# golmschenk/sr-gan

Measured on AMD Instinct MI355X. Metric: SRGAN train images/sec (G+D step), higher is better.
Workload: dtype f32; 1 GPU; crowd SRGAN (KnnDenseNetCat D/DNN + DCGenerator) 512x512, batch 16/GPU, dnn_training_step + gan_training_step per step; global_batch=16, image_size=512, schedule=shared-forwards, parallelism=dp1, random_init_weights=True, gradient_penalty=active, launch=eager (Python tape enqueues every kernel), schedule_check=not run: the --full option runs it

## Files before the change

### include/srgan_hip.h

```cpp
#ifndef SRGAN_HIP_H
#define SRGAN_HIP_H

#include <stdint.h>

#ifdef __cplusplus
extern "C" {
#endif

int srgan_version(void);
const char* srgan_build_id(void);
const char* srgan_last_error(void);

#define SRGAN_DTYPE_F32 0x1u
#define SRGAN_DTYPE_BF16 0x2u
#define SRGAN_DTYPE_F16 0x4u
#define SRGAN_FEATURE_FUSED_BNRELU 0x1u
#define SRGAN_FEATURE_SPLITK_WORKSPACE 0x2u
#define SRGAN_FEATURE_LIVE_PROFILE 0x4u
#define SRGAN_FEATURE_BLOCKED16 0x8u
#define SRGAN_FEATURE_BATCHED_SHADOWS 0x10u
#define SRGAN_FEATURE_CROWD_FULL_IMAGE 0x20u
#define SRGAN_FEATURE_IMAGE_BATCHES 0x40u
#define SRGAN_FEATURE_BATCH_NORM_TRAIN 0x80u
#define SRGAN_FEATURE_BLOCKED_BATCH_NORM 0x100u
#define SRGAN_FEATURE_BLOCKED_FROZEN_NORM 0x200u
#define SRGAN_FEATURE_DEVICE_DRAWS 0x400u
#define SRGAN_FEATURE_IMAGE_SUMMARIES 0x800u
#define SRGAN_FEATURE_DISTRIBUTION_SUMMARIES 0x1000u
typedef struct srgan_capabilities_t {
  int32_t abi_version;
  int32_t struct_bytes;
  char arch[16];
  uint32_t dtypes;
  uint32_t features;
  int64_t workspace_bytes;
  int64_t max_tensor_elements;
} srgan_capabilities_t;
int srgan_capabilities(srgan_capabilities_t* out, int32_t out_bytes);
int64_t srgan_workspace_bytes(void);
int srgan_set_workspace(void* workspace, int64_t bytes, void* stream);
int srgan_split_is_ordered(void* stream);

typedef struct srgan_conv_desc {
  int32_t N, C, H, W;
  int32_t K, R, S;
  int32_t stride_h, stride_w, pad_h, pad_w;
  int32_t OH, OW;
  int64_t x_batch_stride, y_batch_stride;
  int32_t compute_dtype;
} srgan_conv_desc;

#define SRGAN_COMPUTE_F32 0
#define SRGAN_COMPUTE_BF16 1
#define SRGAN_COMPUTE_F16 2

int srgan_conv2d_fwd(const srgan_conv_desc* desc, const float* x, const float* w, const float* bias, float* y,
                     int force_kernel, void* stream);

int srgan_conv2d_bwd_data(const srgan_conv_desc* desc, const float* gy, const float* w, const float* bias, float* gx,
                          int accumulate, int force_kernel, void* stream);

int srgan_conv2d_bwd_weight(const srgan_conv_desc* desc, const float* x, const float* gy, float* gw, int accumulate,
                            int force_kernel, void* stream);

typedef struct srgan_bn_relu { const float* mean; const float* inv_std; const float* gamma; const float* beta; } srgan_bn_relu;
int srgan_conv2d_bnrelu_supported(const srgan_conv_desc* desc, int pass);
int srgan_conv2d_fwd_bnrelu(const srgan_conv_desc* desc, const float* x, const srgan_bn_relu* bn, const float* w,
                            const float* bias, float* y, void* stream);
int srgan_conv2d_fwd_bnrelu_splits(const srgan_conv_desc* desc);
int srgan_conv2d_fwd_bnrelu_into_zeros(const srgan_conv_desc* desc, const float* x, const srgan_bn_relu* bn, const float* w,
                                       const float* bias, float* y, void* stream);
int srgan_conv2d_bwd_data_bnrelu(const srgan_conv_desc* desc, const float* gy, const float* w, const srgan_bn_relu* bn,
                                 const float* x, float* gx, float* g_gamma, float* g_beta, int accumulate, void* stream);
int srgan_conv2d_bwd_weight_bnrelu(const srgan_conv_desc* desc, const float* x, const srgan_bn_relu* bn, const float* gy,
                                   float* gw, int accumulate, void* stream);
typedef struct srgan_bn_reduce_job {
  int64_t partial_offset;
  int32_t tiles, channels;
  const float* inv_std;
  float* g_gamma;
  float* g_beta;
} srgan_bn_reduce_job;
int64_t srgan_conv2d_bwd_data_bnrelu_tiles(const srgan_conv_desc* desc);
int srgan_conv2d_bwd_data_bnrelu_partials(const srgan_conv_desc* desc, const float* gy, const float* w, const srgan_bn_relu* bn,
                                          const float* x, float* gx, float* partials, int accumulate, void* stream);
int srgan_bn_partial_reduce_batched(const srgan_bn_reduce_job* jobs_device, int32_t count, int32_t max_channels, int32_t max_tiles,
                                    const float* scratch, void* stream);

int srgan_wgrad_group_plan(const srgan_conv_desc* desc, const srgan_bn_relu* bn, int64_t x_offset, int64_t gy_offset, float* gw,
                           int64_t gw_offset, int32_t group_size, int64_t group_weights, int64_t partial_offset, void* job,
                           int32_t* grid_x, int32_t* grid_y, int32_t* ragged, int64_t* partial_floats);
int srgan_wgrad_group_run(const void* jobs, int32_t count, int32_t kernel_size, int32_t grid_x, int32_t grid_y, int32_t ragged,
                          int32_t fused_bn, const float* x_base, const float* gy_base, float* gw_base, int64_t sum_co_ci_taps,
                          int64_t pixels, int64_t operand_elements, int64_t partial_floats, void* stream);

int srgan_gemm_f32(int32_t M, int32_t N, int32_t K, const float* A, int64_t sai, int64_t sak, const float* B,
                   int64_t sbk, int64_t sbj, float* C, int64_t sci, int64_t scj, const float* bias,
                   int32_t bias_on_columns, int accumulate, int force_kernel, void* stream);
int srgan_gemm(int32_t M, int32_t N, int32_t K, const float* A, int64_t sai, int64_t sak, const float* B,
               int64_t sbk, int64_t sbj, float* C, int64_t sci, int64_t scj, const float* bias,
               int32_t bias_on_columns, int accumulate, int force_kernel, int compute_dtype, void* stream);

int srgan_ew_unary(int op, const float* x, float* y, int64_t n, float p0, float p1, void* stream);
int srgan_ew_binary(int op, const float* a, const float* b, float* y, int64_t n, float p0, void* stream);
int srgan_fill(float* y, int64_t n, float value, void* stream);

int srgan_chan_affine(const float* x, const float* mean, const float* scale_a, const float* scale_b, const float* shift,
                      float* y, int32_t N, int32_t C, int64_t HW, void* stream);

int srgan_chan_affine_act(const float* x, const float* mean, const float* scale_a, const float* scale_b,
                          const float* shift, const float* mask, int relu, float* y, int32_t N, int32_t C, int64_t HW,
                          void* stream);
int srgan_chan_affine_act_strided(const float* x, const float* mean, const float* scale_a, const float* scale_b,
                                  const float* shift, const float* mask, int relu, float* y, int32_t N, int32_t C,
                                  int64_t HW, int64_t x_batch_stride, int64_t mask_batch_stride, int64_t y_batch_stride,
                                  int accumulate, void* stream);
int srgan_bn_conv_tangent_weights(const float* w, const float* q, const float* inv_std, const float* gamma,
                                  float* w_scaled, float* w_grad, float* gamma_grad, int32_t CO, int32_t CI, int32_t taps,
                                  void* stream);

int srgan_bn_conv_tangent_weights_job(const float* w, const float* inv_std, const float* gamma, float* w_grad,
                                      float* gamma_grad, int64_t offset, int32_t CO, int32_t CI, int32_t taps, void* job);
int srgan_bn_conv_tangent_weights_grouped(const void* jobs, int32_t count, int32_t max_inner, int32_t max_co, float* scaled_base,
                                          const float* q_base, void* stream);

int srgan_bn_act_bwd(const float* g, const float* x, const float* mean, const float* inv_std, const float* gamma,
                     const float* beta, int relu, float* gx, float* g_gamma, float* g_beta, int32_t N, int32_t C,
                     int64_t HW, int64_t g_batch_stride, int64_t x_batch_stride, int64_t gx_batch_stride,
                     int accumulate_gx, int unscaled, void* stream);

int srgan_batch_norm_train_stats(const float* x, float* mean, float* inv_std, float* running_mean, float* running_var,
                                 int64_t* num_batches_tracked, float momentum, float eps, int32_t N, int32_t C, int64_t HW,
                                 void* stream);
int srgan_batch_norm_train_fwd(const float* x, const float* mean, const float* inv_std, const float* gamma, const float* beta,
                               float slope, float* y, int32_t N, int32_t C, int64_t HW, void* stream);
int srgan_batch_norm_train_bwd_reduce(const float* g, const float* x, const float* mean, const float* inv_std, const float* gamma,
                                      const float* beta, float slope, float* sums, float* g_gamma, float* g_beta, int32_t N,
                                      int32_t C, int64_t HW, void* stream);
int srgan_batch_norm_train_bwd_apply(const float* g, const float* x, const float* mean, const float* inv_std, const float* gamma,
                                     const float* beta, float slope, const float* sums, float* gx, int32_t N, int32_t C, int64_t HW,
                                     void* stream);

int srgan_chan_reduce(const float* a, const float* b, const float* mean, const float* scale, float* out, int32_t N,
                      int32_t C, int64_t HW, int accumulate, void* stream);
int srgan_row_max(const float* x, float* out, int32_t B, int32_t F, void* stream);
int srgan_nearest_bin_onehot(const float* y, const float* bins, float* onehot, int32_t B, int32_t K, void* stream);

int srgan_copy_channels(const float* src, int32_t src_channels, int32_t src_first, float* dst, int32_t dst_channels,
                        int32_t dst_first, int32_t count, int32_t N, int64_t HW, int accumulate, void* stream);

int srgan_bn_relu_maxpool_fwd(const float* x, const float* mean, const float* inv_std, const float* gamma, const float* beta,
                              float* y, int32_t* argmax, int32_t N, int32_t C, int32_t H, int32_t W, int32_t k, int32_t s, int32_t p,
                              int32_t OH, int32_t OW, void* stream);
int srgan_bn_relu_maxpool_bwd_supported(int32_t N, int32_t C, int32_t H, int32_t W, int32_t k, int32_t s, int32_t p);
int srgan_bn_relu_maxpool_bwd(const float* gy, const int32_t* argmax, const float* x, const float* mean, const float* inv_std,
                              const float* gamma, const float* beta, float* gx, float* g_gamma, float* g_beta, int32_t N,
                              int32_t C, int32_t H, int32_t W, int32_t k, int32_t s, int32_t p, int32_t OH, int32_t OW,
                              void* stream);
int srgan_bn_relu_avgpool2_supported(int32_t N, int32_t C, int32_t H, int32_t W);
int srgan_bn_relu_avgpool2_fwd(const float* x, const float* mean, const float* inv_std, const float* gamma, const float* beta,
                               float* y, int32_t N, int32_t C, int32_t H, int32_t W, void* stream);
int srgan_bn_relu_avgpool2_bwd(const float* gy, const float* x, const float* mean, const float* inv_std, const float* gamma,
                               const float* beta, float* gx, float* g_gamma, float* g_beta, int32_t N, int32_t C, int32_t H,
                               int32_t W, void* stream);
int srgan_maxpool2d_fwd(const float* x, float* y, int32_t* argmax, int32_t planes, int32_t H, int32_t W, int32_t k,
                        int32_t s, int32_t p, int32_t OH, int32_t OW, void* stream);
int srgan_maxpool2d_bwd(const float* g, const int32_t* argmax, float* gx, int32_t planes, int32_t H, int32_t W, int32_t k,
                        int32_t s, int32_t p, int32_t OH, int32_t OW, void* stream);
int srgan_pool_scatter(const float* g, const int32_t* argmax, float* out, int32_t planes, int64_t in_plane,
                       int64_t out_plane, void* stream);
// ... 20 lines not shown

int srgan_image_batch_gather(const void* store, int store_dtype, int32_t count, int32_t C, int32_t h, int32_t w,
                             const float* labels, const int32_t* order, int64_t first, int32_t B, int32_t H, int32_t W,
                             float* out_images, float* out_labels, void* stream);

int srgan_crowd_extract_windows(const void* image_u8, int32_t H, int32_t W, const int32_t* ys, int32_t ny,
                                const int32_t* xs, int32_t nx, int32_t first, int32_t count, int32_t P,
                                float* out_images, void* stream);
int srgan_crowd_resize_bilinear(const float* in, int32_t B, int32_t h, int32_t w, int32_t P, float* out, void* stream);
int srgan_crowd_blend_windows(const float* densities, const float* counts, const int32_t* ys, int32_t ny, const int32_t* xs,
                              int32_t nx, int32_t H, int32_t W, int32_t P, float* out_density, float* out_count,
                              void* stream);

int srgan_image_grid(const float* images, int32_t N, int32_t C, int32_t H, int32_t W, int32_t nrow, int32_t padding,
                     float pad_value, int32_t normalize, float low, float high, float* out, void* stream);
int srgan_density_heatmaps(const float* labels, const float* predicted, int32_t B, int32_t M, int32_t h, int32_t w, int32_t P,
                           const float* lut, int32_t lut_entries, float* tiles, int64_t tile_stride, float* ranges, void* stream);

#define SRGAN_WASSERSTEIN_MAX_VALUES 16384
int srgan_wasserstein_1d(const float* u, int32_t n, const float* v, int32_t m, float* out, void* stream);
int srgan_kde_curves(const float* samples, const int32_t* offsets, int32_t C, int32_t G, float factor, float cut, float* support,
                     float* density, float* stats, void* stream);
int srgan_curve_frame(const float* vertices, const int32_t* offsets, int32_t C, const float* colours, const float* widths,
                      int32_t H, int32_t W, float x_lo, float x_hi, float y_lo, float y_hi, const float* background,
                      const float* grid_colour, const float* x_ticks, int32_t n_x, const float* y_ticks, int32_t n_y, float* out,
                      void* stream);

int srgan_crowd_iknn_map(const float* heads_yx, int32_t M, int32_t H, int32_t W, int32_t k, float epsilon, float upper_bound,
                         float* out, void* stream);
int srgan_crowd_density_label(const float* heads, int32_t M, int32_t H, int32_t W, float beta, const float* perspective,
                              int32_t flags, void* workspace, float* out, void* stream);

int srgan_adam_step(float* p, const float* g, float* m, float* v, int64_t n, float lr, float beta1, float beta2,
                    float eps, float weight_decay, int32_t step, void* stream);
int srgan_adam_step_counted(float* p, const float* g, float* m, float* v, int64_t n, float lr, float beta1, float beta2,
                            float eps, float weight_decay, int32_t* state, void* stream);

int srgan_pack_bf16(const float* src, uint16_t* dst, int64_t n, void* stream);
int srgan_unpack_bf16(const uint16_t* src, float* dst, int64_t n, void* stream);

int srgan_comm_available(void);
int srgan_comm_unique_id(void* id128);
int srgan_comm_init(void** comm, int32_t world_size, int32_t rank, const void* id128);
int srgan_comm_world_size(void* comm, int32_t* world_size);
int srgan_comm_destroy(void* comm);
int srgan_all_reduce_sum(void* comm, const void* send, void* recv, int64_t count, int32_t dtype, void* stream);
int srgan_reduce_scatter_sum(void* comm, const void* send, void* recv, int64_t recv_count, int32_t dtype, void* stream);
int srgan_all_gather(void* comm, const void* send, void* recv, int64_t send_count, int32_t dtype, void* stream);
int srgan_broadcast(void* comm, void* buffer, int64_t count, int32_t dtype, int32_t root, void* stream);

int srgan_h_pack(const float* x_nchw, void* out, const void* mask_ref, float slope, int32_t N, int32_t C, int64_t HW, int dtype,
                 void* stream);
int srgan_h_unpack(const void* x, float* out_nchw, int32_t N, int32_t C, int64_t HW, int dtype, void* stream);
int srgan_h_add(const void* a, const void* b, void* out, int64_t slots, int dtype, void* stream);
int srgan_h_channel_sums(const void* x, float* out, int32_t N, int32_t C, int64_t HW, int dtype, void* stream);
int srgan_h_maxpool2(const void* x, const void* g, void* out, int64_t planes, int32_t H, int32_t W, int mode, int dtype, void* stream);
int srgan_h_maxpool2_bwd(const void* x, const void* gp, void* gx, int64_t planes, int32_t H, int32_t W, int masked, float slope,
                         int dtype, void* stream);
int64_t srgan_h_conv_weight_slots(int32_t rows, int32_t reduced, int32_t R, int32_t S);
int srgan_h_pack_conv_weights(const float* w, void* packed, int32_t K, int32_t C, int32_t R, int32_t S, int transposed, int dtype,
                              void* stream);
int srgan_h_conv3x3(const void* x, const void* packed, const float* bias, const void* ref, float slope, int epi, void* out,
                    int32_t N, int32_t C_in, int32_t C_out, int32_t rows, int32_t H, int32_t W, int dtype, void* stream);
int srgan_h_conv3x3_wgrad(const void* x, const void* gy, float* gw, int32_t N, int32_t C_in, int32_t C_out, int32_t H, int32_t W,
                          int dtype, void* stream);
int srgan_h_pack_matrix(const float* src, void* out, int64_t rows, int64_t cols, int64_t rows_real, int64_t cols_real,
                        int64_t row_stride, int64_t col_stride, int32_t row_plane, int32_t col_plane, int dtype, void* stream);
int srgan_h_gemm(const void* a, const void* b, const float* bias, const void* ref, float slope, int epi, void* out, int32_t M,
                 int32_t N, int32_t K, int32_t out_cols, int32_t bias_entries, int dtype, void* stream);
int srgan_h_linear_wgrad(const void* s, const void* x, float* gw, int32_t N, int32_t M, int32_t K, int64_t M_real, int64_t K_real,
                         int64_t ldw_m, int64_t ldw_k, int32_t row_plane, int32_t col_plane, int dtype, void* stream);

int64_t srgan_h_k4s2_weight_slots(int32_t A, int32_t B, int direction, int dtype);
int srgan_h_pack_k4s2_weights(const float* w, void* packed, int32_t A, int32_t B, int direction, int dtype, void* stream);
int32_t srgan_h_pack_job_bytes(void);
int64_t srgan_h_pack_job_conv_weights(void* jobs, int64_t first_block, const float* w, void* packed, int32_t K, int32_t C, int32_t R,
                                      int32_t S, int transposed, int dtype);
int64_t srgan_h_pack_job_k4s2_weights(void* jobs, int64_t first_block, const float* w, void* packed, int32_t A, int32_t B,
                                      int direction, int dtype, int32_t* jobs_written);
int64_t srgan_h_pack_job_matrix(void* jobs, int64_t first_block, const float* src, void* out, int64_t rows, int64_t cols,
                                int64_t rows_real, int64_t cols_real, int64_t row_stride, int64_t col_stride, int32_t row_plane,
                                int32_t col_plane, int dtype);
int64_t srgan_h_pack_job_bias_rows(void* jobs, int64_t first_block, const float* bias, float* rows, int32_t channels, int32_t plane);
int srgan_h_pack_batched(const void* jobs_device, int32_t count, int64_t blocks, void* stream);
int srgan_h_conv4x4s2(const void* x, const void* packed, const float* bias, const void* ref, float slope, int epi, void* out,
                      int32_t N, int32_t C_in, int32_t rows, int32_t H, int32_t W, int dtype, void* stream);
int srgan_h_conv_transpose4x4s2(const void* x, const void* packed, const float* bias, const void* ref, float slope, int epi,
                                void* out, int32_t N, int32_t C_in, int32_t rows, int32_t h, int32_t w, int dtype, void* stream);
int srgan_h_k4s2_wgrad(const void* big, const void* small, float* gw, int32_t N, int32_t C_big, int32_t C_small, int32_t H, int32_t W,
                       int small_is_rows, int dtype, void* stream);

int srgan_h_batch_norm_stats(const void* x, float* mean, float* inv_std, float* running_mean, float* running_var,
                             int64_t* num_batches_tracked, float momentum, float eps, int32_t N, int32_t C, int64_t HW,
                             int32_t dtype, void* stream);
int srgan_h_batch_norm_fwd(const void* x, const float* mean, const float* inv_std, const float* gamma, const float* beta,
                           float slope, void* y, int32_t N, int32_t C, int64_t HW, int32_t dtype, void* stream);
int srgan_h_batch_norm_bwd_reduce(const void* s, const void* x, const float* mean, const float* inv_std, float* sums,
                                  float* g_gamma, float* g_beta, int32_t N, int32_t C, int64_t HW, int32_t dtype, void* stream);
int srgan_h_batch_norm_bwd_apply(const void* s, const void* x, const float* mean, const float* inv_std, const float* gamma,
                                 const float* sums, const void* ref, float slope, void* gx, int32_t N, int32_t C, int64_t HW,
                                 int32_t dtype, void* stream);
int srgan_h_frozen_norm_bwd(const void* s, const void* x, const float* mean, const float* inv_std, const float* gamma,
                            const void* ref, float slope, void* gx, float* g_gamma, float* g_beta, int32_t N, int32_t C, int64_t HW,
                            int32_t dtype, void* stream);

int srgan_profile_begin(void);
int srgan_profile_end(double* kernel_ms, double* flops, double* mfma_flops, int64_t* launches);
int srgan_profile_bytes(double* algorithmic_bytes_total);
int srgan_profile_mixed(double* flops, double* kernel_ms);
int64_t srgan_profile_report(char* buffer, int64_t capacity);

#ifdef __cplusplus
}
#endif
#endif
```

### sr-gan_amd/_lib.py

```python
import ctypes
import os

from ._build import LIBRARY, source_id

c_float_p = ctypes.c_void_p
i32, i64, f32, vp = ctypes.c_int32, ctypes.c_int64, ctypes.c_float, ctypes.c_void_p


class ConvDesc(ctypes.Structure):
    _fields_ = [(name, i32) for name in ('N', 'C', 'H', 'W', 'K', 'R', 'S', 'stride_h', 'stride_w', 'pad_h', 'pad_w',
                                         'OH', 'OW')] + [('x_batch_stride', i64), ('y_batch_stride', i64), ('compute_dtype', i32)]


class BnRelu(ctypes.Structure):
    _fields_ = [(name, vp) for name in ('mean', 'inv_std', 'gamma', 'beta')]


class BnReduceJob(ctypes.Structure):
    _fields_ = [('partial_offset', i64), ('tiles', i32), ('channels', i32), ('inv_std', vp), ('g_gamma', vp), ('g_beta', vp)]


class Capabilities(ctypes.Structure):
    _fields_ = [('abi_version', i32), ('struct_bytes', i32), ('arch', ctypes.c_char * 16), ('dtypes', ctypes.c_uint32),
                ('features', ctypes.c_uint32), ('workspace_bytes', i64), ('max_tensor_elements', i64)]


SIGNATURES = {
    'srgan_version': ([], ctypes.c_int),
    'srgan_build_id': ([], ctypes.c_char_p),
    'srgan_last_error': ([], ctypes.c_char_p),
    'srgan_conv2d_fwd': ([ctypes.POINTER(ConvDesc), vp, vp, vp, vp, ctypes.c_int, vp], ctypes.c_int),
    'srgan_conv2d_bwd_data': ([ctypes.POINTER(ConvDesc), vp, vp, vp, vp, ctypes.c_int, ctypes.c_int, vp],
                              ctypes.c_int),
    'srgan_conv2d_bwd_weight': ([ctypes.POINTER(ConvDesc), vp, vp, vp, ctypes.c_int, ctypes.c_int, vp], ctypes.c_int),
    'srgan_conv2d_bnrelu_supported': ([ctypes.POINTER(ConvDesc), ctypes.c_int], ctypes.c_int),
    'srgan_conv2d_fwd_bnrelu': ([ctypes.POINTER(ConvDesc), vp, ctypes.POINTER(BnRelu), vp, vp, vp, vp], ctypes.c_int),
    'srgan_conv2d_fwd_bnrelu_into_zeros': ([ctypes.POINTER(ConvDesc), vp, ctypes.POINTER(BnRelu), vp, vp, vp, vp],
                                           ctypes.c_int),
    'srgan_conv2d_fwd_bnrelu_splits': ([ctypes.POINTER(ConvDesc)], ctypes.c_int),
    'srgan_bn_conv_tangent_weights': ([vp, vp, vp, vp, vp, vp, vp, i32, i32, i32, vp], ctypes.c_int),
    'srgan_conv2d_bwd_data_bnrelu': ([ctypes.POINTER(ConvDesc), vp, vp, ctypes.POINTER(BnRelu), vp, vp, vp, vp,
                                      ctypes.c_int, vp], ctypes.c_int),
    'srgan_conv2d_bwd_data_bnrelu_tiles': ([ctypes.POINTER(ConvDesc)], ctypes.c_int64),
    'srgan_conv2d_bwd_data_bnrelu_partials': ([ctypes.POINTER(ConvDesc), vp, vp, ctypes.POINTER(BnRelu), vp, vp, vp,
                                               ctypes.c_int, vp], ctypes.c_int),
    'srgan_bn_partial_reduce_batched': ([vp, i32, i32, i32, vp, vp], ctypes.c_int),
    'srgan_conv2d_bwd_weight_bnrelu': ([ctypes.POINTER(ConvDesc), vp, ctypes.POINTER(BnRelu), vp, vp, ctypes.c_int, vp],
                                       ctypes.c_int),
    'srgan_gemm_f32': ([i32, i32, i32, vp, i64, i64, vp, i64, i64, vp, i64, i64, vp, i32, ctypes.c_int, ctypes.c_int,
                        vp], ctypes.c_int),
    'srgan_gemm': ([i32, i32, i32, vp, i64, i64, vp, i64, i64, vp, i64, i64, vp, i32, ctypes.c_int, ctypes.c_int,
                    ctypes.c_int, vp], ctypes.c_int),
    'srgan_ew_unary': ([ctypes.c_int, vp, vp, i64, f32, f32, vp], ctypes.c_int),
    'srgan_ew_binary': ([ctypes.c_int, vp, vp, vp, i64, f32, vp], ctypes.c_int),
    'srgan_fill': ([vp, i64, f32, vp], ctypes.c_int),
    'srgan_chan_affine': ([vp, vp, vp, vp, vp, vp, i32, i32, i64, vp], ctypes.c_int),
    'srgan_chan_affine_act': ([vp, vp, vp, vp, vp, vp, ctypes.c_int, vp, i32, i32, i64, vp], ctypes.c_int),
    'srgan_chan_affine_act_strided': ([vp, vp, vp, vp, vp, vp, ctypes.c_int, vp, i32, i32, i64, i64, i64, i64,
                                       ctypes.c_int, vp], ctypes.c_int),
    'srgan_bn_act_bwd': ([vp, vp, vp, vp, vp, vp, ctypes.c_int, vp, vp, vp, i32, i32, i64, i64, i64, i64, ctypes.c_int,
                          ctypes.c_int, vp],
                         ctypes.c_int),
    'srgan_batch_norm_train_stats': ([vp, vp, vp, vp, vp, vp, f32, f32, i32, i32, i64, vp], ctypes.c_int),
    'srgan_batch_norm_train_fwd': ([vp, vp, vp, vp, vp, f32, vp, i32, i32, i64, vp], ctypes.c_int),
    'srgan_batch_norm_train_bwd_reduce': ([vp, vp, vp, vp, vp, vp, f32, vp, vp, vp, i32, i32, i64, vp], ctypes.c_int),
    'srgan_batch_norm_train_bwd_apply': ([vp, vp, vp, vp, vp, vp, f32, vp, vp, i32, i32, i64, vp], ctypes.c_int),
    'srgan_chan_reduce': ([vp, vp, vp, vp, vp, i32, i32, i64, ctypes.c_int, vp], ctypes.c_int),
    'srgan_row_max': ([vp, vp, i32, i32, vp], ctypes.c_int),
    'srgan_nearest_bin_onehot': ([vp, vp, vp, i32, i32, vp], ctypes.c_int),
    'srgan_copy_channels': ([vp, i32, i32, vp, i32, i32, i32, i32, i64, ctypes.c_int, vp], ctypes.c_int),
    'srgan_bn_relu_maxpool_fwd': ([vp, vp, vp, vp, vp, vp, vp, i32, i32, i32, i32, i32, i32, i32, i32, i32, vp], ctypes.c_int),
    'srgan_bn_relu_maxpool_bwd_supported': ([i32, i32, i32, i32, i32, i32, i32], ctypes.c_int),
    'srgan_bn_relu_maxpool_bwd': ([vp, vp, vp, vp, vp, vp, vp, vp, vp, vp, i32, i32, i32, i32, i32, i32, i32, i32, i32, vp],
                                  ctypes.c_int),
    'srgan_bn_relu_avgpool2_supported': ([i32, i32, i32, i32], ctypes.c_int),
    'srgan_bn_relu_avgpool2_fwd': ([vp, vp, vp, vp, vp, vp, i32, i32, i32, i32, vp], ctypes.c_int),
    'srgan_bn_relu_avgpool2_bwd': ([vp, vp, vp, vp, vp, vp, vp, vp, vp, i32, i32, i32, i32, vp], ctypes.c_int),
    'srgan_maxpool2d_fwd': ([vp, vp, vp, i32, i32, i32, i32, i32, i32, i32, i32, vp], ctypes.c_int),
    'srgan_maxpool2d_bwd': ([vp, vp, vp, i32, i32, i32, i32, i32, i32, i32, i32, vp], ctypes.c_int),
    'srgan_pool_scatter': ([vp, vp, vp, i32, i64, i64, vp], ctypes.c_int),
    'srgan_pool_gather': ([vp, vp, vp, i32, i64, i64, vp], ctypes.c_int),
    'srgan_avgpool2d_fwd': ([vp, vp, i32, i32, i32, i32, i32, i32, i32, vp], ctypes.c_int),
    'srgan_avgpool2d_bwd': ([vp, vp, i32, i32, i32, i32, i32, i32, i32, vp], ctypes.c_int),
    'srgan_gp_interpolate': ([vp, vp, vp, vp, i32, i64, vp], ctypes.c_int),
    'srgan_random_fill': ([vp, i64, i64, i32, f32, i32, vp, vp], ctypes.c_int),
    'srgan_random_advance': ([vp, vp], ctypes.c_int),
    'srgan_crowd_map_l1_fwd': ([vp, vp, vp, i32, i32, i64, vp], ctypes.c_int),
    'srgan_crowd_map_l1_bwd': ([vp, vp, vp, vp, i32, i32, i64, vp], ctypes.c_int),
    'srgan_profile_begin': ([], ctypes.c_int),
    'srgan_profile_end': ([ctypes.POINTER(ctypes.c_double), ctypes.POINTER(ctypes.c_double),
                           ctypes.POINTER(ctypes.c_double), ctypes.POINTER(ctypes.c_int64)], ctypes.c_int),
    'srgan_profile_report': ([ctypes.c_char_p, ctypes.c_int64], ctypes.c_int64),
    'srgan_profile_bytes': ([ctypes.POINTER(ctypes.c_double)], ctypes.c_int),
    'srgan_profile_mixed': ([ctypes.POINTER(ctypes.c_double), ctypes.POINTER(ctypes.c_double)], ctypes.c_int),
    'srgan_capabilities': ([ctypes.POINTER(Capabilities), i32], ctypes.c_int),
    'srgan_workspace_bytes': ([], ctypes.c_int64),
    'srgan_set_workspace': ([vp, i64, vp], ctypes.c_int),
    'srgan_split_is_ordered': ([vp], ctypes.c_int),
    'srgan_crowd_density_label': ([vp, i32, i32, i32, f32, vp, i32, vp, vp, vp], ctypes.c_int),
    'srgan_crowd_iknn_map': ([vp, i32, i32, i32, i32, f32, f32, vp, vp], ctypes.c_int),
    'srgan_crowd_extract_patches': ([vp, vp, vp, vp, vp, vp, vp, vp, i32, i32, vp, vp, vp, vp], ctypes.c_int),
    'srgan_image_batch_gather': ([vp, ctypes.c_int, i32, i32, i32, i32, vp, vp, i64, i32, i32, i32, vp, vp, vp], ctypes.c_int),
    'srgan_crowd_extract_windows': ([vp, i32, i32, vp, i32, vp, i32, i32, i32, i32, vp, vp], ctypes.c_int),
    'srgan_crowd_resize_bilinear': ([vp, i32, i32, i32, i32, vp, vp], ctypes.c_int),
    'srgan_crowd_blend_windows': ([vp, vp, vp, i32, vp, i32, i32, i32, i32, vp, vp, vp], ctypes.c_int),
    'srgan_image_grid': ([vp, i32, i32, i32, i32, i32, i32, f32, i32, f32, f32, vp, vp], ctypes.c_int),
    'srgan_density_heatmaps': ([vp, vp, i32, i32, i32, i32, i32, vp, i32, vp, i64, vp, vp], ctypes.c_int),
    'srgan_wasserstein_1d': ([vp, i32, vp, i32, vp, vp], ctypes.c_int),
    'srgan_kde_curves': ([vp, vp, i32, i32, f32, f32, vp, vp, vp, vp], ctypes.c_int),
    'srgan_curve_frame': ([vp, vp, i32, vp, vp, i32, i32, f32, f32, f32, f32, vp, vp, vp, i32, vp, i32, vp, vp], ctypes.c_int),
    'srgan_bn_conv_tangent_weights_job': ([vp, vp, vp, vp, vp, i64, i32, i32, i32, vp], ctypes.c_int),
    'srgan_bn_conv_tangent_weights_grouped': ([vp, i32, i32, i32, vp, vp, vp], ctypes.c_int),
    'srgan_wgrad_group_plan': ([ctypes.POINTER(ConvDesc), ctypes.POINTER(BnRelu), i64, i64, vp, i64, i32, i64, i64, vp, ctypes.POINTER(i32),
                                ctypes.POINTER(i32), ctypes.POINTER(i32), ctypes.POINTER(i64)], ctypes.c_int),
    'srgan_wgrad_group_run': ([vp, i32, i32, i32, i32, i32, i32, vp, vp, vp, i64, i64, i64, i64, vp], ctypes.c_int),
    'srgan_adam_step': ([vp, vp, vp, vp, i64, f32, f32, f32, f32, f32, i32, vp], ctypes.c_int),
    'srgan_adam_step_counted': ([vp, vp, vp, vp, i64, f32, f32, f32, f32, f32, vp, vp], ctypes.c_int),
    'srgan_pack_bf16': ([vp, vp, i64, vp], ctypes.c_int),
    'srgan_unpack_bf16': ([vp, vp, i64, vp], ctypes.c_int),
    'srgan_h_pack': ([vp, vp, vp, f32, i32, i32, i64, ctypes.c_int, vp], ctypes.c_int),
    'srgan_h_unpack': ([vp, vp, i32, i32, i64, ctypes.c_int, vp], ctypes.c_int),
    'srgan_h_add': ([vp, vp, vp, i64, ctypes.c_int, vp], ctypes.c_int),
    'srgan_h_channel_sums': ([vp, vp, i32, i32, i64, ctypes.c_int, vp], ctypes.c_int),
    'srgan_h_maxpool2': ([vp, vp, vp, i64, i32, i32, ctypes.c_int, ctypes.c_int, vp], ctypes.c_int),
    'srgan_h_maxpool2_bwd': ([vp, vp, vp, i64, i32, i32, ctypes.c_int, f32, ctypes.c_int, vp], ctypes.c_int),
    'srgan_h_conv_weight_slots': ([i32, i32, i32, i32], ctypes.c_int64),
    'srgan_h_pack_conv_weights': ([vp, vp, i32, i32, i32, i32, ctypes.c_int, ctypes.c_int, vp], ctypes.c_int),
    'srgan_h_conv3x3': ([vp, vp, vp, vp, f32, ctypes.c_int, vp, i32, i32, i32, i32, i32, i32, ctypes.c_int, vp], ctypes.c_int),
    'srgan_h_conv3x3_wgrad': ([vp, vp, vp, i32, i32, i32, i32, i32, ctypes.c_int, vp], ctypes.c_int),
    'srgan_h_pack_matrix': ([vp, vp, i64, i64, i64, i64, i64, i64, i32, i32, ctypes.c_int, vp], ctypes.c_int),
    'srgan_h_gemm': ([vp, vp, vp, vp, f32, ctypes.c_int, vp, i32, i32, i32, i32, i32, ctypes.c_int, vp], ctypes.c_int),
    'srgan_h_linear_wgrad': ([vp, vp, vp, i32, i32, i32, i64, i64, i64, i64, i32, i32, ctypes.c_int, vp], ctypes.c_int),
    'srgan_h_k4s2_weight_slots': ([i32, i32, ctypes.c_int, ctypes.c_int], ctypes.c_int64),
    'srgan_h_pack_k4s2_weights': ([vp, vp, i32, i32, ctypes.c_int, ctypes.c_int, vp], ctypes.c_int),
    'srgan_h_pack_job_bytes': ([], ctypes.c_int32),
    'srgan_h_pack_job_conv_weights': ([vp, i64, vp, vp, i32, i32, i32, i32, ctypes.c_int, ctypes.c_int], ctypes.c_int64),
    'srgan_h_pack_job_k4s2_weights': ([vp, i64, vp, vp, i32, i32, ctypes.c_int, ctypes.c_int, vp], ctypes.c_int64),
    'srgan_h_pack_job_matrix': ([vp, i64, vp, vp, i64, i64, i64, i64, i64, i64, i32, i32, ctypes.c_int], ctypes.c_int64),
    'srgan_h_pack_job_bias_rows': ([vp, i64, vp, vp, i32, i32], ctypes.c_int64),
    'srgan_h_pack_batched': ([vp, i32, i64, vp], ctypes.c_int),
    'srgan_h_conv4x4s2': ([vp, vp, vp, vp, f32, ctypes.c_int, vp, i32, i32, i32, i32, i32, ctypes.c_int, vp], ctypes.c_int),
    'srgan_h_conv_transpose4x4s2': ([vp, vp, vp, vp, f32, ctypes.c_int, vp, i32, i32, i32, i32, i32, ctypes.c_int, vp], ctypes.c_int),
    'srgan_h_k4s2_wgrad': ([vp, vp, vp, i32, i32, i32, i32, i32, ctypes.c_int, ctypes.c_int, vp], ctypes.c_int),
    'srgan_h_batch_norm_stats': ([vp, vp, vp, vp, vp, vp, f32, f32, i32, i32, i64, i32, vp], ctypes.c_int),
    'srgan_h_batch_norm_fwd': ([vp, vp, vp, vp, vp, f32, vp, i32, i32, i64, i32, vp], ctypes.c_int),
    'srgan_h_batch_norm_bwd_reduce': ([vp, vp, vp, vp, vp, vp, vp, i32, i32, i64, i32, vp], ctypes.c_int),
    'srgan_h_batch_norm_bwd_apply': ([vp, vp, vp, vp, vp, vp, vp, f32, vp, i32, i32, i64, i32, vp], ctypes.c_int),
    'srgan_h_frozen_norm_bwd': ([vp, vp, vp, vp, vp, vp, f32, vp, vp, vp, i32, i32, i64, i32, vp], ctypes.c_int),
    'srgan_comm_available': ([], ctypes.c_int),
    'srgan_comm_unique_id': ([vp], ctypes.c_int),
    'srgan_comm_init': ([ctypes.POINTER(vp), i32, i32, vp], ctypes.c_int),
    'srgan_comm_world_size': ([vp, ctypes.POINTER(i32)], ctypes.c_int),
    'srgan_comm_destroy': ([vp], ctypes.c_int),
    'srgan_all_reduce_sum': ([vp, vp, vp, i64, i32, vp], ctypes.c_int),
    'srgan_reduce_scatter_sum': ([vp, vp, vp, i64, i32, vp], ctypes.c_int),
    'srgan_all_gather': ([vp, vp, vp, i64, i32, vp], ctypes.c_int),
    'srgan_broadcast': ([vp, vp, i64, i32, i32, vp], ctypes.c_int),
}


EINVAL, EUNSUPPORTED, ERANGE = -1, -2, -3


class HipLibraryError(RuntimeError):

    def __init__(self, message, status=None):
        super().__init__(message)
        self.status = status


_library = None


def library():
    global _library
    if _library is None:
        if not os.path.exists(LIBRARY):
            raise HipLibraryError(f'{LIBRARY} is missing: run `python -c "import __graft_entry__ as g; g.build()"` '
                                  '(there is no CPU fallback)')
        import torch
        lib = ctypes.CDLL(LIBRARY)
        for name, (argtypes, restype) in SIGNATURES.items():
            function = getattr(lib, name)
            function.argtypes = argtypes
            function.restype = restype
        built_from = lib.srgan_build_id().decode()
        if built_from != source_id() and os.environ.get('SRGAN_ALLOW_STALE_LIBRARY') != '1':
            raise HipLibraryError(f'{LIBRARY} was built from other kernel sources (library {built_from}, tree '
                                  f'{source_id()}): rebuild with `python -c "import __graft_entry__ as g; g.build()"`')
        _library = lib
    return _library


def capabilities():
    out = Capabilities()
    check(library().srgan_capabilities(ctypes.byref(out), ctypes.sizeof(out)), 'srgan_capabilities')
    return out


_workspaces = {}


def stream_handle(stream=None):
    import torch
    if stream is None:
        device = torch._C._cuda_getDevice()
        handle = torch._C._cuda_getCurrentRawStream(device)
    else:
        device, handle = stream.device.index, stream.cuda_stream
    if (device, handle) not in _workspaces:
        lib = library()
        with torch.cuda.device(device):
            block = torch.empty(lib.srgan_workspace_bytes() // 4, dtype=torch.float32, device=torch.device('cuda', device))
            check(lib.srgan_set_workspace(block.data_ptr(), block.numel() * 4, handle), 'srgan_set_workspace')
        _workspaces[(device, handle)] = block
    return handle


def check(status, what):
    if status != 0:
        message = library().srgan_last_error()
        raise HipLibraryError(f'{what} failed with status {status}: {message.decode() if message else ""}', status)
# ... 1 lines not shown
```

### sr-gan_amd/blocked16.py

```python
import collections
import ctypes
import os

import torch

from . import _lib
from . import functional as F
from .tape import Var, accumulates_into

TORCH_DTYPE = {0: torch.float32, 1: torch.bfloat16, 2: torch.float16}
CODES = {'f32': 0, 'bf16': 1, 'f16': 2, 'fp16': 2}


def group_size(code):
    return 4 if code == 0 else 8


def active_code():
    if not F.STORAGE_DTYPE:
        return None
    return 0 if F.STORAGE_DTYPE == F.STORAGE_BLOCKED_F32 else F.STORAGE_DTYPE


class Blocked:
# ... 145 lines not shown
    data = _new(out_meta.n, out_meta.c, out_meta.h, out_meta.w, out_meta.code, a.device)
    _call(name, a.data_ptr(), b.data_ptr(), bias, _ptr(ref), float(slope), epi, data.data_ptr(), *extents, out_meta.code, F._stream())
    return data, out_meta


class Form(collections.namedtuple('Form', 'name slots source packer tail dtype', defaults=(torch.int32,))):
    __slots__ = ()


class Shadow:
    kind = None

    def __init__(self, module, code, in_blocked=0, plane=1):
        _refuse_under_capture(f'a new {self.kind} weight shadow')
        self.module, self.code, self.in_blocked, self.plane = module, code, in_blocked, plane
        self.forward = self.transposed = self.down = self.up = self.bias_rows = None
        self.key = None
        self._measure()
        arena = getattr(module.weight, '_srgan_arena', None)
        if arena is not None:
            arena.shadows.append(self)

    def fresh(self):
        if self.key != self._version():
            _refuse_under_capture(f'a {self.kind} weight shadow behind its masters')
            self.repack()
            torch.cuda.current_stream().synchronize()
        return self

    def repack(self):
        stream = F._stream()
        for form in self.forms():
            self._pack(form, self._buffer(form.name, form.slots, form.dtype), stream)
        self.key = self._version()

    def _pack(self, form, target, stream):
        _call('srgan_h_pack_' + form.packer, form.source.data_ptr(), target, *form.tail, stream)

    def _fill(self, job, first_block, form, target):
        name = 'srgan_h_pack_job_' + form.packer
        taken = getattr(_lib.library(), name)(job, first_block, form.source.data_ptr(), target, *form.tail)
        _lib.check(min(taken, 0), name)
        return 1, taken

    def _buffer(self, name, slots, dtype=torch.int32):
        if getattr(self, name, None) is None:
            _refuse_under_capture(f'the first {name} buffer of a {self.kind} weight shadow')
            setattr(self, name, torch.empty(slots * 4, dtype=dtype, device=self.module.weight.device))
        return getattr(self, name).data_ptr()

    def _version(self):
        weight = self.module.weight
        arena = getattr(weight, '_srgan_arena', None)
        bias = getattr(self.module, 'bias', None)
        return (weight.data_ptr(), weight._version, None if bias is None else bias._version,
                None if arena is None else (arena.version, arena.data._version))


class Conv3x3Shadow(Shadow):
    kind = 'conv3x3'

    def _measure(self):
        self.k, self.c, self.r, self.s = self.module.weight.shape

    def forms(self):
        k, c, r, s = self.k, self.c, self.r, self.s
        slots = _lib.library().srgan_h_conv_weight_slots
        for name, transposed, rows, reduced in (('forward', 0, k, c), ('transposed', 1, c, k)):
            yield Form(name, slots(rows, reduced, r, s), self.module.weight, 'conv_weights', (k, c, r, s, transposed, self.code))

    def launch(self, x, transposed, epi, slope, ref, bias):
        meta = x.meta
        c_in, c_out = (self.k, self.c) if transposed else (self.c, self.k)
        if meta.c != c_in:
            raise ValueError(f'blocked16 conv: input has {meta.c} channels, the layer expects {c_in}')
        operand = self.transposed if transposed else self.forward
        return _contract('srgan_h_conv3x3', x.data, operand, F._ptr(bias), ref, slope, epi,
                         Blocked(meta.n, c_out, meta.h, meta.w, meta.code), meta.n, c_in, c_out, c_out, meta.h, meta.w)

    def weight_gradient(self, x_side, y_side, into):
        xm = x_side.meta
        _call('srgan_h_conv3x3_wgrad', x_side.data.data_ptr(), y_side.data.data_ptr(), into.data_ptr(), xm.n, xm.c, y_side.meta.c,
              xm.h, xm.w, xm.code, F._stream())


class K4s2Shadow(Shadow):
    kind = 'k4s2'

    def _measure(self):
        self.a, self.b = self.module.weight.shape[:2]
        self.transpose = isinstance(self.module, torch.nn.ConvTranspose2d)

    def forms(self):
        slots = _lib.library().srgan_h_k4s2_weight_slots
        for name, direction in (('down', 0), ('up', 1)):
            yield Form(name, slots(self.a, self.b, direction, self.code), self.module.weight, 'k4s2_weights',
                       (self.a, self.b, direction, self.code))

    def _fill(self, job, first_block, form, target):
        written = ctypes.c_int32()
        _, taken = super()._fill(job, first_block, form._replace(tail=form.tail + (ctypes.byref(written),)), target)
        return written.value, taken

    def launch(self, x, transposed, epi, slope, ref, bias):
        meta, a, b = x.meta, self.a, self.b
        if self.transpose != transposed:
            if meta.c != a:
                raise ValueError(f'blocked16 transposed 4x4 / s2: input has {meta.c} channels, expected {a}')
            return _contract('srgan_h_conv_transpose4x4s2', x.data, self.up, F._ptr(bias), ref, slope, epi,
                             Blocked(meta.n, b, 2 * meta.h, 2 * meta.w, meta.code), meta.n, a, b, meta.h, meta.w)
        if meta.c != b or meta.h % 2 or meta.w % 2:
            raise ValueError(f'blocked16 4x4 / s2: input [{meta.c}, {meta.h}, {meta.w}], expected {b} channels on an even plane')
        return _contract('srgan_h_conv4x4s2', x.data, self.down, F._ptr(bias), ref, slope, epi,
                         Blocked(meta.n, a, meta.h // 2, meta.w // 2, meta.code), meta.n, b, a, meta.h, meta.w)

    def weight_gradient(self, x_side, y_side, into):
        big, small = (y_side, x_side) if self.transpose else (x_side, y_side)
        _call('srgan_h_k4s2_wgrad', big.data.data_ptr(), small.data.data_ptr(), into.data_ptr(), big.meta.n, big.meta.c, small.meta.c,
              big.meta.h, big.meta.w, 1, x_side.meta.code, F._stream())


class LinearShadow(Shadow):
    kind = 'linear'

    def _measure(self):
        weight = self.module.weight
        self.outputs, self.inputs = weight.shape[0], weight.numel() // weight.shape[0]
        self.blocked = self.in_blocked or (self.inputs + 7) // 8 * 8
        self.outputs_padded = (self.outputs + 7) // 8 * 8

    def forms(self):
        outputs, inputs, blocked, padded = self.outputs, self.inputs, self.blocked, self.outputs_padded
        weight, plane, code = self.module.weight, self.plane, self.code
        yield Form('forward', outputs * blocked // 8, weight, 'matrix', (outputs, blocked, outputs, inputs, inputs, 1, 1, plane, code))
        yield Form('transposed', blocked * padded // 8, weight, 'matrix', (blocked, padded, inputs, outputs, 1, inputs, plane, 1, code))

    def launch(self, x, transposed, epi, slope, ref, bias):
        meta, outputs, blocked = x.meta, self.outputs, self.blocked
        if transposed:
            if meta.c != outputs:
                raise ValueError(f'blocked16 linear (data gradient): input has {meta.c} features, expected {outputs}')
            return _contract('srgan_h_gemm', self.transposed, x.data, None, ref, slope, epi,
                             Blocked(meta.n, blocked, 1, 1, meta.code, plane=self.plane, real=self.inputs),
                             blocked, meta.n, outputs, blocked, 0)
        if meta.c != blocked:
            raise ValueError(f'blocked16 linear: input has {meta.c} (blocked) features, the shadow was built for {blocked}')
        return _contract('srgan_h_gemm', self.forward, x.data, F._ptr(bias), ref, slope, epi, Blocked(meta.n, outputs, 1, 1, meta.code),
                         outputs, meta.n, blocked, outputs, outputs)

    def weight_gradient(self, x_side, y_side, into):
        xm = x_side.meta
        _call('srgan_h_linear_wgrad', y_side.data.data_ptr(), x_side.data.data_ptr(), into.data_ptr(), xm.n, self.outputs, xm.c,
              self.outputs, self.inputs, self.inputs, 1, 1, self.plane, xm.code, F._stream())


class SeedShadow(Shadow):
    kind = 'linear_t'

    def _measure(self):
        self.c_in, self.c_out, self.r, self.s = self.module.weight.shape
        self.plane = self.r * self.s
        self.features = self.c_out * self.plane
        self.blocked = (self.c_out + 7) // 8 * 8 * self.plane
        self.c_in_padded = (self.c_in + 7) // 8 * 8

    def forms(self):
        c_in, features, blocked, padded, plane = self.c_in, self.features, self.blocked, self.c_in_padded, self.plane
        weight, code = self.module.weight, self.code
        yield Form('forward', blocked * padded // 8, weight, 'matrix', (blocked, padded, features, c_in, 1, features, plane, 1, code))
        yield Form('transposed', c_in * blocked // 8, weight, 'matrix', (c_in, blocked, c_in, features, features, 1, 1, plane, code))
        if self.module.bias is not None:
            yield Form('bias_rows', blocked // 4, self.module.bias, 'bias_rows', (self.c_out, plane), torch.float32)

    def _pack(self, form, target, stream):
        if form.name != 'bias_rows':
            return super()._pack(form, target, stream)
        channels, plane = form.tail
        full = channels // 8
        rows, bias = self.bias_rows.view(-1, plane, 8), form.source.data
        if full:
            rows[:full].copy_(bias[:full * 8].view(full, 1, 8).expand(full, plane, 8))
        if channels % 8:
            rows[full].zero_()
            rows[full, :, :channels % 8].copy_(bias[full * 8:].view(1, -1).expand(plane, channels % 8))

    def launch(self, x, transposed, epi, slope, ref, bias):
        meta, c_in, c_out, blocked = x.meta, self.c_in, self.c_out, self.blocked
        if transposed:
            if (meta.c, meta.h, meta.w) != (c_out, self.r, self.s):
                raise ValueError('blocked16 seed transposed convolution (data gradient): unexpected input shape')
            return _contract('srgan_h_gemm', self.transposed, x.data, None, ref, slope, epi, Blocked(meta.n, c_in, 1, 1, meta.code),
                             c_in, meta.n, blocked, c_in, 0)
        if meta.c != c_in:
            raise ValueError(f'blocked16 seed transposed convolution: input has {meta.c} features, expected {c_in}')
        rows = None if bias is None else _ptr(self.bias_rows)
        return _contract('srgan_h_gemm', self.forward, x.data, rows, ref, slope, epi, Blocked(meta.n, c_out, self.r, self.s, meta.code),
                         blocked, meta.n, self.c_in_padded, blocked, blocked)

    def weight_gradient(self, x_side, y_side, into):
        xm = x_side.meta
        _call('srgan_h_linear_wgrad', y_side.data.data_ptr(), x_side.data.data_ptr(), into.data_ptr(), xm.n, self.blocked, xm.c,
              self.features, self.c_in, 1, self.features, self.plane, 1, xm.code, F._stream())


SHADOW_KINDS = {cls.kind: cls for cls in (Conv3x3Shadow, K4s2Shadow, LinearShadow, SeedShadow)}
BATCHED_KINDS = tuple(SHADOW_KINDS)


def shadow_of(module, kind, code, in_blocked=0, plane=1):
    table = module.__dict__.setdefault('_srgan_shadows', {})
    key = (kind, code, in_blocked, plane)
    found = table.get(key)
    if found is None:
        found = table[key] = SHADOW_KINDS[kind](module, code, in_blocked, plane)
    return found.fresh()


class _PackPlan:

    def __init__(self, shadows):
        _refuse_under_capture('building the batched shadow refresh')
        size = _lib.library().srgan_h_pack_job_bytes()
        self.shadows = list(shadows)
        self.signature = _signature(self.shadows)
        host = ctypes.create_string_buffer(size * 5 * max(1, len(self.shadows)))
        count = blocks = 0
        device = None
        for shadow in self.shadows:
            device = shadow.module.weight.device
            for form in shadow.forms():
                target = shadow._buffer(form.name, form.slots, form.dtype)
                written, taken = shadow._fill(ctypes.byref(host, count * size), blocks, form, target)
                count, blocks = count + written, blocks + taken
        self.count, self.blocks = count, blocks
        self.table = None
        if count:
            self.table = torch.frombuffer(bytearray(host.raw[:count * size]), dtype=torch.uint8).to(device)

    def run(self):
        if self.table is not None:
            _call('srgan_h_pack_batched', self.table.data_ptr(), self.count, self.blocks, F._stream())
        for shadow in self.shadows:
            shadow.key = shadow._version()


def _signature(shadows):
    return tuple((id(s), s.module.weight.data_ptr(), None if s.module.bias is None else s.module.bias.data_ptr()) for s in shadows)


def _plan(arena):
    plan = getattr(arena, '_pack_plan', None)
    if plan is None or plan.signature != _signature(arena.shadows):
        plan = arena._pack_plan = _PackPlan(arena.shadows)
    return plan


def refresh(arena):
    shadows = getattr(arena, 'shadows', ())
    if not shadows:
        return
    if os.environ.get('SRGAN_H_NO_BATCHED_PACK') == '1':
        for shadow in shadows:
            shadow.repack()
        return
    _plan(arena).run()


def stale(arena):
    return any(shadow.key != shadow._version() for shadow in getattr(arena, 'shadows', ()))


def refresh_if_stale(arena):
    if not stale(arena):
        return False
    refresh(arena)
    return True


def prepare(arena):
    _refuse_under_capture('blocked16.prepare')
    if not getattr(arena, 'shadows', ()):
        return
    if os.environ.get('SRGAN_H_NO_BATCHED_PACK') == '1':
        refresh(arena)
        return
    plan = _plan(arena)
    if stale(arena):
        plan.run()
# ... 220 lines not shown
```

### sr-gan_amd/csrc/blocked16.h

```cpp
#pragma once
#include <type_traits>
#include "common.h"

namespace srgan {

typedef float f32x16 __attribute__((ext_vector_type(16)));
typedef __bf16 h_bf16x8 __attribute__((ext_vector_type(8)));
typedef _Float16 h_f16x8 __attribute__((ext_vector_type(8)));
typedef __bf16 h_bf16x2 __attribute__((ext_vector_type(2)));
typedef _Float16 h_f16x2 __attribute__((ext_vector_type(2)));
typedef short h_s4 __attribute__((ext_vector_type(4)));

struct alignas(16) Slot { uint32_t v[4]; };

template <int PREC>
__device__ __forceinline__ uint32_t h_pack2(float a, float b) {
  if constexpr (PREC == 1) {
    h_bf16x2 h; h[0] = (__bf16)a; h[1] = (__bf16)b;
    return __builtin_bit_cast(uint32_t, h);
  } else {
    h_f16x2 h; h[0] = (_Float16)a; h[1] = (_Float16)b;
    return __builtin_bit_cast(uint32_t, h);
  }
}
// ... 21 lines not shown
  for (int i = 0; i < 4; ++i) s.v[i] = h_pack2<PREC>(f[2 * i], f[2 * i + 1]);
  return s;
}
template <int PREC> struct HGroup { static constexpr int N = PREC == 0 ? 4 : 8; };
template <int PREC>
__device__ __forceinline__ void h_unpack(const Slot& s, float (&f)[HGroup<PREC>::N]) {
  if constexpr (PREC == 0) {
#pragma unroll
    for (int i = 0; i < 4; ++i) f[i] = __uint_as_float(s.v[i]);
  } else {
#pragma unroll
    for (int i = 0; i < 4; ++i) { f[2 * i] = h_lo<PREC>(s.v[i]); f[2 * i + 1] = h_hi<PREC>(s.v[i]); }
  }
}
template <int PREC>
__device__ __forceinline__ Slot h_pack(const float (&f)[HGroup<PREC>::N]) {
  Slot s;
  if constexpr (PREC == 0) {
#pragma unroll
    for (int i = 0; i < 4; ++i) s.v[i] = __float_as_uint(f[i]);
  } else {
#pragma unroll
    for (int i = 0; i < 4; ++i) s.v[i] = h_pack2<PREC>(f[2 * i], f[2 * i + 1]);
  }
  return s;
}
template <int PREC>
__device__ __forceinline__ bool h_slot_positive(const Slot& s, int j) {
  if constexpr (PREC == 0) return __uint_as_float(s.v[j]) > 0.f;
  else return h_positive((s.v[j >> 1] >> (16 * (j & 1))) & 0xFFFFu);
}

__device__ __forceinline__ float h_mask(uint32_t bits16, float slope) { return h_positive(bits16) ? 1.f : slope; }

__device__ __forceinline__ uint2 h_tr_read(uint32_t lds_byte_address) {
  const h_s4 v = __builtin_amdgcn_ds_read_tr16_b64_v4i16((__attribute__((address_space(3))) h_s4*)(uintptr_t)lds_byte_address);
  return __builtin_bit_cast(uint2, v);
}
__device__ __forceinline__ uint32_t h_lds_address(const void* p) {
  return (uint32_t)(uintptr_t)(__attribute__((address_space(3))) const void*)p;
}

template <int PREC>
__device__ __forceinline__ f32x16 h_mfma(const Slot& a, const Slot& b, f32x16 c) {
  if constexpr (PREC == 0) {
#pragma unroll
    for (int i = 0; i < 4; ++i) c = __builtin_amdgcn_mfma_f32_32x32x2f32(__uint_as_float(a.v[i]), __uint_as_float(b.v[i]), c, 0, 0, 0);
    return c;
  } else if constexpr (PREC == 1)
    return __builtin_amdgcn_mfma_f32_32x32x16_bf16(__builtin_bit_cast(h_bf16x8, a), __builtin_bit_cast(h_bf16x8, b), c, 0, 0, 0);
  else
    return __builtin_amdgcn_mfma_f32_32x32x16_f16(__builtin_bit_cast(h_f16x8, a), __builtin_bit_cast(h_f16x8, b), c, 0, 0, 0);
}

__device__ __forceinline__ void h_glds16(const void* lane_pointer, uint32_t lds_dst) {
  unsigned keep;
  asm volatile("s_mov_b32 %0, m0\n\ts_mov_b32 m0, %2\n\ts_nop 0\n\tglobal_load_lds_dwordx4 %1, off\n\ts_mov_b32 m0, %0"
               : "=&s"(keep) : "v"(lane_pointer), "s"(lds_dst) : "memory");
}
template <int N> __device__ __forceinline__ void h_dma_wait_and_barrier() {
  asm volatile("s_waitcnt vmcnt(%0) lgkmcnt(0)\n\ts_barrier" :: "n"(N) : "memory");
}
constexpr int K4_CK = 4;
constexpr int K4_TAPS = 4;

template <int PREC>
__device__ __forceinline__ void h_pack_conv_weights_slot(const float* __restrict__ w, Slot* __restrict__ packed, int64_t slot,
                                                         int32_t CO, int32_t CI, int32_t R, int32_t S, int32_t base, int32_t so,
                                                         int32_t si, int32_t skh, int32_t skw) {
  const int T = R * S;
  const int o = (int)(slot % CO);
  const int64_t rest = slot / CO;
  const int g = (int)(rest & 1);
  const int64_t ct = rest >> 1;
  const int tap = (int)(ct % T), chunk = (int)(ct / T);
  const int kh = tap / S, kw = tap - kh * S;
  float v[8];
#pragma unroll
  for (int j = 0; j < 8; ++j) {
    const int c = chunk * 16 + g * 8 + j;
    v[j] = c < CI ? w[base + o * so + c * si + kh * skh + kw * skw] : 0.f;
  }
  packed[slot] = h_pack8<PREC>(v);
}

template <int PREC>
__device__ __forceinline__ void h_pack_k4s2_weights_slot(const float* __restrict__ w, Slot* __restrict__ packed, int64_t slot,
                                                         int32_t rows, int32_t reduced, int64_t row_stride, int64_t reduced_stride,
                                                         int32_t mode) {
  const int o = (int)(slot % rows);
  int64_t rest = slot / rows;
  const int j = (int)(rest % K4_CK); rest /= K4_CK;
  const int tap = (int)(rest % K4_TAPS);
  const int chunk = (int)(rest / K4_TAPS);
  const int a = tap >> 1, b = tap & 1;
  constexpr int G = HGroup<PREC>::N;
  int kh, kw, first;
  if (mode == 0) { kh = 2 * a + (j >> 1); kw = 2 * b + (j & 1); first = G * chunk; }
  else {
    const int ry = (mode - 1) >> 1, rx = (mode - 1) & 1;
    kh = ry == 0 ? 3 - 2 * a : 2 - 2 * a;
    kw = rx == 0 ? 3 - 2 * b : 2 - 2 * b;
    first = G * (K4_CK * chunk + j);
  }
  float v[G];
#pragma unroll
  for (int i = 0; i < G; ++i)
    v[i] = first + i < reduced ? w[o * row_stride + (int64_t)(first + i) * reduced_stride + kh * 4 + kw] : 0.f;
  packed[slot] = h_pack<PREC>(v);
}

__host__ __device__ __forceinline__ int64_t h_plane_index(int64_t i, int32_t plane) {
  if (plane <= 1) return i;
  const int64_t slot = i >> 3;
  return ((slot / plane) * 8 + (i & 7)) * plane + slot % plane;
}

template <int PREC>
__device__ __forceinline__ void h_pack_matrix_slot(const float* __restrict__ src, Slot* __restrict__ out, int64_t slot,
                                                   int32_t row_slots, int64_t rows_real, int64_t cols_real, int64_t rs, int64_t cs,
                                                   int32_t row_plane, int32_t col_plane) {
  const int64_t r = slot / row_slots;
  const int64_t c0 = (slot % row_slots) * 8;
  const int64_t rr = h_plane_index(r, row_plane);
  float v[8];
#pragma unroll
  for (int j = 0; j < 8; ++j) {
    const int64_t cc = h_plane_index(c0 + j, col_plane);
    v[j] = (rr < rows_real && cc < cols_real) ? src[rr * rs + cc * cs] : 0.f;
  }
  out[slot] = h_pack8<PREC>(v);
}

template <int PREC>
__device__ __forceinline__ void h_pack_matrix_tile(const float* __restrict__ src, Slot* __restrict__ out, float (*tile)[65],
                                                   int tile_index, int64_t rows, int32_t row_slots, int64_t rows_real,
                                                   int64_t cols_real, int64_t cs, int32_t row_plane, int32_t col_plane,
                                                   int32_t tiles_r) {
  const int tid = (int)threadIdx.x;
  const int64_t r0 = (int64_t)(tile_index % tiles_r) * 64, c0 = (int64_t)(tile_index / tiles_r) * 64;
  const int r_load = tid & 63;
  const int64_t rr = h_plane_index(r0 + r_load, row_plane);
  const bool row_ok = r0 + r_load < rows && rr < rows_real;
#pragma unroll
  for (int i = 0; i < 16; ++i) {
    const int c_local = (tid >> 6) + 4 * i;
    const int64_t cc = h_plane_index(c0 + c_local, col_plane);
    tile[c_local][r_load] = (row_ok && c0 + c_local < (int64_t)row_slots * 8 && cc < cols_real) ? src[cc * cs + rr] : 0.f;
  }
  __syncthreads();
#pragma unroll
  for (int i = 0; i < 2; ++i) {
    const int slot_local = tid & 7, r_local = (tid >> 3) + 32 * i;
    if (r0 + r_local >= rows || c0 / 8 + slot_local >= row_slots) continue;
    float v[8];
#pragma unroll
    for (int j = 0; j < 8; ++j) v[j] = tile[slot_local * 8 + j][r_local];
    out[(r0 + r_local) * row_slots + c0 / 8 + slot_local] = h_pack8<PREC>(v);
  }
}

__device__ __forceinline__ void h_bias_rows_slot(const float* __restrict__ bias, float* __restrict__ rows, int64_t slot,
                                                 int32_t channels, int32_t plane) {
  const int g = (int)(slot / plane);
  float4 v[2];
  float* f = reinterpret_cast<float*>(v);
// ... 17 lines not shown
```

### sr-gan_amd/csrc/blocked16.hip

```cpp
#include <type_traits>
#include <string.h>
#include "blocked16.h"
#include "launchers.h"
#include "split_finish.h"
#include <stdlib.h>
#include <atomic>

namespace srgan {

template <int PREC>
__global__ __launch_bounds__(256) void h_pack_kernel(const float* __restrict__ x, Slot* __restrict__ out,
                                                     const Slot* __restrict__ ref, float slope, int64_t slots, int32_t C,
                                                     int32_t CG, int32_t HW) {
  constexpr int G = HGroup<PREC>::N;
  for (int64_t s = (int64_t)blockIdx.x * 256 + threadIdx.x; s < slots; s += (int64_t)gridDim.x * 256) {
    const int pix = (int)(s % HW);
    const int64_t ng = s / HW;
    const int g = (int)(ng % CG);
    const int64_t n = ng / CG;
    float v[G];
#pragma unroll
    for (int j = 0; j < G; ++j) {
      const int c = G * g + j;
      v[j] = c < C ? x[(n * C + c) * HW + pix] : 0.f;
// ... 101 lines not shown
  float v[4][8];
  h_unpack8<PREC>(x[base], v[0]);
  h_unpack8<PREC>(x[base + 1], v[1]);
  h_unpack8<PREC>(x[base + W], v[2]);
  h_unpack8<PREC>(x[base + W + 1], v[3]);
#pragma unroll
  for (int j = 0; j < 8; ++j) {
    m[j] = v[0][j]; at[j] = 0;
#pragma unroll
    for (int q = 1; q < 4; ++q)
      if (v[q][j] > m[j]) { m[j] = v[q][j]; at[j] = q; }
  }
}

template <int PREC, int MODE>
__global__ __launch_bounds__(256) void h_maxpool_kernel(const Slot* __restrict__ x, const Slot* __restrict__ g,
                                                        Slot* __restrict__ out, int64_t planes, int32_t H, int32_t W) {
  const int OH = H / 2, OW = W / 2;
  const int64_t total = planes * OH * OW;
  for (int64_t s = (int64_t)blockIdx.x * 256 + threadIdx.x; s < total; s += (int64_t)gridDim.x * 256) {
    const int ox = (int)(s % OW);
    const int64_t rest = s / OW;
    const int oy = (int)(rest % OH);
    const int64_t plane = rest / OH;
    const int64_t base = (plane * H + 2 * oy) * W + 2 * ox;
    float m[8]; int at[8];
    h_pool_window<PREC>(x, base, W, m, at);
    if (MODE == 0) {
      out[s] = h_pack8<PREC>(m);
    } else {
      float v[4][8], r[8];
      h_unpack8<PREC>(g[base], v[0]);
      h_unpack8<PREC>(g[base + 1], v[1]);
      h_unpack8<PREC>(g[base + W], v[2]);
      h_unpack8<PREC>(g[base + W + 1], v[3]);
#pragma unroll
      for (int j = 0; j < 8; ++j) r[j] = at[j] == 0 ? v[0][j] : (at[j] == 1 ? v[1][j] : (at[j] == 2 ? v[2][j] : v[3][j]));
      out[s] = h_pack8<PREC>(r);
    }
  }
}

template <int PREC>
__global__ __launch_bounds__(256) void h_maxpool_bwd_kernel(const Slot* __restrict__ x, const Slot* __restrict__ gp,
                                                            Slot* __restrict__ gx, int64_t planes, int32_t H, int32_t W,
                                                            int masked, float slope) {
  const int OH = H / 2, OW = W / 2;
  const int64_t total = planes * OH * OW;
  for (int64_t s = (int64_t)blockIdx.x * 256 + threadIdx.x; s < total; s += (int64_t)gridDim.x * 256) {
    const int ox = (int)(s % OW);
    const int64_t rest = s / OW;
    const int oy = (int)(rest % OH);
    const int64_t plane = rest / OH;
    const int64_t base = (plane * H + 2 * oy) * W + 2 * ox;
    float m[8]; int at[8];
    h_pool_window<PREC>(x, base, W, m, at);
    float g[8];
    h_unpack8<PREC>(gp[s], g);
    if (masked) {
#pragma unroll
      for (int j = 0; j < 8; ++j) g[j] *= m[j] > 0.f ? 1.f : slope;
    }
    float r[4][8];
#pragma unroll
    for (int q = 0; q < 4; ++q)
#pragma unroll
      for (int j = 0; j < 8; ++j) r[q][j] = at[j] == q ? g[j] : 0.f;
    gx[base] = h_pack8<PREC>(r[0]);
    gx[base + 1] = h_pack8<PREC>(r[1]);
    gx[base + W] = h_pack8<PREC>(r[2]);
    gx[base + W + 1] = h_pack8<PREC>(r[3]);
  }
}

template <int PREC>
__global__ __launch_bounds__(256) void h_pack_conv_weights_kernel(const float* __restrict__ w, Slot* __restrict__ packed,
                                                                  int64_t slots, int32_t CO, int32_t CI, int32_t R, int32_t S,
                                                                  int32_t base, int32_t so, int32_t si, int32_t skh, int32_t skw) {
  const int64_t slot = (int64_t)blockIdx.x * 256 + threadIdx.x;
  if (slot >= slots) return;
  h_pack_conv_weights_slot<PREC>(w, packed, slot, CO, CI, R, S, base, so, si, skh, skw);
}

__global__ __launch_bounds__(256) void h_pack_batched_kernel(const HPackJob* __restrict__ jobs, int32_t count) {
  __shared__ float tile[64][65];
  int lo = 0, hi = count - 1;
  const int64_t block = blockIdx.x;
  while (lo < hi) {
    const int mid = (lo + hi + 1) >> 1;
    if (jobs[mid].first_block <= block) lo = mid; else hi = mid - 1;
  }
  const HPackJob job = jobs[lo];
  const int64_t slot = (block - job.first_block) * 256 + threadIdx.x;
  if (slot >= job.slots) return;
  const int32_t* q = job.p;
  if (job.kind == 0) {
    if (job.prec == 1) h_pack_conv_weights_slot<1>(job.w, job.packed, slot, q[0], q[1], q[2], q[3], q[4], q[5], q[6], q[7], q[8]);
    else h_pack_conv_weights_slot<2>(job.w, job.packed, slot, q[0], q[1], q[2], q[3], q[4], q[5], q[6], q[7], q[8]);
  } else if (job.kind == 1) {
    if (job.prec == 0) h_pack_k4s2_weights_slot<0>(job.w, job.packed, slot, q[0], q[1], q[2], q[3], q[4]);
    else if (job.prec == 1) h_pack_k4s2_weights_slot<1>(job.w, job.packed, slot, q[0], q[1], q[2], q[3], q[4]);
    else h_pack_k4s2_weights_slot<2>(job.w, job.packed, slot, q[0], q[1], q[2], q[3], q[4]);
  } else if (job.kind == 2) {
    if (job.prec == 1) h_pack_matrix_slot<1>(job.w, job.packed, slot, q[0], q[1], q[2], q[3], q[4], q[5], q[6]);
    else h_pack_matrix_slot<2>(job.w, job.packed, slot, q[0], q[1], q[2], q[3], q[4], q[5], q[6]);
  } else if (job.kind == 3) {
    const int tile_index = (int)(block - job.first_block);
    if (job.prec == 1) h_pack_matrix_tile<1>(job.w, job.packed, tile, tile_index, q[0], q[1], q[2], q[3], q[4], q[5], q[6], q[7]);
    else h_pack_matrix_tile<2>(job.w, job.packed, tile, tile_index, q[0], q[1], q[2], q[3], q[4], q[5], q[6], q[7]);
  } else {
    h_bias_rows_slot(job.w, reinterpret_cast<float*>(job.packed), slot, q[0], q[1]);
  }
}

struct HConv3Params {
  const Slot* in; const Slot* wp; Slot* out; const float* bias; const Slot* ref;
  float slope;
  int32_t epi;
  int32_t N, CGI, CGO, CO, C_real, H, W;
  int32_t chunks, chunks_per_split;
  int32_t tiles_x, tiles_y, tiles_m;
  float* split_ws; unsigned int* split_tickets;
  int32_t xcd_remap;
};

__device__ unsigned int g_hconv3_split_tickets[SPLIT_TICKET_SETS * SPLIT_TICKET_TILES];

template <int BM>
__device__ __forceinline__ void hconv3_stage_bias(const float* bias, int epi, int C_real, int m0, float* bias_rows) {
  if (epi == 1 && bias != nullptr) {
    if ((int)threadIdx.x < BM) bias_rows[threadIdx.x] = m0 + (int)threadIdx.x < C_real ? bias[m0 + threadIdx.x] : 0.f;
    __syncthreads();
  }
}

template <int BM, int NI, int TW, int ROWS, int PREC>
__device__ __forceinline__ void hconv3_epilogue(const HConv3Params& p, f32x16 (&acc)[BM / 32][NI], int n0, int y0, int x0, int m0,
                                                int wave, int l31, int lhi, const float* bias_rows) {
  constexpr int MI = BM / 32;
  const int HW = p.H * p.W;
  const bool with_bias = p.epi == 1 && p.bias != nullptr;
  float4 bias4[MI][4];
#pragma unroll
  for (int mi = 0; mi < MI; ++mi)
#pragma unroll
    for (int qd = 0; qd < 4; ++qd)
      bias4[mi][qd] = with_bias ? *reinterpret_cast<const float4*>(&bias_rows[mi * 32 + 8 * qd + 4 * lhi]) : make_float4(0.f, 0.f, 0.f, 0.f);
#pragma unroll
  for (int ni = 0; ni < NI; ++ni) {
    const int q = (wave * NI + ni) * 32 + l31;
    const int n = n0 + q / (ROWS * TW), y = y0 + (q / TW) % ROWS, x = x0 + q % TW;
    if (n >= p.N || y >= p.H || x >= p.W) continue;
    const int64_t pixel = (int64_t)n * p.CGO * HW + y * p.W + x;
    uint2 refs[MI][4];
    if (p.epi == 2) {
#pragma unroll
      for (int mi = 0; mi < MI; ++mi)
#pragma unroll
        for (int qd = 0; qd < 4; ++qd) {
          const int group = (m0 + mi * 32) / 8 + qd;
          refs[mi][qd] = group < p.CGO ? *(reinterpret_cast<const uint2*>(p.ref + pixel + (int64_t)group * HW) + lhi) : uint2{0u, 0u};
        }
    }
#pragma unroll
    for (int mi = 0; mi < MI; ++mi) {
#pragma unroll
      for (int qp = 0; qp < 2; ++qp) {
        const int g0 = (m0 + mi * 32) / 8 + 2 * qp;
        uint2 packed[2];
#pragma unroll
        for (int h = 0; h < 2; ++h) {
          const int qd = 2 * qp + h;
          float v[4];
#pragma unroll
          for (int j = 0; j < 4; ++j) v[j] = acc[mi][ni][4 * qd + j];
          if (p.epi == 1) {
            const float4 b4 = bias4[mi][qd];
            v[0] += b4.x; v[1] += b4.y; v[2] += b4.z; v[3] += b4.w;
#pragma unroll
            for (int j = 0; j < 4; ++j) v[j] = v[j] > 0.f ? v[j] : v[j] * p.slope;
          } else if (p.epi == 2) {
            const uint2 r = refs[mi][qd];
            v[0] *= h_mask(r.x & 0xFFFFu, p.slope); v[1] *= h_mask(r.x >> 16, p.slope);
            v[2] *= h_mask(r.y & 0xFFFFu, p.slope); v[3] *= h_mask(r.y >> 16, p.slope);
          }
          packed[h].x = h_pack2<PREC>(v[0], v[1]);
          packed[h].y = h_pack2<PREC>(v[2], v[3]);
        }
        const auto first = __builtin_amdgcn_permlane32_swap(packed[0].x, packed[1].x, false, false);
        const auto second = __builtin_amdgcn_permlane32_swap(packed[0].y, packed[1].y, false, false);
        const int group = g0 + lhi;
        if (group < p.CGO) {
          uint4 whole;
          whole.x = first[0]; whole.y = second[0]; whole.z = first[1]; whole.w = second[1];
// ... 464 lines not shown
        b.v[0] = b0.x; b.v[1] = b0.y; b.v[2] = b1.x; b.v[3] = b1.y;
        acc[tap] = h_mfma<PREC>(a, b, acc[tap]);
      }
    }
  }

  float* mine = p.partial + ((int64_t)blockIdx.x * p.walkers + walker) * (9 * 16 * THREADS) + tid;
#pragma unroll
  for (int t = 0; t < 9; ++t)
#pragma unroll
    for (int r = 0; r < 16; ++r) mine[(t * 16 + r) * THREADS] = acc[t][r];
}

__global__ __launch_bounds__(256) void hwgrad3x3_finish_kernel(const float* __restrict__ partial, float* __restrict__ gw,
                                                               int32_t CO, int32_t CI, int32_t tiles_ci, int32_t walkers,
                                                               int32_t block_rows) {
  __shared__ float sums[4][9][64];
  const int lane = (int)threadIdx.x & 63, part = (int)threadIdx.x >> 6;
  const int block = (int)blockIdx.x / block_rows, row = (int)blockIdx.x % block_rows;
  const int tco = block / tiles_ci, tci = block % tiles_ci;
  const int co = tco * block_rows + row;
  if (co >= CO) return;
  const int threads = 4 * block_rows;
  const int64_t per_walker = (int64_t)9 * 16 * threads;
  const int r32 = row & 31, lhi = (r32 >> 2) & 1, r = (r32 & 3) + 4 * (r32 >> 3);
  const int thread = ((row >> 5) * 2 + (lane >> 5)) * 64 + lhi * 32 + (lane & 31);
  const float* base = partial + (int64_t)block * walkers * per_walker + r * threads + thread;
  float total[9];
#pragma unroll
  for (int t = 0; t < 9; ++t) total[t] = 0.f;
  for (int w0 = part; w0 < walkers; w0 += 16) {
    float v[4][9];
#pragma unroll
    for (int d = 0; d < 4; ++d) {
      const int w = w0 + 4 * d;
#pragma unroll
      for (int t = 0; t < 9; ++t) v[d][t] = w < walkers ? base[(int64_t)w * per_walker + t * 16 * threads] : 0.f;
    }
#pragma unroll
    for (int d = 0; d < 4; ++d)
      if (w0 + 4 * d < walkers)
#pragma unroll
        for (int t = 0; t < 9; ++t) total[t] += v[d][t];
  }
#pragma unroll
  for (int t = 0; t < 9; ++t) sums[part][t][lane] = total[t];
  __syncthreads();
  float previous[3];
#pragma unroll
  for (int e = 0; e < 3; ++e) {
    const int i = (int)threadIdx.x + 256 * e, ci_local = i / 9, tap = i - ci_local * 9, ci = tci * 64 + ci_local;
    previous[e] = (i < 576 && ci < CI) ? gw[((int64_t)co * CI + ci) * 9 + tap] : 0.f;
  }
#pragma unroll
  for (int e = 0; e < 3; ++e) {
    const int i = (int)threadIdx.x + 256 * e, ci_local = i / 9, tap = i - ci_local * 9, ci = tci * 64 + ci_local;
    if (i < 576 && ci < CI)
      gw[((int64_t)co * CI + ci) * 9 + tap] = previous[e] + ((sums[0][tap][ci_local] + sums[1][tap][ci_local]) + (sums[2][tap][ci_local] + sums[3][tap][ci_local]));
  }
}

static int check_dtype(int dtype) {
  SRGAN_REQUIRE(dtype == 1 || dtype == 2, SRGAN_EINVAL, "blocked 16-bit tensors are bf16 (1) or fp16 (2)");
  return SRGAN_OK;
}
static int check_dtype_or_f32(int dtype) {
  SRGAN_REQUIRE(dtype >= 0 && dtype <= 2, SRGAN_EINVAL, "blocked tensors are fp32 (0), bf16 (1) or fp16 (2)");
  return SRGAN_OK;
}

static void conv_weights_job(HPackJob& job, const float* w, void* packed, int32_t K, int32_t C, int32_t R, int32_t S, int transposed,
                             int dtype) {
  memset(&job, 0, sizeof(job));
  const int rows = transposed ? C : K, reduced = transposed ? K : C;
  job.w = w; job.packed = (Slot*)packed; job.kind = 0; job.prec = dtype;
  job.slots = (int64_t)((reduced + 15) / 16) * R * S * 2 * rows;
  job.p[0] = rows; job.p[1] = reduced; job.p[2] = R; job.p[3] = S;
  job.p[4] = transposed ? R * S - 1 : 0;
  job.p[5] = transposed ? R * S : C * R * S;
  job.p[6] = transposed ? C * R * S : R * S;
  job.p[7] = transposed ? -S : S; job.p[8] = transposed ? -1 : 1;
}

}

using namespace srgan;

extern "C" {

int srgan_h_pack(const float* x, void* out, const void* mask_ref, float slope, int32_t N, int32_t C, int64_t HW, int dtype,
                 void* stream) {
  hipStream_t s = (hipStream_t)stream;
  if (const int status = check_dtype_or_f32(dtype)) return status;
  SRGAN_REQUIRE(x && out && N >= 0 && C > 0 && HW > 0 && HW < ((int64_t)1 << 31), SRGAN_EINVAL, "srgan_h_pack arguments");
  const int group = dtype == 0 ? 4 : 8, CG = (C + group - 1) / group;
  const int64_t slots = (int64_t)N * CG * HW;
  if (slots == 0) return SRGAN_OK;
  const dim3 grid(stream_grid(slots, 256));
  if (dtype == 0) hipLaunchKernelGGL(h_pack_kernel<0>, grid, dim3(256), 0, s, x, (Slot*)out, (const Slot*)mask_ref, slope, slots, C, CG, (int32_t)HW);
  else if (dtype == 1) hipLaunchKernelGGL(h_pack_kernel<1>, grid, dim3(256), 0, s, x, (Slot*)out, (const Slot*)mask_ref, slope, slots, C, CG, (int32_t)HW);
  else hipLaunchKernelGGL(h_pack_kernel<2>, grid, dim3(256), 0, s, x, (Slot*)out, (const Slot*)mask_ref, slope, slots, C, CG, (int32_t)HW);
  return launch_status();
}

int srgan_h_unpack(const void* x, float* out, int32_t N, int32_t C, int64_t HW, int dtype, void* stream) {
  hipStream_t s = (hipStream_t)stream;
  if (const int status = check_dtype_or_f32(dtype)) return status;
  SRGAN_REQUIRE(x && out && N >= 0 && C > 0 && HW > 0 && HW < ((int64_t)1 << 31), SRGAN_EINVAL, "srgan_h_unpack arguments");
  const int group = dtype == 0 ? 4 : 8, CG = (C + group - 1) / group;
  const int64_t slots = (int64_t)N * CG * HW;
  if (slots == 0) return SRGAN_OK;
  const dim3 grid(stream_grid(slots, 256));
  if (dtype == 0) hipLaunchKernelGGL(h_unpack_kernel<0>, grid, dim3(256), 0, s, (const Slot*)x, out, slots, C, CG, (int32_t)HW);
  else if (dtype == 1) hipLaunchKernelGGL(h_unpack_kernel<1>, grid, dim3(256), 0, s, (const Slot*)x, out, slots, C, CG, (int32_t)HW);
  else hipLaunchKernelGGL(h_unpack_kernel<2>, grid, dim3(256), 0, s, (const Slot*)x, out, slots, C, CG, (int32_t)HW);
  return launch_status();
}

int srgan_h_add(const void* a, const void* b, void* out, int64_t slots, int dtype, void* stream) {
  hipStream_t s = (hipStream_t)stream;
  if (const int status = check_dtype_or_f32(dtype)) return status;
  SRGAN_REQUIRE(a && b && out && slots >= 0, SRGAN_EINVAL, "srgan_h_add arguments");
  if (slots == 0) return SRGAN_OK;
  const dim3 grid(stream_grid(slots, 256));
  if (dtype == 0) hipLaunchKernelGGL(h_add_kernel<0>, grid, dim3(256), 0, s, (const Slot*)a, (const Slot*)b, (Slot*)out, slots);
  else if (dtype == 1) hipLaunchKernelGGL(h_add_kernel<1>, grid, dim3(256), 0, s, (const Slot*)a, (const Slot*)b, (Slot*)out, slots);
  else hipLaunchKernelGGL(h_add_kernel<2>, grid, dim3(256), 0, s, (const Slot*)a, (const Slot*)b, (Slot*)out, slots);
  return launch_status();
}

int srgan_h_channel_sums(const void* x, float* out, int32_t N, int32_t C, int64_t HW, int dtype, void* stream) {
  hipStream_t s = (hipStream_t)stream;
  if (const int status = check_dtype_or_f32(dtype)) return status;
  SRGAN_REQUIRE(x && out && N > 0 && C > 0 && HW > 0 && HW < ((int64_t)1 << 31), SRGAN_EINVAL, "srgan_h_channel_sums arguments");
  const int group = dtype == 0 ? 4 : 8, CG = (C + group - 1) / group;
  const int64_t per_group = (int64_t)N * HW;
  int parts = (int)((per_group + 4095) / 4096);
  if (parts > 256) parts = 256;
  if (parts < 1) parts = 1;
  while (parts > 1 && (int64_t)parts * CG > 4096) parts >>= 1;
  unsigned int* tickets = nullptr;
  float* part = row_finish_workspace(CG, parts, 8, g_h_sum_tickets, s, &tickets);
  if (!part) {
    tickets = nullptr;
    part = partial_workspace((size_t)CG * parts * 8 * sizeof(float), s);
  }
  SRGAN_REQUIRE(part, SRGAN_EINVAL, "srgan_h_channel_sums: register a workspace for this stream first (srgan_set_workspace)");
  const dim3 grid((unsigned)CG, (unsigned)parts);
  if (dtype == 0) hipLaunchKernelGGL(h_channel_sums_kernel<0>, grid, dim3(256), 0, s, (const Slot*)x, part, N, CG, (int32_t)HW, parts, tickets, out, C);
  else if (dtype == 1) hipLaunchKernelGGL(h_channel_sums_kernel<1>, grid, dim3(256), 0, s, (const Slot*)x, part, N, CG, (int32_t)HW, parts, tickets, out, C);
  else hipLaunchKernelGGL(h_channel_sums_kernel<2>, grid, dim3(256), 0, s, (const Slot*)x, part, N, CG, (int32_t)HW, parts, tickets, out, C);
  if (!tickets) hipLaunchKernelGGL(h_channel_sums_finish_kernel, dim3((C + 255) / 256), dim3(256), 0, s, part, out, C, parts, group);
  return launch_status();
}

int srgan_h_maxpool2(const void* x, const void* g, void* out, int64_t planes, int32_t H, int32_t W, int mode, int dtype,
                     void* stream) {
  hipStream_t s = (hipStream_t)stream;
  if (const int status = check_dtype(dtype)) return status;
  SRGAN_REQUIRE(x && out && planes >= 0 && H >= 2 && W >= 2 && H % 2 == 0 && W % 2 == 0 && (mode == 0 || (mode == 2 && g)),
                SRGAN_EINVAL, "srgan_h_maxpool2 arguments (even planes; mode 0 or 2)");
  const int64_t total = planes * (H / 2) * (W / 2);
  if (total == 0) return SRGAN_OK;
  const dim3 grid(stream_grid(total, 256));
  if (dtype == 1) {
    if (mode == 0) hipLaunchKernelGGL((h_maxpool_kernel<1, 0>), grid, dim3(256), 0, s, (const Slot*)x, (const Slot*)g, (Slot*)out, planes, H, W);
// ... 27 lines not shown
                              void* stream) {
  hipStream_t s = (hipStream_t)stream;
  if (const int status = check_dtype(dtype)) return status;
  SRGAN_REQUIRE(w && packed && K > 0 && C > 0 && R > 0 && S > 0, SRGAN_EINVAL, "srgan_h_pack_conv_weights arguments");
  HPackJob job;
  conv_weights_job(job, w, packed, K, C, R, S, transposed, dtype);
  const dim3 grid((unsigned)((job.slots + 255) / 256));
  const int32_t* q = job.p;
  if (dtype == 1) hipLaunchKernelGGL(h_pack_conv_weights_kernel<1>, grid, dim3(256), 0, s, w, (Slot*)packed, job.slots, q[0], q[1], q[2], q[3], q[4], q[5], q[6], q[7], q[8]);
  else hipLaunchKernelGGL(h_pack_conv_weights_kernel<2>, grid, dim3(256), 0, s, w, (Slot*)packed, job.slots, q[0], q[1], q[2], q[3], q[4], q[5], q[6], q[7], q[8]);
  return launch_status();
}

int32_t srgan_h_pack_job_bytes(void) { return (int32_t)sizeof(HPackJob); }

int64_t srgan_h_pack_job_conv_weights(void* jobs, int64_t first_block, const float* w, void* packed, int32_t K, int32_t C, int32_t R,
                                      int32_t S, int transposed, int dtype) {
  if (const int status = check_dtype(dtype)) return status;
  SRGAN_REQUIRE(jobs && first_block >= 0 && w && packed && K > 0 && C > 0 && R > 0 && S > 0, SRGAN_EINVAL,
                "srgan_h_pack_job_conv_weights arguments");
  HPackJob job;
  conv_weights_job(job, w, packed, K, C, R, S, transposed, dtype);
  job.first_block = first_block;
  memcpy(jobs, &job, sizeof(job));
  return (job.slots + 255) / 256;
}

int64_t srgan_h_pack_job_k4s2_weights(void* jobs, int64_t first_block, const float* w, void* packed, int32_t A, int32_t B,
                                      int direction, int dtype, int32_t* jobs_written) {
  SRGAN_REQUIRE(dtype >= 0 && dtype <= 2, SRGAN_EINVAL, "srgan_h_pack_job_k4s2_weights dtype");
  SRGAN_REQUIRE(jobs && first_block >= 0 && w && packed && A > 0 && B > 0 && (direction == 0 || direction == 1) && jobs_written,
                SRGAN_EINVAL, "srgan_h_pack_job_k4s2_weights arguments");
  const int64_t slots = srgan_h_k4s2_weight_slots(A, B, direction, dtype) / (direction ? 4 : 1);
  const int64_t blocks = (slots + 255) / 256;
  const int count = direction ? 4 : 1;
  for (int cls = 0; cls < count; ++cls) {
    HPackJob job;
    memset(&job, 0, sizeof(job));
    job.w = w; job.packed = (Slot*)packed + cls * slots; job.slots = slots; job.first_block = first_block + cls * blocks;
    job.kind = 1; job.prec = dtype;
    job.p[0] = direction ? B : A; job.p[1] = direction ? A : B;
    job.p[2] = direction ? 16 : B * 16; job.p[3] = direction ? B * 16 : 16; job.p[4] = direction ? 1 + cls : 0;
    memcpy((char*)jobs + cls * sizeof(job), &job, sizeof(job));
  }
  *jobs_written = count;
  return count * blocks;
}

int64_t srgan_h_pack_job_matrix(void* jobs, int64_t first_block, const float* src, void* out, int64_t rows, int64_t cols,
                                int64_t rows_real, int64_t cols_real, int64_t row_stride, int64_t col_stride, int32_t row_plane,
                                int32_t col_plane, int dtype) {
  if (const int status = check_dtype(dtype)) return status;
  const int64_t limit = (int64_t)1 << 31;
  SRGAN_REQUIRE(jobs && first_block >= 0 && src && out && rows > 0 && cols > 0 && rows < limit && cols < limit && rows_real >= 0 &&
                rows_real < limit && cols_real >= 0 && cols_real < limit && row_stride > 0 && row_stride < limit && col_stride > 0 &&
                col_stride < limit && row_plane >= 0 && col_plane >= 0, SRGAN_EINVAL, "srgan_h_pack_job_matrix arguments");
  const int64_t row_slots = (cols + 7) / 8;
  HPackJob job;
  memset(&job, 0, sizeof(job));
  job.w = src; job.packed = (Slot*)out; job.first_block = first_block; job.prec = dtype;
  if (row_stride == 1 && col_stride != 1) {
    const int64_t tiles_r = (rows + 63) / 64, tiles = tiles_r * ((row_slots * 8 + 63) / 64);
    SRGAN_REQUIRE(tiles < limit / 256, SRGAN_EINVAL, "srgan_h_pack_job_matrix size");
    job.kind = 3; job.slots = tiles * 256;
    job.p[0] = (int32_t)rows; job.p[1] = (int32_t)row_slots; job.p[2] = (int32_t)rows_real; job.p[3] = (int32_t)cols_real;
    job.p[4] = (int32_t)col_stride; job.p[5] = row_plane; job.p[6] = col_plane; job.p[7] = (int32_t)tiles_r;
  } else {
    job.kind = 2; job.slots = rows * row_slots;
    job.p[0] = (int32_t)row_slots; job.p[1] = (int32_t)rows_real; job.p[2] = (int32_t)cols_real; job.p[3] = (int32_t)row_stride;
    job.p[4] = (int32_t)col_stride; job.p[5] = row_plane; job.p[6] = col_plane;
  }
  memcpy(jobs, &job, sizeof(job));
  return (job.slots + 255) / 256;
}

int64_t srgan_h_pack_job_bias_rows(void* jobs, int64_t first_block, const float* bias, float* rows, int32_t channels, int32_t plane) {
  SRGAN_REQUIRE(jobs && first_block >= 0 && bias && rows && channels > 0 && plane > 0 &&
                (int64_t)(channels + 7) / 8 * plane < ((int64_t)1 << 31), SRGAN_EINVAL, "srgan_h_pack_job_bias_rows arguments");
  HPackJob job;
  memset(&job, 0, sizeof(job));
  job.w = bias; job.packed = (Slot*)rows; job.first_block = first_block; job.kind = 4; job.prec = 0;
  job.slots = (int64_t)(channels + 7) / 8 * plane;
  job.p[0] = channels; job.p[1] = plane;
  memcpy(jobs, &job, sizeof(job));
  return (job.slots + 255) / 256;
}

int srgan_h_pack_batched(const void* jobs_device, int32_t count, int64_t blocks, void* stream) {
  hipStream_t s = (hipStream_t)stream;
  SRGAN_REQUIRE(jobs_device && count > 0 && blocks > 0 && blocks < ((int64_t)1 << 31), SRGAN_EINVAL, "srgan_h_pack_batched arguments");
  hipLaunchKernelGGL(h_pack_batched_kernel, dim3((unsigned)blocks), dim3(256), 0, s, (const HPackJob*)jobs_device, count);
  return launch_status();
}

int srgan_h_conv3x3(const void* x, const void* packed, const float* bias, const void* ref, float slope, int epi, void* out,
                    int32_t N, int32_t C_in, int32_t C_out, int32_t rows, int32_t H, int32_t W, int dtype, void* stream) {
  hipStream_t s = (hipStream_t)stream;
  if (const int status = check_dtype(dtype)) return status;
  SRGAN_REQUIRE(x && packed && out && N > 0 && C_in > 0 && C_out > 0 && rows > 0 && H > 0 && W > 0 && epi >= 0 && epi <= 2 &&
                (epi != 2 || ref), SRGAN_EINVAL, "srgan_h_conv3x3 arguments");
  HConv3Params p;
  p.in = (const Slot*)x; p.wp = (const Slot*)packed; p.out = (Slot*)out; p.bias = bias; p.ref = (const Slot*)ref;
  p.slope = slope; p.epi = epi;
  p.N = N; p.CGI = (C_in + 7) / 8; p.CGO = (C_out + 7) / 8; p.CO = rows; p.C_real = C_out; p.H = H; p.W = W;
  p.chunks = (p.CGI + 1) / 2;
  SRGAN_REQUIRE((int64_t)N * (p.CGI > p.CGO ? p.CGI : p.CGO) * H * W < ((int64_t)1 << 31), SRGAN_ERANGE, "srgan_h_conv3x3 tensor size");
  HConv3Plan plan;
  const int rows_needed = p.CGO * 8 < rows ? p.CGO * 8 : rows;
  SRGAN_REQUIRE(hconv3_plan(N, p.CGI, rows_needed, H, W, plan), SRGAN_EUNSUPPORTED, "srgan_h_conv3x3 plane size");
  p.tiles_x = plan.tiles_x; p.tiles_y = plan.tiles_y; p.tiles_m = plan.tiles_m;
  p.chunks_per_split = plan.chunks_per;
  p.split_ws = nullptr; p.split_tickets = nullptr;
  int split = plan.split;
  if (split > 1) {
    int ticket_set = -1;
    const int64_t accumulators = (int64_t)(plan.bm / 32) * plan.ni * 16 * 256;
    float* ws = split_workspace(plan.blocks, split, accumulators, 0, s, &ticket_set);
    unsigned int* tickets = ws ? device_tickets(g_hconv3_split_tickets) : nullptr;
    if (ws && tickets) {
      p.split_ws = ws;
      p.split_tickets = tickets + (size_t)ticket_set * SPLIT_TICKET_TILES;
    } else {
      split = 1;
      p.chunks_per_split = p.chunks;
    }
  }
  p.xcd_remap = (plan.blocks % 8 == 0 && plan.blocks >= 64) ? 1 : 0;
  const dim3 grid((unsigned)plan.blocks, (unsigned)split, 1);
  static const int ring_env = getenv("SRGAN_H_DMA_RING") ? atoi(getenv("SRGAN_H_DMA_RING")) : -1;
  const int ring = ring_env >= 0 ? ring_env : 2;
  const Slot* zero = (ring == 2 || ring == 3) && split == 1 && plan.bm == 64
                         ? h_zero_slots() : nullptr;
  const int slot = profile_bracket_begin(s);
  if (zero) {
    int launched;
    if (ring == 3) launched = dtype == 1 ? hconv3_dma_launch<1, 3>(p, plan, grid, s, zero) : hconv3_dma_launch<2, 3>(p, plan, grid, s, zero);
    else launched = dtype == 1 ? hconv3_dma_launch<1, 2>(p, plan, grid, s, zero) : hconv3_dma_launch<2, 2>(p, plan, grid, s, zero);
    if (launched != SRGAN_OK) {
      profile_bracket_end(slot, s, 0, 0, 0, 14, plan.bm, plan.ni * 128, split);
      return launched;
    }
  }
  else if (dtype == 1) hconv3_launch<1>(p, plan, grid, s);
  else hconv3_launch<2>(p, plan, grid, s);
  const int status = launch_status();
  const double pixels = (double)N * H * W;
  profile_bracket_end_bytes(slot, s, rows_needed, (int64_t)pixels, (int64_t)p.CGI * 8 * 9, 14, plan.bm, plan.ni * 128, split,
                            2.0 * (pixels * p.CGI * 8 + pixels * p.CGO * 8 * (epi == 2 ? 2 : 1) + (double)rows * p.CGI * 8 * 9), dtype);
  return status;
}

int srgan_h_conv3x3_wgrad(const void* x, const void* gy, float* gw, int32_t N, int32_t C_in, int32_t C_out, int32_t H, int32_t W,
                          int dtype, void* stream) {
  hipStream_t s = (hipStream_t)stream;
  if (const int status = check_dtype(dtype)) return status;
  SRGAN_REQUIRE(x && gy && gw && N > 0 && C_in > 0 && C_out > 0 && H > 0 && W > 0, SRGAN_EINVAL, "srgan_h_conv3x3_wgrad arguments");
  HWgrad3Params p;
  p.x = (const Slot*)x; p.gy = (const Slot*)gy;
  p.N = N; p.CGX = (C_in + 7) / 8; p.CGY = (C_out + 7) / 8; p.H = H; p.W = W;
  int tw, rows;
  if (W > 16) { tw = 32; rows = 2; }
  else if (W == 8 && H == 8) { tw = 8; rows = 8; }
  else if (W == 4 && H == 4) { tw = 4; rows = 4; }
  else { tw = 16; rows = 4; }
  const int img = HWGRAD_P / (rows * tw);
  p.tiles_x = (W + tw - 1) / tw;
// ... 44 lines not shown
```

### sr-gan_amd/csrc/conv3x3.hip

```cpp
#include "common.h"
#include "launchers.h"
#include "split_finish.h"
#include <stdlib.h>
#include <type_traits>

namespace srgan {

typedef float f32x16 __attribute__((ext_vector_type(16)));
typedef __bf16 bf16x8 __attribute__((ext_vector_type(8)));
typedef _Float16 f16x8 __attribute__((ext_vector_type(8)));

struct Conv3Params {
  const float* in;
  const float* w;
  float* out;
  const float* bias;
  int32_t N, CI, CO, H, W;
  int64_t in_bs, out_bs;
  int32_t w_so, w_si, w_skh, w_skw, w_base;
  int32_t tiles_x, tiles_y, tiles_m;
  int32_t ci_per_split;
  int32_t mode;
  float* split_ws;
  unsigned int* split_tickets;
  const float* bn_mean; const float* bn_inv; const float* bn_gamma; const float* bn_beta;
  const float* epi_x; int64_t epi_x_bs;
  float* epi_partial; int32_t epi_tiles;
  const void* w_packed;
  int32_t out_plane, out_sy, out_sx, out_off;
  int32_t taps;
  int32_t xcd_remap;
};

constexpr int CONV3_PRO_MAX_CI = 512;

__device__ unsigned int g_conv3_split_tickets[SPLIT_TICKET_SETS * SPLIT_TICKET_TILES];

template <int BM, int TH, int CI_T, bool PRO, int TW, bool EPI = false, int TAPS = 0x1FF>
__global__ __launch_bounds__(256, 2) void conv3x3_lds_kernel(const Conv3Params p) {
  static_assert(!EPI || !PRO, "the batch-norm backward epilogue pairs with the plain kernel");
  static_assert(TAPS == 0x1FF || (!EPI && !PRO), "tap subsets pair with the plain kernel");
  constexpr int RPB = 32 / TW;
  constexpr int ROWS = TH * RPB;
  constexpr int PH = ROWS + 2, PW = TW + 2, PHPW = PH * PW;
  constexpr int MI = BM / 32, NI = TH / 4;
  constexpr int LDW = BM + 1;
  constexpr int PATCH = CI_T * PHPW, WTS = CI_T * 9 * BM;
  constexpr int NP = (PATCH + 255) / 256, NW = (WTS + 255) / 256;
  static_assert(CI_T % 2 == 0 && NI >= 1 && MI >= 1, "bad tile");
  __shared__ float lds[PATCH + CI_T * 9 * LDW];
  __shared__ float2 coef[PRO ? CONV3_PRO_MAX_CI : 1];
  float* patch = lds;
  float* wt = lds + PATCH;

  const int tid = threadIdx.x, lane = tid & 63, wave = tid >> 6, l31 = lane & 31, lhi = lane >> 5;
  int block = blockIdx.x;
  if (p.xcd_remap) block = (block & 7) * ((int)gridDim.x >> 3) + (block >> 3);
  const int logical_block = block;
  const int tm = block % p.tiles_m; block /= p.tiles_m;
  const int tx = block % p.tiles_x; block /= p.tiles_x;
  const int ty = block % p.tiles_y;
  const int n = block / p.tiles_y;
  const int m0 = tm * BM, y0 = ty * ROWS, x0 = tx * TW;
  const int cbeg = (int)blockIdx.y * p.ci_per_split;
  const int cend = min(p.CI, cbeg + p.ci_per_split);
  const int HW = p.H * p.W;

  int poff[NP], woff[NW];
#pragma unroll
  for (int e = 0; e < NP; ++e) {
    const int flat = e * 256 + tid;
    const int c = flat / PHPW, rem = flat - c * PHPW;
    const int py = rem / PW, px = rem - py * PW;
    const int y = y0 - 1 + py, x = x0 - 1 + px;
    const bool ok = flat < PATCH && (unsigned)y < (unsigned)p.H && (unsigned)x < (unsigned)p.W;
    poff[e] = ok ? c * HW + y * p.W + x : -1;
  }
#pragma unroll
  for (int e = 0; e < NW; ++e) {
    const int flat = e * 256 + tid;
    const int o = flat / (CI_T * 9), r = flat - o * (CI_T * 9);
    const int ci = r / 9, tap = r - ci * 9;
    const int kh = tap / 3, kw = tap - kh * 3;
    const bool ok = flat < WTS && (m0 + o) < p.CO && ((p.taps >> tap) & 1);
    woff[e] = ok ? p.w_base + (m0 + o) * p.w_so + ci * p.w_si + kh * p.w_skh + kw * p.w_skw : -1;
  }
  const float* in_n = p.in + (int64_t)n * p.in_bs;

  float rp[NP], rw[NW];
  auto fetch = [&](int c0) {
    const int room = cend - c0;
#pragma unroll
    for (int e = 0; e < NP; ++e) {
      const int flat = e * 256 + tid;
      const bool ok = poff[e] >= 0 && flat / PHPW < room;
      rp[e] = in_n[(int64_t)c0 * HW + (ok ? poff[e] : 0)];
    }
#pragma unroll
    for (int e = 0; e < NW; ++e) {
      const int flat = e * 256 + tid;
      const int ci = (flat % (CI_T * 9)) / 9;
      const bool ok = woff[e] >= 0 && ci < room;
      rw[e] = p.w[ok ? woff[e] + c0 * p.w_si : 0];
    }
  };
  auto stage = [&](int c0) {
    const int room = cend - c0;
#pragma unroll
    for (int e = 0; e < NP; ++e) {
      const int flat = e * 256 + tid;
      const bool ok = poff[e] >= 0 && flat / PHPW < room;
      float v = rp[e];
      if (PRO) {
        const float2 cf = coef[min(c0 - cbeg + flat / PHPW, CONV3_PRO_MAX_CI - 1)];
        v = fmaxf(fmaf(v, cf.x, cf.y), 0.f);
      }
      if (flat < PATCH) patch[flat] = ok ? v : 0.f;
    }
#pragma unroll
    for (int e = 0; e < NW; ++e) {
      const int flat = e * 256 + tid;
      const int o = flat / (CI_T * 9), r = flat - o * (CI_T * 9);
      const bool ok = woff[e] >= 0 && r / 9 < room;
      if (flat < WTS) wt[r * LDW + o] = ok ? rw[e] : 0.f;
    }
  };

  f32x16 acc[MI][NI];
#pragma unroll
  for (int mi = 0; mi < MI; ++mi)
#pragma unroll
    for (int ni = 0; ni < NI; ++ni)
#pragma unroll
      for (int r = 0; r < 16; ++r) acc[mi][ni][r] = 0.f;

  const float* a_base = wt + lhi * 9 * LDW + l31;
  const float* b_base = patch + lhi * PHPW + ((wave * NI) * RPB + l31 / TW) * PW + l31 % TW;

  if (cbeg < cend) {
    fetch(cbeg);
    if (PRO) {
      for (int c = tid; c < cend - cbeg; c += 256) {
        float a, b;
        bn_coefficients(p.bn_mean[cbeg + c], p.bn_inv[cbeg + c], p.bn_gamma[cbeg + c], p.bn_beta[cbeg + c], a, b);
        coef[c] = make_float2(a, b);
      }
      __syncthreads();
    }
    stage(cbeg);
    __syncthreads();
    for (int c0 = cbeg; c0 < cend; c0 += CI_T) {
      const bool more = c0 + CI_T < cend;
      if (more) fetch(c0 + CI_T);
#pragma unroll 1
      for (int cp = 0; cp < CI_T / 2; ++cp) {
        const float* a_cp = a_base + cp * (2 * 9 * LDW);
        const float* b_cp = b_base + cp * (2 * PHPW);
#pragma unroll
        for (int tap = 0; tap < 9; ++tap) {
          if (!((TAPS >> tap) & 1)) continue;
          const int kh = tap / 3, kw = tap % 3;
          float a[MI], b[NI];
#pragma unroll
          for (int mi = 0; mi < MI; ++mi) a[mi] = a_cp[tap * LDW + mi * 32];
#pragma unroll
          for (int ni = 0; ni < NI; ++ni) b[ni] = b_cp[(ni * RPB + kh) * PW + kw];
#pragma unroll
          for (int mi = 0; mi < MI; ++mi)
#pragma unroll
            for (int ni = 0; ni < NI; ++ni)
              acc[mi][ni] = __builtin_amdgcn_mfma_f32_32x32x2f32(a[mi], b[ni], acc[mi][ni], 0, 0, 0);
        }
      }
      __syncthreads();
      if (more) {
        stage(c0 + CI_T);
        __syncthreads();
      }
    }
  }

  const int x = x0 + l31 % TW;
  float* out_n = p.out + (int64_t)n * p.out_bs;
  if (EPI) {
    float* table = lds;
    float* sums = lds + BM * 4;
    if (tid < BM) {
      const int o = min(m0 + tid, p.CO - 1);
      const float mu = p.bn_mean[o];
      float a, b;
      bn_coefficients(mu, p.bn_inv[o], p.bn_gamma[o], p.bn_beta[o], a, b);
      table[tid * 4 + 0] = a; table[tid * 4 + 1] = b; table[tid * 4 + 2] = mu;
    }
    __syncthreads();
    const float* x_n = p.epi_x + (int64_t)n * p.epi_x_bs;
    const bool sums_wanted = p.epi_partial != nullptr;
    int pix[NI];
    bool inside[NI];
#pragma unroll
    for (int ni = 0; ni < NI; ++ni) {
      const int y = y0 + (wave * NI + ni) * RPB + l31 / TW;
      inside[ni] = y < p.H && x < p.W;
      pix[ni] = inside[ni] ? y * p.W + x : 0;
    }
#pragma unroll
    for (int mi = 0; mi < MI; ++mi) {
      float xs[NI][16];
#pragma unroll
      for (int ni = 0; ni < NI; ++ni)
#pragma unroll
        for (int r = 0; r < 16; ++r) {
          const int o = min(m0 + mi * 32 + (r & 3) + 8 * (r >> 2) + 4 * lhi, p.CO - 1);
          xs[ni][r] = x_n[(int64_t)o * HW + pix[ni]];
        }
#pragma unroll
      for (int r = 0; r < 16; ++r) {
        const int row = mi * 32 + (r & 3) + 8 * (r >> 2) + 4 * lhi;
        const int o = m0 + row;
        const float4 t = *reinterpret_cast<const float4*>(table + row * 4);
        float plain = 0.f, centred = 0.f;
#pragma unroll
        for (int ni = 0; ni < NI; ++ni) {
          const bool ok = inside[ni] && o < p.CO;
          const float v = (ok && fmaf(xs[ni][r], t.x, t.y) > 0.f) ? acc[mi][ni][r] : 0.f;
          if (ok) __builtin_nontemporal_store(v * t.x, out_n + (int64_t)o * HW + pix[ni]);
          plain += v;
          centred += v * (xs[ni][r] - t.z);
        }
        if (sums_wanted) {
          plain = half_wave_sum(plain);
          centred = half_wave_sum(centred);
          if (l31 == 31) {
            sums[(wave * 2 + 0) * BM + row] = plain;
            sums[(wave * 2 + 1) * BM + row] = centred;
          }
        }
      }
    }
    if (sums_wanted) {
      __syncthreads();
      if (tid < 2 * BM) {
        const int q = tid / BM, row = tid - q * BM;
        const float total = (sums[(0 * 2 + q) * BM + row] + sums[(1 * 2 + q) * BM + row]) +
                            (sums[(2 * 2 + q) * BM + row] + sums[(3 * 2 + q) * BM + row]);
        const int o = m0 + row;
        if (o < p.CO) p.epi_partial[((int64_t)q * p.epi_tiles + logical_block / p.tiles_m) * p.CO + o] = total;
      }
    }
    return;
  }
  int mode = p.mode;
  if (mode >= 3) {
    constexpr int COUNT = MI * NI * 16;
    if (!split_finish_ordered<COUNT, 256>(p.split_ws + (int64_t)logical_block * gridDim.y * (COUNT * 256), (int)blockIdx.y,
                                          (int)gridDim.y, p.split_tickets + logical_block,
                                          [&](int i) { return acc[i / (NI * 16)][(i / 16) % NI][i % 16]; },
                                          [&](int i, float v) { acc[i / (NI * 16)][(i / 16) % NI][i % 16] = v; }))
      return;
    mode -= 3;
  }
  const bool add_bias = p.bias != nullptr && (blockIdx.y == 0 || p.mode >= 3);
// ... 284 lines not shown
#pragma unroll
    for (int e = 0; e < NW; ++e) {
      const int flat = e * 256 + tid;
      Half8 v = rw[e];
      if (woff[e] < 0) v = Half8{{0u, 0u, 0u, 0u}};
      if (flat < WT_Q) stage_base[PATCH_Q + flat] = v;
    }
  };

  f32x16 acc[MI];
#pragma unroll
  for (int mi = 0; mi < MI; ++mi)
#pragma unroll
    for (int r = 0; r < 16; ++r) acc[mi][r] = 0.f;

  const int q = wave * 32 + l31, qi = q / PP, qy = (q / P) % P, qx = q % P;
  const int b_lane = lhi * (IMG * PHW) + qi * PHW + qy * PW + qx;
  const int a_lane = PATCH_Q + lhi * BM + l31;

  if (cbeg < cend) {
    fetch(cbeg);
    stage(cbeg, lds);
    __syncthreads();
    int cur = 0;
    for (int c0 = cbeg; c0 < cend; c0 += 16) {
      const bool more = c0 + 16 < cend;
      if (more) fetch(c0 + 16);
      const Half8* st = lds + cur * STAGE_Q;
#pragma unroll
      for (int tap = 0; tap < 9; ++tap) {
        const int kh = tap / 3, kw = tap % 3;
        frag a[MI];
#pragma unroll
        for (int mi = 0; mi < MI; ++mi) a[mi] = *reinterpret_cast<const frag*>(&st[a_lane + tap * 2 * BM + mi * 32]);
        const frag b = *reinterpret_cast<const frag*>(&st[b_lane + kh * PW + kw]);
#pragma unroll
        for (int mi = 0; mi < MI; ++mi) {
          if constexpr (PREC == 1) acc[mi] = __builtin_amdgcn_mfma_f32_32x32x16_bf16(a[mi], b, acc[mi], 0, 0, 0);
          else acc[mi] = __builtin_amdgcn_mfma_f32_32x32x16_f16(a[mi], b, acc[mi], 0, 0, 0);
        }
      }
      if (more) stage(c0 + 16, lds + (cur ^ 1) * STAGE_Q);
      __syncthreads();
      cur ^= 1;
    }
  }

  int mode = p.mode;
  if (mode >= 3) {
    constexpr int COUNT = MI * 16;
    if (!split_finish_ordered<COUNT, 256>(p.split_ws + (int64_t)block * gridDim.y * (COUNT * 256), (int)blockIdx.y, (int)gridDim.y,
                                          p.split_tickets + block, [&](int i) { return acc[i / 16][i % 16]; },
                                          [&](int i, float v) { acc[i / 16][i % 16] = v; }))
      return;
    mode -= 3;
  }
  if (n0 + qi >= p.N) return;
  float* out_n = p.out + (int64_t)(n0 + qi) * p.out_bs;
  const bool add_bias = p.bias != nullptr && (blockIdx.y == 0 || p.mode >= 3);
#pragma unroll
  for (int mi = 0; mi < MI; ++mi) {
#pragma unroll
    for (int r = 0; r < 16; ++r) {
      const int o = m0 + mi * 32 + (r & 3) + 8 * (r >> 2) + 4 * lhi;
      if (o >= p.CO) continue;
      float v = acc[mi][r];
      if (add_bias) v += p.bias[o];
      float* dst = out_n + (int64_t)o * PP + qy * P + qx;
      if (mode == 0) __builtin_nontemporal_store(v, dst);
      else if (mode == 1) *dst += v;
      else unsafeAtomicAdd(dst, v);
    }
  }
}

template <int BM, int CI_T, int TW, int TAPS>
static void launch_conv3_plain(const Conv3Params& p, int th, dim3 grid, hipStream_t stream) {
  if (th == 8) hipLaunchKernelGGL((conv3x3_lds_kernel<BM, 8, CI_T, false, TW, false, TAPS>), grid, dim3(256), 0, stream, p);
  else hipLaunchKernelGGL((conv3x3_lds_kernel<BM, 4, CI_T, false, TW, false, TAPS>), grid, dim3(256), 0, stream, p);
}

template <int BM, int CI_T, int TW>
static void launch_conv3_w(const Conv3Params& p, int th, dim3 grid, hipStream_t stream) {
  if (p.epi_x) {
    if (th == 8) hipLaunchKernelGGL((conv3x3_lds_kernel<BM, 8, CI_T, false, TW, true>), grid, dim3(256), 0, stream, p);
    else hipLaunchKernelGGL((conv3x3_lds_kernel<BM, 4, CI_T, false, TW, true>), grid, dim3(256), 0, stream, p);
  } else if (p.bn_mean) {
    if (th == 8) hipLaunchKernelGGL((conv3x3_lds_kernel<BM, 8, CI_T, true, TW>), grid, dim3(256), 0, stream, p);
    else hipLaunchKernelGGL((conv3x3_lds_kernel<BM, 4, CI_T, true, TW>), grid, dim3(256), 0, stream, p);
  } else {
    switch (p.taps) {
      case 0x01B: launch_conv3_plain<BM, CI_T, TW, 0x01B>(p, th, grid, stream); break;
      case 0x036: launch_conv3_plain<BM, CI_T, TW, 0x036>(p, th, grid, stream); break;
      case 0x0D8: launch_conv3_plain<BM, CI_T, TW, 0x0D8>(p, th, grid, stream); break;
      case 0x1B0: launch_conv3_plain<BM, CI_T, TW, 0x1B0>(p, th, grid, stream); break;
      default: launch_conv3_plain<BM, CI_T, TW, 0x1FF>(p, th, grid, stream); break;
    }
  }
}

template <int BM, int CI_T>
static void launch_conv3(const Conv3Params& p, int th, int tw, dim3 grid, hipStream_t stream) {
  if (tw == 16) launch_conv3_w<BM, CI_T, 16>(p, 4, grid, stream);
  else launch_conv3_w<BM, CI_T, 32>(p, th, grid, stream);
}

template <int BM, int PREC, int TAPS>
static void launch_conv3_mixed_taps(const Conv3Params& p, int th, int tw, dim3 grid, hipStream_t stream) {
  if (tw == 16) hipLaunchKernelGGL((conv3x3_mixed_kernel<BM, 4, 16, PREC, TAPS>), grid, dim3(256), 0, stream, p);
  else if (th == 8) hipLaunchKernelGGL((conv3x3_mixed_kernel<BM, 8, 32, PREC, TAPS>), grid, dim3(256), 0, stream, p);
  else hipLaunchKernelGGL((conv3x3_mixed_kernel<BM, 4, 32, PREC, TAPS>), grid, dim3(256), 0, stream, p);
}

template <int BM, int PREC>
static void launch_conv3_mixed_bm(const Conv3Params& p, int th, int tw, dim3 grid, hipStream_t stream) {
  switch (p.taps) {
    case 0x01B: launch_conv3_mixed_taps<BM, PREC, 0x01B>(p, th, tw, grid, stream); break;
    case 0x036: launch_conv3_mixed_taps<BM, PREC, 0x036>(p, th, tw, grid, stream); break;
    case 0x0D8: launch_conv3_mixed_taps<BM, PREC, 0x0D8>(p, th, tw, grid, stream); break;
    case 0x1B0: launch_conv3_mixed_taps<BM, PREC, 0x1B0>(p, th, tw, grid, stream); break;
    default: launch_conv3_mixed_taps<BM, PREC, 0x1FF>(p, th, tw, grid, stream); break;
  }
}

template <int P>
static void launch_conv3_mixed_small(const Conv3Params& p, int bm, int precision, dim3 grid, hipStream_t stream) {
  if (precision == 1) {
    if (bm == 64) hipLaunchKernelGGL((conv3x3_mixed_small_kernel<64, P, 1>), grid, dim3(256), 0, stream, p);
    else hipLaunchKernelGGL((conv3x3_mixed_small_kernel<32, P, 1>), grid, dim3(256), 0, stream, p);
  } else {
    if (bm == 64) hipLaunchKernelGGL((conv3x3_mixed_small_kernel<64, P, 2>), grid, dim3(256), 0, stream, p);
    else hipLaunchKernelGGL((conv3x3_mixed_small_kernel<32, P, 2>), grid, dim3(256), 0, stream, p);
  }
}

static void launch_conv3_mixed(const Conv3Params& p, int bm, int th, int tw, int precision, dim3 grid, hipStream_t stream) {
  if (precision == 1) {
    if (bm == 64) launch_conv3_mixed_bm<64, 1>(p, th, tw, grid, stream);
    else launch_conv3_mixed_bm<32, 1>(p, th, tw, grid, stream);
  } else {
    if (bm == 64) launch_conv3_mixed_bm<64, 2>(p, th, tw, grid, stream);
    else launch_conv3_mixed_bm<32, 2>(p, th, tw, grid, stream);
  }
}

struct Conv3Plan { int bm, th, tw, ci_t, tiles_x, tiles_y, tiles_m, split, chunks_per; int64_t blocks; bool small; };

static Conv3Plan conv3x3_plan(int32_t N, int32_t CI, int32_t CO, int32_t H, int32_t W, bool allow_split = true,
                              int precision = 0, bool small_ok = true) {
  Conv3Plan plan;
  plan.small = precision != 0 && small_ok && H == W && (W == 4 || W == 8);
  if (plan.small) {
    const int images = 128 / (H * W);
    plan.tw = W; plan.th = 4; plan.ci_t = 16; plan.tiles_x = 1;
    plan.bm = CO > 32 ? 64 : 32;
    plan.tiles_m = (CO + plan.bm - 1) / plan.bm;
    plan.tiles_y = (N + images - 1) / images;
    plan.blocks = (int64_t)plan.tiles_y * plan.tiles_m;
  } else {
  const int tw = W <= 16 ? 16 : 32;
  plan.tw = tw;
  plan.tiles_x = (W + tw - 1) / tw;
  int bm = CO > 32 ? 64 : 32;
  int th = tw == 16 ? 4 : 8;
  auto rows = [&](int th_) { return th_ * (32 / tw); };
  auto count = [&](int bm_, int th_) {
    return (int64_t)N * ((H + rows(th_) - 1) / rows(th_)) * plan.tiles_x * ((CO + bm_ - 1) / bm_);
  };
  while (count(bm, th) < 512) {
    if (th == 8) th = 4;
    else if (bm > 32) { bm >>= 1; th = 4; }
    else break;
  }
  plan.bm = bm; plan.th = th;
  plan.ci_t = bm == 64 ? 4 : 8;
  if (precision) plan.ci_t = 16;
  plan.tiles_m = (CO + bm - 1) / bm;
  plan.tiles_y = (H + rows(th) - 1) / rows(th);
  plan.blocks = count(bm, th);
  }
  const int chunks = (CI + plan.ci_t - 1) / plan.ci_t;
  int split = 1;
  constexpr int split_below = 384;
  if (allow_split && plan.blocks < split_below && chunks >= 4) {
    split = (int)((512 + plan.blocks - 1) / plan.blocks);
    if (split > chunks / 2) split = chunks / 2;
  }
  plan.chunks_per = (chunks + split - 1) / split;
  plan.split = (chunks + plan.chunks_per - 1) / plan.chunks_per;
  return plan;
}

int conv3x3_splits(int32_t N, int32_t CI, int32_t CO, int32_t H, int32_t W, int precision) {
  return conv3x3_plan(N, CI, CO, H, W, true, precision, false).split;
}

bool conv3x3_epilogue_supported(int32_t N, int32_t CI, int32_t CO, int32_t H, int32_t W) {
  return conv3x3_plan(N, CI, CO, H, W, false).bm <= 64;
}

int64_t conv3x3_epilogue_tiles(int32_t N, int32_t CI, int32_t CO, int32_t H, int32_t W) {
  const Conv3Plan plan = conv3x3_plan(N, CI, CO, H, W, false);
  return plan.blocks / plan.tiles_m;
}

int conv3x3_run(const float* in, int64_t in_bs, const float* w, int32_t w_base, int32_t w_so, int32_t w_si, int32_t w_skh,
                int32_t w_skw, const float* bias, float* out, int64_t out_bs, int32_t N, int32_t CI, int32_t CO, int32_t H,
                int32_t W, int accumulate, hipStream_t stream, const float* const* bn, const BnBackwardEpilogue* epilogue,
                int precision, const Conv3Placement* placement) {
  Conv3Params p;
  p.taps = placement ? placement->taps : 0x1FF;
  p.out_plane = placement ? placement->out_plane : H * W;
  p.out_sy = placement ? placement->out_sy : W;
  p.out_sx = placement ? placement->out_sx : 1;
  p.out_off = placement ? placement->out_off : 0;
  SRGAN_REQUIRE(placement == nullptr || (bn == nullptr && epilogue == nullptr), SRGAN_EUNSUPPORTED,
                "conv3x3 tap subsets / strided output: plain kernel only");
  SRGAN_REQUIRE(precision == 0 || (bn == nullptr && epilogue == nullptr), SRGAN_EUNSUPPORTED,
                "conv3x3 mixed precision: the fused batch-norm forms are fp32");
  p.in = in; p.w = w; p.out = out; p.bias = bias;
  p.bn_mean = bn ? bn[0] : nullptr; p.bn_inv = bn ? bn[1] : nullptr;
  p.bn_gamma = bn ? bn[2] : nullptr; p.bn_beta = bn ? bn[3] : nullptr;
  p.epi_x = nullptr; p.epi_x_bs = 0; p.epi_partial = nullptr; p.epi_tiles = 0; p.w_packed = nullptr;
  SRGAN_REQUIRE(bn == nullptr || CI <= CONV3_PRO_MAX_CI, SRGAN_EUNSUPPORTED, "conv3x3 fused batch-norm channel count");
  p.N = N; p.CI = CI; p.CO = CO; p.H = H; p.W = W;
  p.in_bs = in_bs; p.out_bs = out_bs;
  p.w_so = w_so; p.w_si = w_si; p.w_skh = w_skh; p.w_skw = w_skw; p.w_base = w_base;
  const Conv3Plan plan = conv3x3_plan(N, CI, CO, H, W, epilogue == nullptr, precision, placement == nullptr);
  const int bm = plan.bm, th = plan.th, tw = plan.tw, split = plan.split;
  p.tiles_x = plan.tiles_x; p.tiles_y = plan.tiles_y; p.tiles_m = plan.tiles_m;
  p.ci_per_split = plan.chunks_per * plan.ci_t;
  const int64_t blocks = plan.blocks;
  SRGAN_REQUIRE(blocks < (int64_t)1 << 31 && split <= 65535, SRGAN_ERANGE, "conv3x3 grid");
  p.split_ws = nullptr; p.split_tickets = nullptr;
  const int packed_slots = precision ? ((CI + 15) / 16) * 18 * CO : 0;
  if (split > 1) {
    int ticket_set = -1;
    const int64_t accumulators = (plan.small ? bm / 32 : (bm / 32) * (th / 4)) * 16 * 256;
    float* ws = split_workspace(blocks, split, accumulators, (size_t)packed_slots * sizeof(Half8), stream, &ticket_set);
    unsigned int* tickets = ws ? device_tickets(g_conv3_split_tickets) : nullptr;
    if (ws && tickets) {
      p.mode = accumulate == 1 ? 4 : 3;
      p.split_ws = ws;
      p.split_tickets = tickets + (size_t)ticket_set * SPLIT_TICKET_TILES;
    } else {
      SRGAN_REQUIRE(placement == nullptr || accumulate != 0, SRGAN_EUNSUPPORTED,
                    "conv3x3 strided output with an atomic K split needs a pre-zeroed (or accumulated) output");
      if (accumulate == 0)
        if (const int status = zero_rows(out, out_bs, (int64_t)CO * H * W, N, stream)) return status;
      p.mode = 2;
    }
  } else {
    p.mode = accumulate == 1 ? 1 : 0;
  }
  if (epilogue) {
    SRGAN_REQUIRE(!bn && !bias && !accumulate && split == 1 && bm <= 64, SRGAN_EUNSUPPORTED,
                  "conv3x3 batch-norm backward epilogue (store mode, unsplit, <= 64-row tile)");
    p.epi_x = epilogue->x; p.epi_x_bs = epilogue->x_bs;
    p.bn_mean = epilogue->bn[0]; p.bn_inv = epilogue->bn[1]; p.bn_gamma = epilogue->bn[2]; p.bn_beta = epilogue->bn[3];
    p.epi_tiles = (int32_t)(blocks / plan.tiles_m);
    if (epilogue->partial_out) {
      p.epi_partial = epilogue->partial_out;
    } else if (epilogue->g_gamma) {
      p.epi_partial = partial_workspace((size_t)2 * p.epi_tiles * CO * sizeof(float), stream);
      SRGAN_REQUIRE(p.epi_partial, SRGAN_EINVAL, "conv3x3 batch-norm backward epilogue: register a workspace for this "
                    "stream first (srgan_set_workspace, >= srgan_workspace_bytes())");
    }
  }
  p.xcd_remap = (blocks % 8 == 0 && blocks >= 64) ? 1 : 0;
  dim3 grid((unsigned)blocks, (unsigned)split, 1);
  const int profile_slot = profile_bracket_begin(stream);
  if (precision) {
    const int slots = packed_slots;
    Half8* packed = reinterpret_cast<Half8*>(partial_workspace((size_t)slots * sizeof(Half8), stream));
    SRGAN_REQUIRE(packed, SRGAN_EINVAL, "conv3x3 mixed precision: register a workspace for this stream first "
                  "(srgan_set_workspace, >= srgan_workspace_bytes(); the packed weights take 2 bytes per element)");
    if (precision == 1) hipLaunchKernelGGL(conv3x3_pack_weights_kernel<1>, dim3((slots + 255) / 256), dim3(256), 0, stream, p, packed, slots);
    else hipLaunchKernelGGL(conv3x3_pack_weights_kernel<2>, dim3((slots + 255) / 256), dim3(256), 0, stream, p, packed, slots);
    p.w_packed = packed;
    if (plan.small && W == 4) launch_conv3_mixed_small<4>(p, bm, precision, grid, stream);
    else if (plan.small) launch_conv3_mixed_small<8>(p, bm, precision, grid, stream);
    else launch_conv3_mixed(p, bm, th, tw, precision, grid, stream);
  }
  else if (bm == 32) launch_conv3<32, 8>(p, th, tw, grid, stream);
  else launch_conv3<64, 4>(p, th, tw, grid, stream);
  if (p.epi_partial && !epilogue->partial_out)
    bn_partial_reduce_run(p.epi_partial, p.epi_tiles, CO, p.bn_inv, epilogue->g_gamma, epilogue->g_beta, stream);
  const int status = launch_status();
  const int64_t pixels3 = (int64_t)N * H * W;
  profile_bracket_end(profile_slot, stream, CO, pixels3, (int64_t)CI * __builtin_popcount((unsigned)p.taps), 2, bm, th * 32, split, 0, 0,
                      (int64_t)CI * pixels3 + (epilogue ? (int64_t)CO * pixels3 : 0), precision);
  return status;
}

}
```

### sr-gan_amd/csrc/gather_gemm_kernels.hip

```cpp
#include "common.h"
#include "split_finish.h"
#include "gather_gemm.h"
#include "conv_plan.h"
#include "launchers.h"
#include <stdarg.h>
#include <string.h>
#include <stdlib.h>
#include <atomic>
#include <map>
#include <mutex>
#include <string>
#include <type_traits>
#include <type_traits>
#include <utility>

namespace srgan {

static thread_local char g_error[512] = "";

void set_error(const char* fmt, ...) {
  va_list ap;
  va_start(ap, fmt);
  vsnprintf(g_error, sizeof(g_error), fmt, ap);
  va_end(ap);
// ... 926 lines not shown
  SRGAN_REQUIRE(gy && w && gx, SRGAN_EINVAL, "srgan_conv2d_bwd_data pointers");
  SRGAN_REQUIRE(g.x_bs == (int64_t)g.C * g.H * g.W, SRGAN_EUNSUPPORTED, "srgan_conv2d_bwd_data dense gx");
  const int dtype = desc->compute_dtype;
  SRGAN_REQUIRE(dtype_ok(dtype), SRGAN_EINVAL, "srgan_conv2d_bwd_data compute_dtype");
  if (dtype && force_kernel == 0 && use_conv3x3_mixed(g, g.C))
    return conv3x3_run(gy, g.y_bs, w, 8, 9, g.C * 9, -3, -1, bias, gx, g.x_bs, g.N, g.K, g.C, g.H, g.W, accumulate,
                       (hipStream_t)stream, nullptr, nullptr, dtype);
  if (force_kernel == 0 && dtype == 0 && bias == nullptr && !accumulate &&
      stem7x7_geometry(g.C, g.K, g.R, g.S, g.sh, g.sw, g.ph, g.pw) && (g.W & 1) == 0 && (((uintptr_t)gx) & 7) == 0)
    return stem7x7_bwd_data_run(gy, g.y_bs, w, gx, g.x_bs, g.N, g.H, g.W, g.K, g.OH, g.OW, (hipStream_t)stream);
  if (force_kernel == 0 && g.R == 4 && g.S == 4 && g.sh == 2 && g.sw == 2 && g.ph == 1 &&
      g.pw == 1 && g.H == 2 * g.OH && g.W == 2 * g.OW && g.OW >= 8 && (g.C >= 8 || dtype) && !accumulate) {
    const bool split = conv3x3_splits(g.N, g.K, g.C, g.OH, g.OW, dtype) > 1 && !srgan_split_is_ordered(stream);
    if (split) if (const int status = zero_floats(gx, (int64_t)g.N * g.x_bs, (hipStream_t)stream)) return status;
    for (int a = 0; a < 2; ++a)
      for (int b = 0; b < 2; ++b) {
        Conv3Placement placement;
        placement.taps = (0x01B << (3 * a)) << b;
        placement.out_plane = g.H * g.W; placement.out_sy = 2 * g.W; placement.out_sx = 2; placement.out_off = a * g.W + b;
        const int status = conv3x3_run(gy, g.y_bs, w, (3 + a) * 4 + (3 + b), 16, g.C * 16, -8, -2, bias, gx, g.x_bs, g.N, g.K,
                                       g.C, g.OH, g.OW, split ? 2 : 0, (hipStream_t)stream, nullptr, nullptr, dtype, &placement);
        if (status != SRGAN_OK) return status;
      }
    return SRGAN_OK;
  }
  if (dtype) force_kernel = 2;
  if (use_pointwise(g, g.C, force_kernel))
    return pointwise_run(gy, g.y_bs, w, 1, g.C, bias, gx, g.x_bs, g.N, g.K, g.C, g.H * g.W, accumulate,
                         (hipStream_t)stream);
  if (use_conv3x3(g, g.C, force_kernel))
    return conv3x3_run(gy, g.y_bs, w, 8, 9, g.C * 9, -3, -1, bias, gx, g.x_bs, g.N, g.K, g.C, g.H, g.W, accumulate,
                       (hipStream_t)stream);
  std::vector<GatherGemm> plans = plan_conv_bwd_data(g, gy, w, bias, gx);
  for (GatherGemm& plan : plans) plan.precision = dtype;
  return gg_run_group(plans, gx, (int64_t)g.N * g.x_bs, accumulate, force_kernel, (hipStream_t)stream);
}

int srgan_conv2d_bwd_weight(const srgan_conv_desc* desc, const float* x, const float* gy, float* gw,
                            int accumulate, int force_kernel, void* stream) {
  ConvGeom g;
  SRGAN_GEOM(desc, g, "srgan_conv2d_bwd_weight");
  SRGAN_REQUIRE(x && gy && gw, SRGAN_EINVAL, "srgan_conv2d_bwd_weight pointers");
  const int dtype = desc->compute_dtype;
  SRGAN_REQUIRE(dtype_ok(dtype), SRGAN_EINVAL, "srgan_conv2d_bwd_weight compute_dtype");
  if (dtype && force_kernel == 0 && wgrad3x3_geometry(g, 8, true) &&
      (((uintptr_t)x | (uintptr_t)gy) & 15) == 0)
    return conv3x3_wgrad_run(x, g.x_bs, gy, g.y_bs, gw, g.N, g.C, g.K, g.H, g.W, accumulate, (hipStream_t)stream, nullptr,
                             dtype);
  if (dtype) force_kernel = 2;
  if (use_pointwise_wgrad(g, x, gy, force_kernel))
    return pointwise_wgrad_run(x, g.x_bs, gy, g.y_bs, gw, g.N, g.C, g.K, g.H * g.W, accumulate, (hipStream_t)stream);
  if (force_kernel == 0 && dtype == 0 && stem7x7_geometry(g.C, g.K, g.R, g.S, g.sh, g.sw, g.ph, g.pw))
    return stem7x7_wgrad_run(x, g.x_bs, gy, g.y_bs, gw, g.N, g.H, g.W, g.K, g.OH, g.OW, accumulate, (hipStream_t)stream);
  if (use_wgrad3x3(g, x, gy, force_kernel))
    return conv3x3_wgrad_run(x, g.x_bs, gy, g.y_bs, gw, g.N, g.C, g.K, g.H, g.W, accumulate, (hipStream_t)stream);
  std::vector<GatherGemm> plans{plan_conv_bwd_weight(g, x, gy, gw)};
  plans[0].precision = dtype;
  return gg_run_group(plans, gw, (int64_t)g.K * g.C * g.R * g.S, accumulate, force_kernel, (hipStream_t)stream);
}

static bool bn_ok(const srgan_bn_relu* bn) { return bn && bn->mean && bn->inv_std && bn->gamma && bn->beta; }

int srgan_conv2d_bnrelu_supported(const srgan_conv_desc* desc, int pass) {
  ConvGeom g;
  if (desc && desc->compute_dtype != 0) return 0;
  if (!to_geom(desc, g) || geom_largest_extent(g) >= ((int64_t)1 << 31)) return 0;
  if (pass == 0) {
    if (pointwise(g)) return use_pointwise(g, g.K, 0) ? 1 : 0;
    return (use_conv3x3(g, g.K, 0) && g.C <= 512) ? 1 : 0;
  }
  if (pass == 1) {
    if ((size_t)g.N * g.H * g.W * g.C / 8 > WORKSPACE_BYTES) return 0;
    if (pointwise(g)) return use_pointwise(g, g.C, 0) ? 1 : 0;
    return (use_conv3x3(g, g.C, 0) && conv3x3_epilogue_supported(g.N, g.K, g.C, g.H, g.W)) ? 1 : 0;
  }
  if (pass == 2) {
    if (pointwise(g)) return pointwise_wgrad_geometry(g) ? 1 : 0;
    return wgrad3x3_geometry(g) ? 1 : 0;
  }
  return 0;
}

static int fwd_bnrelu(const srgan_conv_desc* desc, const float* x, const srgan_bn_relu* bn, const float* w, const float* bias,
                      float* y, int y_state, int* plan_only_split, void* stream) {
  ConvGeom g;
  SRGAN_GEOM(desc, g, "srgan_conv2d_fwd_bnrelu");
  SRGAN_REQUIRE(plan_only_split || (x && w && y && bn_ok(bn)), SRGAN_EINVAL, "srgan_conv2d_fwd_bnrelu pointers");
  SRGAN_REQUIRE(srgan_conv2d_bnrelu_supported(desc, 0), SRGAN_EUNSUPPORTED, "srgan_conv2d_fwd_bnrelu geometry support");
  const float* const coefficients[4] = {bn ? bn->mean : nullptr, bn ? bn->inv_std : nullptr, bn ? bn->gamma : nullptr,
                                        bn ? bn->beta : nullptr};
  if (pointwise(g) && (plan_only_split || ((uintptr_t)w & 15) == 0) &&
      pointwise_ksplit_wanted(g.N, g.C, g.K, g.H * g.W, true)) {
    if (plan_only_split) { *plan_only_split = 1; return SRGAN_OK; }
    return pointwise_ksplit_run(x, g.x_bs, w, bias, y, g.y_bs, g.N, g.C, g.K, g.H * g.W, 0, (hipStream_t)stream,
                                coefficients);
  }
  if (pointwise(g))
    return pointwise_run(x, g.x_bs, w, g.C, 1, bias, y, g.y_bs, g.N, g.C, g.K, g.H * g.W, y_state, (hipStream_t)stream,
                         coefficients, nullptr, plan_only_split);
  if (plan_only_split) { *plan_only_split = conv3x3_splits(g.N, g.C, g.K, g.H, g.W); return SRGAN_OK; }
  return conv3x3_run(x, g.x_bs, w, 0, g.C * 9, 9, 3, 1, bias, y, g.y_bs, g.N, g.C, g.K, g.H, g.W, y_state,
                     (hipStream_t)stream, coefficients);
}

int srgan_conv2d_fwd_bnrelu(const srgan_conv_desc* desc, const float* x, const srgan_bn_relu* bn, const float* w,
                            const float* bias, float* y, void* stream) {
  return fwd_bnrelu(desc, x, bn, w, bias, y, 0, nullptr, stream);
}

int srgan_conv2d_fwd_bnrelu_into_zeros(const srgan_conv_desc* desc, const float* x, const srgan_bn_relu* bn, const float* w,
                                       const float* bias, float* y, void* stream) {
  return fwd_bnrelu(desc, x, bn, w, bias, y, 2, nullptr, stream);
}

int srgan_conv2d_fwd_bnrelu_splits(const srgan_conv_desc* desc) {
  int split = 0;
  return fwd_bnrelu(desc, nullptr, nullptr, nullptr, nullptr, nullptr, 0, &split, nullptr) == SRGAN_OK ? split : -1;
}

static int bwd_data_bnrelu(const srgan_conv_desc* desc, const float* gy, const float* w, const srgan_bn_relu* bn, const float* x,
                          float* gx, float* g_gamma, float* g_beta, float* partials, int accumulate, void* stream) {
  ConvGeom g;
  SRGAN_GEOM(desc, g, "srgan_conv2d_bwd_data_bnrelu");
  SRGAN_REQUIRE(gy && w && x && gx && bn_ok(bn), SRGAN_EINVAL, "srgan_conv2d_bwd_data_bnrelu pointers");
  SRGAN_REQUIRE((g_gamma == nullptr) == (g_beta == nullptr), SRGAN_EINVAL,
                "srgan_conv2d_bwd_data_bnrelu parameter gradients (both or neither)");
  SRGAN_REQUIRE(srgan_conv2d_bnrelu_supported(desc, 1), SRGAN_EUNSUPPORTED,
                "srgan_conv2d_bwd_data_bnrelu geometry support");
  BnBackwardEpilogue epilogue;
  epilogue.x = x; epilogue.x_bs = g.x_bs;
  epilogue.bn[0] = bn->mean; epilogue.bn[1] = bn->inv_std; epilogue.bn[2] = bn->gamma; epilogue.bn[3] = bn->beta;
  epilogue.g_gamma = g_gamma; epilogue.g_beta = g_beta; epilogue.partial_out = partials;
  if (pointwise(g))
    return pointwise_run(gy, g.y_bs, w, 1, g.C, nullptr, gx, g.x_bs, g.N, g.K, g.C, g.H * g.W, accumulate,
                         (hipStream_t)stream, nullptr, &epilogue);
  SRGAN_REQUIRE(!accumulate, SRGAN_EUNSUPPORTED, "srgan_conv2d_bwd_data_bnrelu 3x3: gx is stored, not accumulated");
  return conv3x3_run(gy, g.y_bs, w, 8, 9, g.C * 9, -3, -1, nullptr, gx, g.x_bs, g.N, g.K, g.C, g.H, g.W, 0,
                     (hipStream_t)stream, nullptr, &epilogue);
}

int srgan_conv2d_bwd_data_bnrelu(const srgan_conv_desc* desc, const float* gy, const float* w, const srgan_bn_relu* bn,
                                 const float* x, float* gx, float* g_gamma, float* g_beta, int accumulate, void* stream) {
  return bwd_data_bnrelu(desc, gy, w, bn, x, gx, g_gamma, g_beta, nullptr, accumulate, stream);
}

int64_t srgan_conv2d_bwd_data_bnrelu_tiles(const srgan_conv_desc* desc) {
  ConvGeom g;
  if (!to_geom(desc, g) || !srgan_conv2d_bnrelu_supported(desc, 1)) return -1;
  return pointwise(g) ? pointwise_epilogue_tiles(g.N, g.H * g.W) : conv3x3_epilogue_tiles(g.N, g.K, g.C, g.H, g.W);
}

int srgan_conv2d_bwd_data_bnrelu_partials(const srgan_conv_desc* desc, const float* gy, const float* w, const srgan_bn_relu* bn,
                                          const float* x, float* gx, float* partials, int accumulate, void* stream) {
  SRGAN_REQUIRE(partials != nullptr, SRGAN_EINVAL, "srgan_conv2d_bwd_data_bnrelu_partials: the partial-sum region");
  return bwd_data_bnrelu(desc, gy, w, bn, x, gx, nullptr, nullptr, partials, accumulate, stream);
}

int srgan_bn_partial_reduce_batched(const srgan_bn_reduce_job* jobs_device, int32_t count, int32_t max_channels, int32_t max_tiles,
                                    const float* scratch, void* stream) {
  SRGAN_REQUIRE(jobs_device && scratch && count > 0 && max_channels > 0 && max_tiles > 0, SRGAN_EINVAL,
                "srgan_bn_partial_reduce_batched arguments");
  SRGAN_REQUIRE(count <= 65535, SRGAN_ERANGE, "srgan_bn_partial_reduce_batched job count");
  return bn_partial_reduce_batched_run(jobs_device, count, max_channels, max_tiles, scratch, (hipStream_t)stream);
}

int srgan_conv2d_bwd_weight_bnrelu(const srgan_conv_desc* desc, const float* x, const srgan_bn_relu* bn, const float* gy,
                                   float* gw, int accumulate, void* stream) {
  ConvGeom g;
  SRGAN_GEOM(desc, g, "srgan_conv2d_bwd_weight_bnrelu");
  SRGAN_REQUIRE(x && gy && gw && bn_ok(bn), SRGAN_EINVAL, "srgan_conv2d_bwd_weight_bnrelu pointers");
  SRGAN_REQUIRE(srgan_conv2d_bnrelu_supported(desc, 2), SRGAN_EUNSUPPORTED,
                "srgan_conv2d_bwd_weight_bnrelu geometry support");
  const float* const coefficients[4] = {bn->mean, bn->inv_std, bn->gamma, bn->beta};
  if (pointwise(g))
    return pointwise_wgrad_run(x, g.x_bs, gy, g.y_bs, gw, g.N, g.C, g.K, g.H * g.W, accumulate, (hipStream_t)stream,
                               coefficients);
  return conv3x3_wgrad_run(x, g.x_bs, gy, g.y_bs, gw, g.N, g.C, g.K, g.H, g.W, accumulate, (hipStream_t)stream,
                           coefficients);
}

int srgan_wgrad_group_plan(const srgan_conv_desc* desc, const srgan_bn_relu* bn, int64_t x_offset, int64_t gy_offset, float* gw,
                           int64_t gw_offset, int32_t group_size, int64_t group_weights, int64_t partial_offset, void* job, int32_t* grid_x,
                           int32_t* grid_y, int32_t* ragged, int64_t* partial_floats) {
  ConvGeom g;
  SRGAN_GEOM(desc, g, "srgan_wgrad_group_plan");
  SRGAN_REQUIRE(job && grid_x && grid_y && ragged && partial_floats && (bn == nullptr || bn_ok(bn)) && x_offset >= 0 &&
                gy_offset >= 0 && gw_offset >= 0 && partial_offset >= 0 && group_size >= 1 && group_weights >= 0, SRGAN_EINVAL,
                "srgan_wgrad_group_plan arguments");
  SRGAN_REQUIRE(srgan_conv2d_bnrelu_supported(desc, 2), SRGAN_EUNSUPPORTED, "srgan_wgrad_group_plan geometry support");
  const float* const coefficients[4] = {bn ? bn->mean : nullptr, bn ? bn->inv_std : nullptr, bn ? bn->gamma : nullptr,
                                        bn ? bn->beta : nullptr};
  const float* const* fused = bn ? coefficients : nullptr;
  if (pointwise(g))
    return pointwise_wgrad_group_plan(x_offset, g.x_bs, gy_offset, g.y_bs, gw, gw_offset, g.N, g.C, g.K, g.H * g.W, fused,
                                      group_size, group_weights, partial_offset, job, grid_x, grid_y, ragged, partial_floats);
  return conv3x3_wgrad_group_plan(x_offset, g.x_bs, gy_offset, g.y_bs, gw, gw_offset, g.N, g.C, g.K, g.H, g.W, fused, group_size,
                                  partial_offset, job, grid_x, grid_y, ragged, partial_floats);
}

int srgan_wgrad_group_run(const void* jobs, int32_t count, int32_t kernel_size, int32_t grid_x, int32_t grid_y, int32_t ragged,
                          int32_t fused_bn, const float* x_base, const float* gy_base, float* gw_base, int64_t sum_co_ci_taps,
                          int64_t pixels, int64_t operand_elements, int64_t partial_floats, void* stream) {
  SRGAN_REQUIRE(jobs && x_base && gy_base && count >= 1 && grid_x >= 1 && grid_y >= 1 && (kernel_size == 1 || kernel_size == 3) &&
                partial_floats >= 0, SRGAN_EINVAL, "srgan_wgrad_group_run arguments");
  if (kernel_size == 1)
    return pointwise_wgrad_group_run(jobs, count, grid_x, grid_y, ragged, fused_bn, x_base, gy_base, gw_base, sum_co_ci_taps,
                                     pixels, operand_elements, partial_floats, (hipStream_t)stream);
  return conv3x3_wgrad_group_run(jobs, count, grid_x, grid_y, ragged, x_base, gy_base, gw_base, sum_co_ci_taps, pixels,
                                 operand_elements, partial_floats, (hipStream_t)stream);
}

int srgan_profile_begin(void) {
  std::lock_guard<std::mutex> lock(g_profile.mutex);
  g_profile.slots = 0;
  g_profile.records.clear();
  g_profile.flops = g_profile.mfma_flops = g_profile.bytes = 0.0;
  g_profile.launches = 0;
  g_profile.enabled.store(true, std::memory_order_release);
  return SRGAN_OK;
}

// ... 16 lines not shown
}

int srgan_profile_bytes(double* algorithmic_bytes_total) {
  std::lock_guard<std::mutex> lock(g_profile.mutex);
  if (algorithmic_bytes_total) *algorithmic_bytes_total = g_profile.bytes;
  return SRGAN_OK;
}

int srgan_profile_mixed(double* flops, double* kernel_ms) {
  std::lock_guard<std::mutex> lock(g_profile.mutex);
  double f = 0.0, total = 0.0;
  for (size_t i = 0; i < g_profile.slots; ++i) {
    const ProfileRecord& r = g_profile.records[i];
    if (r.M < 0 || r.precision == 0) continue;
    float ms = 0.f;
    if (hipEventElapsedTime(&ms, g_profile.events[2 * i], g_profile.events[2 * i + 1]) != hipSuccess) continue;
    total += ms;
    f += 2.0 * (double)r.M * (double)r.N * (double)r.K;
  }
  if (flops) *flops = f;
  if (kernel_ms) *kernel_ms = total;
  return SRGAN_OK;
}

int64_t srgan_profile_report(char* buffer, int64_t capacity) {
  struct Key { int32_t v[9]; bool operator<(const Key& o) const { return memcmp(v, o.v, sizeof(v)) < 0; } };
  struct Acc { int64_t count = 0; double ms = 0.0, bytes = 0.0; };
  std::map<Key, Acc> table;
  std::lock_guard<std::mutex> lock(g_profile.mutex);
  for (size_t i = 0; i < g_profile.slots; ++i) {
    const ProfileRecord& r = g_profile.records[i];
    if (r.M < 0) continue;
    float ms = 0.f;
    if (hipEventElapsedTime(&ms, g_profile.events[2 * i], g_profile.events[2 * i + 1]) != hipSuccess) continue;
    Key k{{r.M, r.N, r.K, r.kind, r.bm, r.bn, r.split, r.akf, r.bkf}};
    Acc& a = table[k];
    a.count += 1;
    a.ms += ms;
    a.bytes += r.bytes;
  }
  std::string out;
  char line[200];
  for (const auto& kv : table) {
    const int32_t* v = kv.first.v;
    snprintf(line, sizeof(line), "%d %d %d %d %d %d %d %d %d %lld %.4f %.0f\n", v[0], v[1], v[2], v[3], v[4], v[5], v[6], v[7],
             v[8], (long long)kv.second.count, kv.second.ms, kv.second.bytes);
    out += line;
  }
  if (buffer && capacity > 0) {
    const size_t n = out.size() < (size_t)capacity - 1 ? out.size() : (size_t)capacity - 1;
    memcpy(buffer, out.data(), n);
    buffer[n] = 0;
  }
  return (int64_t)out.size() + 1;
}

int64_t srgan_workspace_bytes(void) { return (int64_t)WORKSPACE_BYTES; }

int srgan_set_workspace(void* workspace, int64_t bytes, void* stream) {
  SRGAN_REQUIRE(workspace == nullptr || bytes >= (int64_t)WORKSPACE_BYTES, SRGAN_EINVAL,
                "srgan_set_workspace: at least srgan_workspace_bytes() bytes");
  SRGAN_REQUIRE(((uintptr_t)workspace & 15) == 0, SRGAN_EINVAL, "srgan_set_workspace: 16-byte alignment");
  return workspace_register((float*)workspace, (size_t)(bytes > 0 ? bytes : 0), (hipStream_t)stream);
}

int srgan_split_is_ordered(void* stream) {
  if (split_atomics_forced()) return 0;
  const int set = workspace_index((hipStream_t)stream);
  return set >= 0 && set < SPLIT_TICKET_SETS ? 1 : 0;
}

int srgan_capabilities(srgan_capabilities_t* out, int32_t out_bytes) {
  SRGAN_REQUIRE(out != nullptr && out_bytes >= (int32_t)sizeof(srgan_capabilities_t), SRGAN_EINVAL,
                "srgan_capabilities: output struct");
  memset(out, 0, sizeof(*out));
  out->abi_version = srgan_version();
  out->struct_bytes = (int32_t)sizeof(*out);
  snprintf(out->arch, sizeof(out->arch), "gfx950");
  out->dtypes = SRGAN_DTYPE_F32 | SRGAN_DTYPE_BF16 | SRGAN_DTYPE_F16;
  out->features = SRGAN_FEATURE_FUSED_BNRELU | SRGAN_FEATURE_SPLITK_WORKSPACE | SRGAN_FEATURE_LIVE_PROFILE |
                  SRGAN_FEATURE_BLOCKED16 | SRGAN_FEATURE_BATCHED_SHADOWS | SRGAN_FEATURE_CROWD_FULL_IMAGE |
                  SRGAN_FEATURE_IMAGE_BATCHES | SRGAN_FEATURE_BATCH_NORM_TRAIN | SRGAN_FEATURE_BLOCKED_BATCH_NORM |
                  SRGAN_FEATURE_BLOCKED_FROZEN_NORM | SRGAN_FEATURE_DEVICE_DRAWS | SRGAN_FEATURE_IMAGE_SUMMARIES |
                  SRGAN_FEATURE_DISTRIBUTION_SUMMARIES;
  out->workspace_bytes = (int64_t)WORKSPACE_BYTES;
  out->max_tensor_elements = ((int64_t)1 << 31) - 1;
  return SRGAN_OK;
}

int srgan_gemm_f32(int32_t M, int32_t N, int32_t K, const float* A, int64_t sai, int64_t sak, const float* B,
                   int64_t sbk, int64_t sbj, float* C, int64_t sci, int64_t scj, const float* bias,
                   int32_t bias_on_columns, int accumulate, int force_kernel, void* stream) {
  return srgan_gemm(M, N, K, A, sai, sak, B, sbk, sbj, C, sci, scj, bias, bias_on_columns, accumulate, force_kernel, 0, stream);
}

int srgan_gemm(int32_t M, int32_t N, int32_t K, const float* A, int64_t sai, int64_t sak, const float* B,
               int64_t sbk, int64_t sbj, float* C, int64_t sci, int64_t scj, const float* bias,
               int32_t bias_on_columns, int accumulate, int force_kernel, int compute_dtype, void* stream) {
  SRGAN_REQUIRE(M > 0 && N > 0 && K >= 0 && A && B && C, SRGAN_EINVAL, "srgan_gemm_f32 arguments");
  SRGAN_REQUIRE(dtype_ok(compute_dtype), SRGAN_EINVAL, "srgan_gemm compute_dtype");
  if (compute_dtype) force_kernel = 2;
  const int64_t lim = (int64_t)1 << 31;
  SRGAN_REQUIRE(M * sai + K * sak < lim && K * sbk + N * sbj < lim && M * sci + N * scj < lim, SRGAN_ERANGE,
                "srgan_gemm_f32 extents");
  SRGAN_REQUIRE((scj == 1 && sci == N) || (sci == 1 && scj == M), SRGAN_EUNSUPPORTED, "srgan_gemm_f32 dense C");
  GatherGemm p = plan_gemm(M, N, K, A, (int32_t)sai, (int32_t)sak, B, (int32_t)sbk, (int32_t)sbj, C, (int32_t)sci,
                           (int32_t)scj, bias, bias_on_columns);
  if (sci == 1 && scj != 1) {
    p = gg_transposed(p);
    choose_staging(p);
  }
  p.precision = compute_dtype;
  std::vector<GatherGemm> plans{p};
  return gg_run_group(plans, C, (int64_t)M * N, accumulate, force_kernel, (hipStream_t)stream);
}

}
```

### sr-gan_amd/csrc/launchers.h

```cpp
#pragma once
#include "common.h"

namespace srgan {

int profile_bracket_begin(hipStream_t stream);
int profile_bracket_end(int slot, hipStream_t stream, int64_t M, int64_t N, int64_t K, int kind, int bm, int bn, int split,
                        int akf = 0, int bkf = 0, int64_t b_unique = 0, int precision = 0);
int profile_bracket_end_bytes(int slot, hipStream_t stream, int64_t M, int64_t N, int64_t K, int kind, int bm, int bn, int split,
                              double bytes, int precision);

struct Conv3Placement { int32_t taps, out_plane, out_sy, out_sx, out_off; };
int conv3x3_splits(int32_t N, int32_t CI, int32_t CO, int32_t H, int32_t W, int precision = 0);
bool conv3x3_epilogue_supported(int32_t N, int32_t CI, int32_t CO, int32_t H, int32_t W);
int64_t conv3x3_epilogue_tiles(int32_t N, int32_t CI, int32_t CO, int32_t H, int32_t W);
int conv3x3_run(const float* in, int64_t in_bs, const float* w, int32_t w_base, int32_t w_so, int32_t w_si, int32_t w_skh,
                int32_t w_skw, const float* bias, float* out, int64_t out_bs, int32_t N, int32_t CI, int32_t CO, int32_t H,
                int32_t W, int accumulate, hipStream_t stream, const float* const* bn = nullptr,
                const BnBackwardEpilogue* epilogue = nullptr, int precision = 0, const Conv3Placement* placement = nullptr);

constexpr int GROUP_OVERSUBSCRIPTION = 4;

int conv3x3_wgrad_run(const float* x, int64_t x_bs, const float* gy, int64_t gy_bs, float* gw, int32_t N, int32_t CI,
                      int32_t CO, int32_t H, int32_t W, int accumulate, hipStream_t stream, const float* const* bn = nullptr,
                      int precision = 0);
int conv3x3_wgrad_group_plan(int64_t x_off, int64_t x_bs, int64_t gy_off, int64_t gy_bs, float* gw, int64_t gw_off, int32_t N, int32_t CI,
                             int32_t CO, int32_t H, int32_t W, const float* const* bn, int32_t group, int64_t partial_offset, void* job_out,
                             int32_t* grid_x, int32_t* grid_y, int32_t* ragged, int64_t* partial_floats);
int conv3x3_wgrad_group_run(const void* jobs, int32_t count, int32_t grid_x, int32_t grid_y, int32_t ragged,
                            const float* x_base, const float* gy_base, float* gw_base, int64_t flops_mn, int64_t pixels,
                            int64_t elements, int64_t partial_floats, hipStream_t stream);

int pointwise_run(const float* in, int64_t in_bs, const float* w, int32_t w_so, int32_t w_si, const float* bias, float* out,
                  int64_t out_bs, int32_t N, int32_t CI, int32_t CO, int32_t HW, int accumulate, hipStream_t stream,
                  const float* const* bn = nullptr, const BnBackwardEpilogue* epilogue = nullptr,
                  int* plan_only_split = nullptr);
int64_t pointwise_epilogue_tiles(int32_t N, int32_t HW);
void bn_partial_reduce_run(const float* partial, int tiles, int CO, const float* inv_std, float* g_gamma, float* g_beta,
                           hipStream_t stream);
int bn_partial_reduce_batched_run(const srgan_bn_reduce_job* jobs, int count, int max_channels, int max_tiles,
                                  const float* scratch, hipStream_t stream);

bool pointwise_ring_eligible(const float* in, int64_t in_bs, const float* w, int32_t w_so, int32_t w_si, const float* bias,
                             const float* out, int64_t out_bs, int32_t N, int32_t CI, int32_t CO, int32_t HW, bool fused_pro,
                             const BnBackwardEpilogue* epilogue, int* tile_pixels);
int pointwise_ring_run(const float* in, int64_t in_bs, const float* w, int32_t w_so, int32_t w_si, float* out, int64_t out_bs,
                       int32_t N, int32_t CI, int32_t CO, int32_t HW, int accumulate, hipStream_t stream,
                       const float* const* bn, const BnBackwardEpilogue* epilogue, float* epi_partial, int32_t epi_cols,
                       int tile_pixels, int32_t* rows_done);

bool pointwise_ksplit_wanted(int32_t N, int32_t K, int32_t M, int32_t HW, bool fused_bn);
int pointwise_ksplit_run(const float* in, int64_t in_bs, const float* w, const float* bias, float* out, int64_t out_bs,
                         int32_t N, int32_t K, int32_t M, int32_t HW, int accumulate, hipStream_t stream,
                         const float* const* bn);

bool pointwise_wgrad_enabled();
int pointwise_wgrad_run(const float* x, int64_t x_bs, const float* gy, int64_t gy_bs, float* gw, int32_t N, int32_t CI,
                        int32_t CO, int32_t HW, int accumulate, hipStream_t stream, const float* const* bn = nullptr);
int pointwise_wgrad_group_plan(int64_t x_off, int64_t x_bs, int64_t gy_off, int64_t gy_bs, float* gw, int64_t gw_off, int32_t N, int32_t CI,
                               int32_t CO, int32_t HW, const float* const* bn, int32_t group, int64_t group_weights, int64_t partial_offset,
                               void* job_out, int32_t* grid_x, int32_t* grid_y, int32_t* ragged, int64_t* partial_floats);
int pointwise_wgrad_group_run(const void* jobs, int32_t count, int32_t grid_x, int32_t grid_y, int32_t ragged, int32_t fused_bn,
                              const float* x_base, const float* gy_base, float* gw_base, int64_t flops_mn, int64_t pixels,
                              int64_t elements, int64_t partial_floats, hipStream_t stream);

int bn_train_stats_run(const float* x, float* mean, float* inv_std, float* running_mean, float* running_var,
                       int64_t* num_batches_tracked, float momentum, float eps, int32_t N, int32_t C, int64_t HW,
                       hipStream_t stream);
int bn_train_fwd_run(const float* x, const float* mean, const float* inv_std, const float* gamma, const float* beta, float slope,
                     float* y, int32_t N, int32_t C, int64_t HW, hipStream_t stream);
int bn_train_bwd_reduce_run(const float* g, const float* x, const float* mean, const float* inv_std, const float* gamma,
                            const float* beta, float slope, float* sums, float* g_gamma, float* g_beta, int32_t N, int32_t C,
                            int64_t HW, hipStream_t stream);
int bn_train_bwd_apply_run(const float* g, const float* x, const float* mean, const float* inv_std, const float* gamma,
                           const float* beta, float slope, const float* sums, float* gx, int32_t N, int32_t C, int64_t HW,
                           hipStream_t stream);

int h_frozen_norm_bwd_run(const void* s, const void* x, const float* mean, const float* inv_std, const float* gamma, const void* ref,
                          float slope, void* gx, float* g_gamma, float* g_beta, int32_t N, int32_t C, int64_t HW, int32_t dtype,
                          hipStream_t stream);

bool stem7x7_geometry(int32_t C, int32_t K, int32_t R, int32_t S, int32_t sh, int32_t sw, int32_t ph, int32_t pw);
int stem7x7_fwd_run(const float* x, int64_t x_bs, const float* w, float* y, int64_t y_bs, int32_t N, int32_t H, int32_t W,
                    int32_t K, int32_t OH, int32_t OW, hipStream_t stream);
int stem7x7_wgrad_run(const float* x, int64_t x_bs, const float* gy, int64_t gy_bs, float* gw, int32_t N, int32_t H, int32_t W,
                      int32_t K, int32_t OH, int32_t OW, int accumulate, hipStream_t stream);
int stem7x7_bwd_data_run(const float* gy, int64_t gy_bs, const float* w, float* gx, int64_t gx_bs, int32_t N, int32_t H,
                         int32_t W, int32_t K, int32_t OH, int32_t OW, hipStream_t stream);


int image_grid_run(const float* images, int32_t N, int32_t C, int32_t H, int32_t W, int32_t nrow, int32_t padding, float pad_value,
                   int32_t normalize, float low, float high, float* out, hipStream_t stream);
int density_heatmaps_run(const float* labels, const float* predicted, int32_t B, int32_t M, int32_t h, int32_t w, int32_t P,
                         const float* lut, int32_t lut_entries, float* tiles, int64_t tile_stride, float* ranges,
                         hipStream_t stream);

int wasserstein_run(const float* u, int32_t n, const float* v, int32_t m, float* out, hipStream_t stream);
int kde_curves_run(const float* samples, const int32_t* offsets, int32_t C, int32_t G, float factor, float cut, float* support,
                   float* density, float* stats, hipStream_t stream);
int curve_frame_run(const float* vertices, const int32_t* offsets, int32_t C, const float* colours, const float* widths, int32_t H,
                    int32_t W, float x_lo, float x_hi, float y_lo, float y_hi, const float* background, const float* grid_colour,
                    const float* x_ticks, int32_t n_x, const float* y_ticks, int32_t n_y, float* out, hipStream_t stream);
// ... 3 lines not shown
```

### sr-gan_amd/fused.py

```python

import torch

from . import _lib
from . import functional as F
from .tape import Var, Node, grad_enabled, incoming_gradient_is_exclusive, at_sweep_end
from .nn import parameter_var


ENABLED = True
POOL_FIRST = True
PROLOGUE = True
EPILOGUE = True
WGRAD_STREAM = False
_side_streams = {}


def _side_stream(device, main=None):
    key = (str(device), main.cuda_stream if main is not None else 0)
    if key not in _side_streams:
        _side_streams[key] = torch.cuda.Stream(device=device)
    return _side_streams[key]


def _launch_on_side_stream(device, tensors, launch):
# ... 95 lines not shown
        partial_at = 0
        weights = sum(width * (c0 + i * growth) if size == 1 else growth * width * 9 for i in range(len(layers)))
        for index, layer in enumerate(layers):
            cin = c0 + index * growth
            if size == 1:
                norm, gw = layer.norm1, layer.conv1.weight.grad
                if tangent is None:
                    desc, x_offset = _desc(n, cin, h, w, width, 1, 1, 1, 0, buffer_bs, 0), 0
                else:
                    desc, x_offset = _desc(n, cin, h, w, width, 1, 1, 1, 0), u1_offsets[index]
                gy_offset = index * n * width * hw
                co_ci_taps += width * cin
                elements += (cin + width) * n * hw
            else:
                desc, norm, gw = _desc(n, width, h, w, growth, 3, 3, 1, 1, 0, buffer_bs), layer.norm2, layer.conv2.weight.grad
                x_offset, gy_offset = index * n * width * hw, cin * hw
                co_ci_taps += growth * width * 9
                elements += (width + growth) * n * hw
            bn = None
            if tangent is None:
                inv, mean = norm._inverse_std()
                plan['keep'].append((inv, mean))
                bn = _lib.BnRelu(mean.data.data_ptr(), inv.data.data_ptr(), norm.weight.data_ptr(), norm.bias.data_ptr())
            gx, gy, rg, partial = ctypes.c_int32(), ctypes.c_int32(), ctypes.c_int32(), ctypes.c_int64()
            status = lib.srgan_wgrad_group_plan(desc, bn, x_offset, gy_offset, gw.data_ptr() if tangent is None else None,
                                                0 if tangent is None else tangent['offsets'][index][0 if size == 1 else 1],
                                                len(layers), weights, partial_at, ctypes.byref(slots, 128 * index), ctypes.byref(gx),
                                                ctypes.byref(gy), ctypes.byref(rg), ctypes.byref(partial))
            if status != 0:
                plans[key] = None
                return None
            partial_at += partial.value
            grid_x, grid_y, ragged = max(grid_x, gx.value), max(grid_y, gy.value), ragged | rg.value
        table = torch.frombuffer(bytearray(bytes(slots)), dtype=torch.uint8).to(device)
        plan[size] = dict(table=table, count=len(layers), grid_x=grid_x, grid_y=grid_y, ragged=ragged, co_ci_taps=co_ci_taps,
                          pixels=n * hw, elements=elements, partial_floats=partial_at)
    plans[key] = plan
    return plan


def _run_wgrad_group(group, size, fused_bn, x_base, gy_base, gw_base, stream):
    F._call('srgan_wgrad_group_run', group['table'].data_ptr(), group['count'], size, group['grid_x'], group['grid_y'],
            group['ragged'], 1 if fused_bn else 0, x_base.data_ptr(), gy_base.data_ptr(),
            gw_base.data_ptr() if gw_base is not None else None, group['co_ci_taps'], group['pixels'], group['elements'],
            group['partial_floats'], stream)


def _tangent_plan(layers, c0, growth, device):
    import ctypes
    key = (c0, str(device), layers[0].conv1.weight.data_ptr(), layers[-1].conv2.weight.grad.data_ptr())
    plans = layers[0].__dict__.setdefault('_srgan_tangent_plans', {})
    if key in plans:
        return plans[key]
    lib = _lib.library()
    slots = (ctypes.c_byte * (64 * 2 * len(layers)))()
    offsets, at, max_inner, max_co, keep = [], 0, 0, 0, []
    for index, layer in enumerate(layers):
        pair = []
        for which, (conv, norm, taps) in enumerate(((layer.conv1, layer.norm1, 1), (layer.conv2, layer.norm2, 9))):
            inv, _ = norm._inverse_std()
            keep.append(inv)
            co, ci = conv.weight.shape[0], conv.weight.shape[1]
            _lib.check(lib.srgan_bn_conv_tangent_weights_job(conv.weight.data_ptr(), inv.data.data_ptr(), norm.weight.data_ptr(),
                                                             conv.weight.grad.data_ptr(), norm.weight.grad.data_ptr(), at, co,
                                                             ci, taps, ctypes.byref(slots, 64 * (2 * index + which))),
                       'srgan_bn_conv_tangent_weights_job')
            pair.append(at)
            at += conv.weight.numel()
            max_inner, max_co = max(max_inner, ci * taps), max(max_co, co)
        offsets.append(tuple(pair))
    table = torch.frombuffer(bytearray(bytes(slots)), dtype=torch.uint8).to(device)
    plans[key] = dict(table=table, count=2 * len(layers), offsets=offsets, total=at, max_inner=max_inner, max_co=max_co,
                      keep=keep)
    return plans[key]


def _block_parameters(layers):
    cached = layers[0].__dict__.get('_srgan_block_parameters')
    if cached is None or cached[0] != len(layers):
        cached = layers[0].__dict__['_srgan_block_parameters'] = (len(layers), [p for layer in layers for p in layer.parameters()])
    return cached[1]


def dense_block(x, layers):
    n, c0, h, w = x.shape
    hw = h * w
    growth = layers[0].conv2.out_channels
    total = c0 + len(layers) * growth
    device = x.data.device
    stream = F._stream()
    buffer = _empty((n, total, h, w), device)
    buffer_bs = total * hw
    saved = []
    parameter_vars = [parameter_var(p) for p in _block_parameters(layers)]
    requires = grad_enabled() and (x.requires_grad or any(v.requires_grad for v in parameter_vars))
    train = requires and any(v.requires_grad for v in parameter_vars)
    width = layers[0].conv1.out_channels
    lib = _lib.library()
    probe1 = _desc(n, c0, h, w, width, 1, 1, 1, 0, buffer_bs, 0)
    probe2 = _desc(n, width, h, w, growth, 3, 3, 1, 1, 0, buffer_bs)
    prologue = PROLOGUE and all(lib.srgan_conv2d_bnrelu_supported(d, kind) for d in (probe1, probe2) for kind in (0, 2))
    epilogue1 = EPILOGUE and prologue and bool(lib.srgan_conv2d_bnrelu_supported(
        _desc(n, c0, h, w, width, 1, 1, 1, 0, buffer_bs, 0), 1))
    epilogue2 = EPILOGUE and prologue and bool(lib.srgan_conv2d_bnrelu_supported(probe2, 1))

    def bn_struct(norm):
        inv, mean = norm._inverse_std()
        return _lib.BnRelu(mean.data.data_ptr(), inv.data.data_ptr(), norm.weight.data_ptr(), norm.bias.data_ptr())

    zero_b1 = zero_new = False
    b1_all = None
    if prologue:
        last_cin = c0 + (len(layers) - 1) * growth
        atomics = not lib.srgan_split_is_ordered(stream)
        zero_b1 = atomics and lib.srgan_conv2d_fwd_bnrelu_splits(_desc(n, last_cin, h, w, width, 1, 1, 1, 0, buffer_bs, 0)) > 1
        zero_new = atomics and lib.srgan_conv2d_fwd_bnrelu_splits(probe2) > 1
        if zero_new:
            F._call('srgan_fill', buffer.data_ptr(), buffer.numel(), 0.0, stream)
        if zero_b1:
            b1_all = _zeros((len(layers), n, width, h, w), device)
        elif requires and GROUPED_WGRAD:
            b1_all = _empty((len(layers), n, width, h, w), device)
    F._call('srgan_copy_channels', x.data.data_ptr(), c0, 0, buffer.data_ptr(), total, 0, c0, n, hw, 0, stream)
    forward1 = 'srgan_conv2d_fwd_bnrelu_into_zeros' if zero_b1 else 'srgan_conv2d_fwd_bnrelu'
    forward2 = 'srgan_conv2d_fwd_bnrelu_into_zeros' if zero_new else 'srgan_conv2d_fwd_bnrelu'
    for index, layer in enumerate(layers):
        cin = c0 + index * growth
        b1 = b1_all[index] if b1_all is not None else _empty((n, width, h, w), device)
        if prologue:
            F._call(forward1, _desc(n, cin, h, w, width, 1, 1, 1, 0, buffer_bs, 0), buffer.data_ptr(),
                    bn_struct(layer.norm1), layer.conv1.weight.data_ptr(), None, b1.data_ptr(), stream)
            F._call(forward2, _desc(n, width, h, w, growth, 3, 3, 1, 1, 0, buffer_bs), b1.data_ptr(),
                    bn_struct(layer.norm2), layer.conv2.weight.data_ptr(), None, _ptr(buffer, cin * hw), stream)
            if requires:
                saved.append([None, b1, None])
            continue
        inv1, mean1 = layer.norm1._inverse_std()
        inv2, mean2 = layer.norm2._inverse_std()
        t1 = _empty((n, cin, h, w), device)
        F._call('srgan_chan_affine_act_strided', buffer.data_ptr(), mean1.data.data_ptr(), inv1.data.data_ptr(),
                layer.norm1.weight.data_ptr(), layer.norm1.bias.data_ptr(), None, 1, t1.data_ptr(), n, cin, hw,
                buffer_bs, 0, 0, 0, stream)
        F._call('srgan_conv2d_fwd', _desc(n, cin, h, w, width, 1, 1, 1, 0), t1.data_ptr(), layer.conv1.weight.data_ptr(),
                None, b1.data_ptr(), 0, stream)
        t2 = _empty((n, width, h, w), device)
        F._call('srgan_chan_affine_act', b1.data_ptr(), mean2.data.data_ptr(), inv2.data.data_ptr(),
                layer.norm2.weight.data_ptr(), layer.norm2.bias.data_ptr(), None, 1, t2.data_ptr(), n, width, hw, stream)
        F._call('srgan_conv2d_fwd', _desc(n, width, h, w, growth, 3, 3, 1, 1, 0, buffer_bs), t2.data_ptr(),
                layer.conv2.weight.data_ptr(), None, _ptr(buffer, cin * hw), 0, stream)
        if requires:
            saved.append([t1 if train else None, b1, t2 if train else None])

    out = Var(buffer, requires_grad=requires)
    if not requires:
        return out

    def norm_pointers(norm):
        inv, mean = norm._inverse_std()
        return mean.data.data_ptr(), inv.data.data_ptr(), norm.weight.data_ptr(), norm.bias.data_ptr()

    def backward(g, needs):
        recorded = grad_enabled()
        want_params = any(needs[1:])
        if recorded and want_params:
            raise NotImplementedError('a recorded (create_graph) backward of the fused dense block yields the input '
                                      'gradient only; set srgan_amd.fused.ENABLED = False for parameter gradients of '
                                      'a recorded backward')
        stream = F._stream()
        if not recorded and incoming_gradient_is_exclusive() and g.data.is_contiguous():
            gbuf = g.data
        else:
            gbuf = _empty(g.shape, device)
            F._call('srgan_ew_unary', F.U_COPY, g.data.data_ptr(), gbuf.data_ptr(), gbuf.numel(), 0.0, 0.0, stream)
        kept = [None] * len(layers)
        plan = scratch = None
        if BATCHED_REDUCE and want_params and (epilogue1 or epilogue2):
            plan = _reduce_plan(layers, n, c0, h, w, growth, buffer_bs, epilogue1, epilogue2, device)
            if plan is not None:
                scratch = _empty((plan['total'],), device)
        side_ok = WGRAD_STREAM and want_params and prologue and not recorded and not torch.cuda.is_current_stream_capturing()
        grouped = None
        if GROUPED_WGRAD and want_params and prologue and not recorded and b1_all is not None:
            grouped = _wgrad_plan(layers, n, c0, h, w, growth, buffer_bs, device)
        overlap = side_ok and grouped is None
        one_tensor = grouped is not None or (recorded and GROUPED_WGRAD and prologue)
        g_b1_all = _empty((len(layers), n, layers[0].conv1.out_channels, h, w), device) if one_tensor else None
        if overlap:
            main = torch.cuda.current_stream(device)
            side = _side_stream(device, main)
            wstream = _lib.stream_handle(side)
            alive = []
        else:
            wstream = stream
        for index in range(len(layers) - 1, -1, -1):
            layer = layers[index]
            t1, b1, t2 = saved[index]
            cin = c0 + index * growth
            width = layer.conv1.out_channels
            mean1, inv1, gamma1, beta1 = norm_pointers(layer.norm1)
            mean2, inv2, gamma2, beta2 = norm_pointers(layer.norm2)
            g_new = _ptr(gbuf, cin * hw)
            desc2 = _desc(n, width, h, w, growth, 3, 3, 1, 1, 0, buffer_bs)
            if overlap:
                side.wait_stream(main)
            if grouped is not None:
                pass
            elif want_params and prologue:
                F._call('srgan_conv2d_bwd_weight_bnrelu', desc2, b1.data_ptr(), bn_struct(layer.norm2), g_new,
                        layer.conv2.weight.grad.data_ptr(), 1, wstream)
            elif want_params:
                F._call('srgan_conv2d_bwd_weight', desc2, t2.data_ptr(), g_new, layer.conv2.weight.grad.data_ptr(), 1, 0,
                        stream)
            g_b1 = g_b1_all[index] if g_b1_all is not None else _empty(b1.shape, device)
            if epilogue2 and plan is not None:
                F._call('srgan_conv2d_bwd_data_bnrelu_partials', desc2, g_new, layer.conv2.weight.data_ptr(),
                        bn_struct(layer.norm2), b1.data_ptr(), g_b1.data_ptr(), _ptr(scratch, plan['offsets'][index][2]), 0, stream)
            elif epilogue2:
                F._call('srgan_conv2d_bwd_data_bnrelu', desc2, g_new, layer.conv2.weight.data_ptr(),
                        bn_struct(layer.norm2), b1.data_ptr(), g_b1.data_ptr(),
                        layer.norm2.weight.grad.data_ptr() if want_params else None,
                        layer.norm2.bias.grad.data_ptr() if want_params else None, 0, stream)
            else:
                g_t2 = _empty(b1.shape, device)
                F._call('srgan_conv2d_bwd_data', desc2, g_new, layer.conv2.weight.data_ptr(), None, g_t2.data_ptr(), 0, 0,
                        stream)
                F._call('srgan_bn_act_bwd', g_t2.data_ptr(), b1.data_ptr(), mean2, inv2, gamma2, beta2, 1,
                        g_b1.data_ptr(), layer.norm2.weight.grad.data_ptr() if want_params else None,
                        layer.norm2.bias.grad.data_ptr() if want_params else None, n, width, hw, 0, 0, 0, 0, 0, stream)
                del g_t2
            desc1 = _desc(n, cin, h, w, width, 1, 1, 1, 0)
            if overlap:
                side.wait_stream(main)
                alive.extend((g_b1, b1))
            if grouped is not None:
                pass
            elif want_params and prologue:
                F._call('srgan_conv2d_bwd_weight_bnrelu', _desc(n, cin, h, w, width, 1, 1, 1, 0, buffer_bs, 0),
                        buffer.data_ptr(), bn_struct(layer.norm1), g_b1.data_ptr(), layer.conv1.weight.grad.data_ptr(), 1,
                        wstream)
            elif want_params:
                F._call('srgan_conv2d_bwd_weight', desc1, t1.data_ptr(), g_b1.data_ptr(),
                        layer.conv1.weight.grad.data_ptr(), 1, 0, stream)
            if epilogue1 and plan is not None:
                F._call('srgan_conv2d_bwd_data_bnrelu_partials', _desc(n, cin, h, w, width, 1, 1, 1, 0, buffer_bs, 0),
                        g_b1.data_ptr(), layer.conv1.weight.data_ptr(), bn_struct(layer.norm1), buffer.data_ptr(),
                        gbuf.data_ptr(), _ptr(scratch, plan['offsets'][index][1]), 1, stream)
            elif epilogue1:
                F._call('srgan_conv2d_bwd_data_bnrelu', _desc(n, cin, h, w, width, 1, 1, 1, 0, buffer_bs, 0),
                        g_b1.data_ptr(), layer.conv1.weight.data_ptr(), bn_struct(layer.norm1), buffer.data_ptr(),
                        gbuf.data_ptr(), layer.norm1.weight.grad.data_ptr() if want_params else None,
                        layer.norm1.bias.grad.data_ptr() if want_params else None, 1, stream)
            else:
                g_t1 = _empty((n, cin, h, w), device)
                F._call('srgan_conv2d_bwd_data', desc1, g_b1.data_ptr(), layer.conv1.weight.data_ptr(), None,
                        g_t1.data_ptr(), 0, 0, stream)
                F._call('srgan_bn_act_bwd', g_t1.data_ptr(), buffer.data_ptr(), mean1, inv1, gamma1, beta1, 1,
                        gbuf.data_ptr(), layer.norm1.weight.grad.data_ptr() if want_params else None,
                        layer.norm1.bias.grad.data_ptr() if want_params else None, n, cin, hw, 0, buffer_bs, buffer_bs,
                        1, 0, stream)
            if recorded:
                kept[index] = (g_b1, b1)
            else:
                saved[index] = None
        if grouped is not None:
            def run_groups(on):
                _run_wgrad_group(grouped[3], 3, True, b1_all, gbuf, None, on)
                _run_wgrad_group(grouped[1], 1, True, buffer, g_b1_all, None, on)
            if side_ok:
                _launch_on_side_stream(device, (b1_all, gbuf, buffer, g_b1_all), run_groups)
            else:
                run_groups(stream)
        if plan is not None:
            F._call('srgan_bn_partial_reduce_batched', plan['jobs'].data_ptr(), plan['count'], plan['max_channels'],
                    plan['max_tiles'], scratch.data_ptr(), stream)
        if overlap:
            main.wait_stream(side)
            del alive
        gx = None
        if needs[0]:
            gx_data = _empty((n, c0, h, w), device)
            F._call('srgan_copy_channels', gbuf.data_ptr(), total, 0, gx_data.data_ptr(), c0, 0, c0, n, hw, 0, stream)
            gx = Var(gx_data)
            if recorded:
                gx.requires_grad = True
                gx.node = Node((g,) + tuple(parameter_vars), lambda v, needs2: double_backward(v, needs2, gbuf, kept, g_b1_all),
                               'dense_block_backward')
        return (gx,) + (None,) * len(parameter_vars)

    def double_backward(v, needs2, gbuf, kept, g_b1_all=None):
        if grad_enabled():
            raise NotImplementedError('third-order differentiation of the fused dense block')
        stream = F._stream()
        want_params = any(needs2[1:])
        vbuf = _empty((n, total, h, w), device)
        F._call('srgan_copy_channels', v.data.data_ptr(), c0, 0, vbuf.data_ptr(), total, 0, c0, n, hw, 0, stream)
        tangent = _tangent_plan(layers, c0, growth, device)
        scaled_all = _empty((tangent['total'],), device)
        q_all = _zeros((tangent['total'],), device) if want_params else None
        F._call('srgan_bn_conv_tangent_weights_grouped', tangent['table'].data_ptr(), tangent['count'], tangent['max_inner'],
# ... 124 lines not shown
```

Before: 87.66 images/s.

## Stream pre-packed 3x3 dense-block weight images into LDS via async DMA

Adds a per-layer packed weight image for the dense-block 3x3 convolutions (forward and transposed layouts, padded to 64 output channels). It is cached by the weight versions and built through the batched shadow packer. The conv3x3 LDS kernel gains a WIMG variant that double-buffers weight slices with global-to-LDS 16-byte DMA instead of register-staged strided loads, overlapping them with the MFMA loop. The aim is to cut weight gather and staging cost and free registers. The cost is extra repacking whenever weights change and more LDS per block from two weight stages.

```diff
diff --git a/include/srgan_hip.h b/include/srgan_hip.h
--- a/include/srgan_hip.h
+++ b/include/srgan_hip.h
@@ -27,6 +27,7 @@
 #define SRGAN_FEATURE_DEVICE_DRAWS 0x400u
 #define SRGAN_FEATURE_IMAGE_SUMMARIES 0x800u
 #define SRGAN_FEATURE_DISTRIBUTION_SUMMARIES 0x1000u
+#define SRGAN_FEATURE_CONV3X3_WEIGHT_IMAGE 0x2000u
 typedef struct srgan_capabilities_t {
   int32_t abi_version;
   int32_t struct_bytes;
@@ -86,6 +87,15 @@
                                           const float* x, float* gx, float* partials, int accumulate, void* stream);
 int srgan_bn_partial_reduce_batched(const srgan_bn_reduce_job* jobs_device, int32_t count, int32_t max_channels, int32_t max_tiles,
                                     const float* scratch, void* stream);
+int64_t srgan_conv3x3_image_floats(int32_t CI, int32_t CO);
+int srgan_conv2d_fwd_bnrelu_image(const srgan_conv_desc* desc, const float* x, const srgan_bn_relu* bn, const float* w,
+                                  const float* image, const float* bias, float* y, void* stream);
+int srgan_conv2d_bwd_data_bnrelu_image(const srgan_conv_desc* desc, const float* gy, const float* w, const float* image,
+                                       const srgan_bn_relu* bn, const float* x, float* gx, float* g_gamma, float* g_beta,
+                                       int accumulate, void* stream);
+int srgan_conv2d_bwd_data_bnrelu_partials_image(const srgan_conv_desc* desc, const float* gy, const float* w, const float* image,
+                                                const srgan_bn_relu* bn, const float* x, float* gx, float* partials,
+                                                int accumulate, void* stream);
 
 int srgan_wgrad_group_plan(const srgan_conv_desc* desc, const srgan_bn_relu* bn, int64_t x_offset, int64_t gy_offset, float* gw,
                            int64_t gw_offset, int32_t group_size, int64_t group_weights, int64_t partial_offset, void* job,
@@ -272,6 +282,9 @@
                                 int64_t rows_real, int64_t cols_real, int64_t row_stride, int64_t col_stride, int32_t row_plane,
                                 int32_t col_plane, int dtype);
 int64_t srgan_h_pack_job_bias_rows(void* jobs, int64_t first_block, const float* bias, float* rows, int32_t channels, int32_t plane);
+int srgan_h_pack_conv3x3_image(const float* w, float* image, int32_t K, int32_t C, int transposed, void* stream);
+int64_t srgan_h_pack_job_conv3x3_image(void* jobs, int64_t first_block, const float* w, float* image, int32_t K, int32_t C,
+                                       int transposed);
 int srgan_h_pack_batched(const void* jobs_device, int32_t count, int64_t blocks, void* stream);
 int srgan_h_conv4x4s2(const void* x, const void* packed, const float* bias, const void* ref, float slope, int epi, void* out,
                       int32_t N, int32_t C_in, int32_t rows, int32_t H, int32_t W, int dtype, void* stream);
diff --git a/sr-gan_amd/_lib.py b/sr-gan_amd/_lib.py
--- a/sr-gan_amd/_lib.py
+++ b/sr-gan_amd/_lib.py
@@ -44,6 +44,12 @@
     'srgan_conv2d_bwd_data_bnrelu_tiles': ([ctypes.POINTER(ConvDesc)], ctypes.c_int64),
     'srgan_conv2d_bwd_data_bnrelu_partials': ([ctypes.POINTER(ConvDesc), vp, vp, ctypes.POINTER(BnRelu), vp, vp, vp,
                                                ctypes.c_int, vp], ctypes.c_int),
+    'srgan_conv3x3_image_floats': ([i32, i32], ctypes.c_int64),
+    'srgan_conv2d_fwd_bnrelu_image': ([ctypes.POINTER(ConvDesc), vp, ctypes.POINTER(BnRelu), vp, vp, vp, vp, vp], ctypes.c_int),
+    'srgan_conv2d_bwd_data_bnrelu_image': ([ctypes.POINTER(ConvDesc), vp, vp, vp, ctypes.POINTER(BnRelu), vp, vp, vp, vp,
+                                            ctypes.c_int, vp], ctypes.c_int),
+    'srgan_conv2d_bwd_data_bnrelu_partials_image': ([ctypes.POINTER(ConvDesc), vp, vp, vp, ctypes.POINTER(BnRelu), vp, vp, vp,
+                                                     ctypes.c_int, vp], ctypes.c_int),
     'srgan_bn_partial_reduce_batched': ([vp, i32, i32, i32, vp, vp], ctypes.c_int),
     'srgan_conv2d_bwd_weight_bnrelu': ([ctypes.POINTER(ConvDesc), vp, ctypes.POINTER(BnRelu), vp, vp, ctypes.c_int, vp],
                                        ctypes.c_int),
@@ -138,6 +144,8 @@
     'srgan_h_pack_job_k4s2_weights': ([vp, i64, vp, vp, i32, i32, ctypes.c_int, ctypes.c_int, vp], ctypes.c_int64),
     'srgan_h_pack_job_matrix': ([vp, i64, vp, vp, i64, i64, i64, i64, i64, i64, i32, i32, ctypes.c_int], ctypes.c_int64),
     'srgan_h_pack_job_bias_rows': ([vp, i64, vp, vp, i32, i32], ctypes.c_int64),
+    'srgan_h_pack_conv3x3_image': ([vp, vp, i32, i32, ctypes.c_int, vp], ctypes.c_int),
+    'srgan_h_pack_job_conv3x3_image': ([vp, i64, vp, vp, i32, i32, ctypes.c_int], ctypes.c_int64),
     'srgan_h_pack_batched': ([vp, i32, i64, vp], ctypes.c_int),
     'srgan_h_conv4x4s2': ([vp, vp, vp, vp, f32, ctypes.c_int, vp, i32, i32, i32, i32, i32, ctypes.c_int, vp], ctypes.c_int),
     'srgan_h_conv_transpose4x4s2': ([vp, vp, vp, vp, f32, ctypes.c_int, vp, i32, i32, i32, i32, i32, ctypes.c_int, vp], ctypes.c_int),
diff --git a/sr-gan_amd/blocked16.py b/sr-gan_amd/blocked16.py
--- a/sr-gan_amd/blocked16.py
+++ b/sr-gan_amd/blocked16.py
@@ -251,6 +251,20 @@
         xm = x_side.meta
         _call('srgan_h_conv3x3_wgrad', x_side.data.data_ptr(), y_side.data.data_ptr(), into.data_ptr(), xm.n, xm.c, y_side.meta.c,
               xm.h, xm.w, xm.code, F._stream())
+
+
+class Conv3x3ImageShadow(Shadow):
+    kind = 'conv3x3_image'
+
+    def _measure(self):
+        self.k, self.c, r, s = self.module.weight.shape
+        if (r, s) != (3, 3):
+            raise ValueError('blocked16: a weight image is the operand of a 3x3 convolution')
+
+    def forms(self):
+        floats = _lib.library().srgan_conv3x3_image_floats
+        for name, transposed, rows, reduced in (('forward', 0, self.k, self.c), ('transposed', 1, self.c, self.k)):
+            yield Form(name, floats(reduced, rows) // 4, self.module.weight, 'conv3x3_image', (self.k, self.c, transposed), torch.float32)
 
 
 class K4s2Shadow(Shadow):
@@ -372,7 +386,7 @@
               self.features, self.c_in, 1, self.features, self.plane, 1, xm.code, F._stream())
 
 
-SHADOW_KINDS = {cls.kind: cls for cls in (Conv3x3Shadow, K4s2Shadow, LinearShadow, SeedShadow)}
+SHADOW_KINDS = {cls.kind: cls for cls in (Conv3x3Shadow, Conv3x3ImageShadow, K4s2Shadow, LinearShadow, SeedShadow)}
 BATCHED_KINDS = tuple(SHADOW_KINDS)
 
 
diff --git a/sr-gan_amd/csrc/blocked16.h b/sr-gan_amd/csrc/blocked16.h
--- a/sr-gan_amd/csrc/blocked16.h
+++ b/sr-gan_amd/csrc/blocked16.h
@@ -127,6 +127,20 @@
     v[j] = c < CI ? w[base + o * so + c * si + kh * skh + kw * skw] : 0.f;
   }
   packed[slot] = h_pack8<PREC>(v);
+}
+
+__host__ __device__ __forceinline__ int32_t conv3x3_image_co_pad(int32_t CO) { return (CO + 63) & ~63; }
+__host__ __device__ __forceinline__ int64_t conv3x3_image_floats(int32_t CI, int32_t CO) {
+  return (int64_t)((CI + 7) & ~7) * 9 * conv3x3_image_co_pad(CO);
+}
+__device__ __forceinline__ void conv3x3_image_element(const float* __restrict__ w, float* __restrict__ image, int64_t element,
+                                                      int32_t CO, int32_t CI, int32_t base, int32_t so, int32_t si, int32_t skh,
+                                                      int32_t skw) {
+  const int co_pad = conv3x3_image_co_pad(CO);
+  const int o = (int)(element % co_pad), row = (int)(element / co_pad);
+  const int ci = row / 9, tap = row - ci * 9;
+  const int kh = tap / 3, kw = tap - kh * 3;
+  image[element] = (o < CO && ci < CI) ? w[base + o * so + ci * si + kh * skh + kw * skw] : 0.f;
 }
 
 template <int PREC>
diff --git a/sr-gan_amd/csrc/blocked16.hip b/sr-gan_amd/csrc/blocked16.hip
--- a/sr-gan_amd/csrc/blocked16.hip
+++ b/sr-gan_amd/csrc/blocked16.hip
@@ -207,6 +207,14 @@
   h_pack_conv_weights_slot<PREC>(w, packed, slot, CO, CI, R, S, base, so, si, skh, skw);
 }
 
+__global__ __launch_bounds__(256) void conv3x3_image_kernel(const float* __restrict__ w, float* __restrict__ image, int64_t floats,
+                                                            int32_t CO, int32_t CI, int32_t base, int32_t so, int32_t si,
+                                                            int32_t skh, int32_t skw) {
+  const int64_t element = (int64_t)blockIdx.x * 256 + threadIdx.x;
+  if (element >= floats) return;
+  conv3x3_image_element(w, image, element, CO, CI, base, so, si, skh, skw);
+}
+
 __global__ __launch_bounds__(256) void h_pack_batched_kernel(const HPackJob* __restrict__ jobs, int32_t count) {
   __shared__ float tile[64][65];
   int lo = 0, hi = count - 1;
@@ -233,8 +241,10 @@
     const int tile_index = (int)(block - job.first_block);
     if (job.prec == 1) h_pack_matrix_tile<1>(job.w, job.packed, tile, tile_index, q[0], q[1], q[2], q[3], q[4], q[5], q[6], q[7]);
     else h_pack_matrix_tile<2>(job.w, job.packed, tile, tile_index, q[0], q[1], q[2], q[3], q[4], q[5], q[6], q[7]);
+  } else if (job.kind == 4) {
+    h_bias_rows_slot(job.w, reinterpret_cast<float*>(job.packed), slot, q[0], q[1]);
   } else {
-    h_bias_rows_slot(job.w, reinterpret_cast<float*>(job.packed), slot, q[0], q[1]);
+    conv3x3_image_element(job.w, reinterpret_cast<float*>(job.packed), slot, q[0], q[1], q[2], q[3], q[4], q[5], q[6]);
   }
 }
 
@@ -865,6 +875,18 @@
   job.p[7] = transposed ? -S : S; job.p[8] = transposed ? -1 : 1;
 }
 
+static void conv3x3_image_job(HPackJob& job, const float* w, float* image, int32_t K, int32_t C, int transposed) {
+  memset(&job, 0, sizeof(job));
+  const int rows = transposed ? C : K, reduced = transposed ? K : C;
+  job.w = w; job.packed = (Slot*)image; job.kind = 5; job.prec = 0;
+  job.slots = conv3x3_image_floats(reduced, rows);
+  job.p[0] = rows; job.p[1] = reduced;
+  job.p[2] = transposed ? 8 : 0;
+  job.p[3] = transposed ? 9 : C * 9;
+  job.p[4] = transposed ? C * 9 : 9;
+  job.p[5] = transposed ? -3 : 3; job.p[6] = transposed ? -1 : 1;
+}
+
 }
 
 using namespace srgan;
@@ -1058,6 +1080,33 @@
   job.w = bias; job.packed = (Slot*)rows; job.first_block = first_block; job.kind = 4; job.prec = 0;
   job.slots = (int64_t)(channels + 7) / 8 * plane;
   job.p[0] = channels; job.p[1] = plane;
+  memcpy(jobs, &job, sizeof(job));
+  return (job.slots + 255) / 256;
+}
+
+int64_t srgan_conv3x3_image_floats(int32_t CI, int32_t CO) {
+  return (CI > 0 && CO > 0) ? conv3x3_image_floats(CI, CO) : 0;
+}
+
+int srgan_h_pack_conv3x3_image(const float* w, float* image, int32_t K, int32_t C, int transposed, void* stream) {
+  SRGAN_REQUIRE(w && image && K > 0 && C > 0 && (transposed == 0 || transposed == 1) && (((uintptr_t)image) & 15) == 0 &&
+                (int64_t)K * C * 9 < ((int64_t)1 << 31), SRGAN_EINVAL, "srgan_h_pack_conv3x3_image arguments");
+  HPackJob job;
+  conv3x3_image_job(job, w, image, K, C, transposed);
+  const int32_t* q = job.p;
+  hipLaunchKernelGGL(conv3x3_image_kernel, dim3((unsigned)((job.slots + 255) / 256)), dim3(256), 0, (hipStream_t)stream, w, image,
+                     job.slots, q[0], q[1], q[2], q[3], q[4], q[5], q[6]);
+  return launch_status();
+}
+
+int64_t srgan_h_pack_job_conv3x3_image(void* jobs, int64_t first_block, const float* w, float* image, int32_t K, int32_t C,
+                                       int transposed) {
+  SRGAN_REQUIRE(jobs && first_block >= 0 && w && image && K > 0 && C > 0 && (transposed == 0 || transposed == 1) &&
+                (((uintptr_t)image) & 15) == 0 && (int64_t)K * C * 9 < ((int64_t)1 << 31), SRGAN_EINVAL,
+                "srgan_h_pack_job_conv3x3_image arguments");
+  HPackJob job;
+  conv3x3_image_job(job, w, image, K, C, transposed);
+  job.first_block = first_block;
   memcpy(jobs, &job, sizeof(job));
   return (job.slots + 255) / 256;
 }
diff --git a/sr-gan_amd/csrc/conv3x3.hip b/sr-gan_amd/csrc/conv3x3.hip
--- a/sr-gan_amd/csrc/conv3x3.hip
+++ b/sr-gan_amd/csrc/conv3x3.hip
@@ -1,5 +1,6 @@
 #include "common.h"
 #include "launchers.h"
+#include "lds_dma.h"
 #include "split_finish.h"
 #include <stdlib.h>
 #include <type_traits>
@@ -36,24 +37,29 @@
 
 __device__ unsigned int g_conv3_split_tickets[SPLIT_TICKET_SETS * SPLIT_TICKET_TILES];
 
-template <int BM, int TH, int CI_T, bool PRO, int TW, bool EPI = false, int TAPS = 0x1FF>
+template <int BM, int TH, int CI_T, bool PRO, int TW, bool EPI = false, int TAPS = 0x1FF, bool WIMG = false>
 __global__ __launch_bounds__(256, 2) void conv3x3_lds_kernel(const Conv3Params p) {
   static_assert(!EPI || !PRO, "the batch-norm backward epilogue pairs with the plain kernel");
   static_assert(TAPS == 0x1FF || (!EPI && !PRO), "tap subsets pair with the plain kernel");
+  static_assert(!WIMG || TAPS == 0x1FF, "the weight image holds the full window");
   constexpr int RPB = 32 / TW;
   constexpr int ROWS = TH * RPB;
   constexpr int PH = ROWS + 2, PW = TW + 2, PHPW = PH * PW;
   constexpr int MI = BM / 32, NI = TH / 4;
-  constexpr int LDW = BM + 1;
+  constexpr int LDW = WIMG ? BM : BM + 1;
   constexpr int PATCH = CI_T * PHPW, WTS = CI_T * 9 * BM;
-  constexpr int NP = (PATCH + 255) / 256, NW = (WTS + 255) / 256;
+  constexpr int NP = (PATCH + 255) / 256, NW = WIMG ? 0 : (WTS + 255) / 256;
+  constexpr int WSTAGE = CI_T * 9 * LDW;
+  constexpr int WDMA = WTS / 256, WROWS = 256 / BM;
   static_assert(CI_T % 2 == 0 && NI >= 1 && MI >= 1, "bad tile");
-  __shared__ float lds[PATCH + CI_T * 9 * LDW];
+  static_assert(!WIMG || (WTS % 256 == 0 && PATCH % 4 == 0 && 256 % BM == 0), "whole 16-byte DMA instructions, aligned stages");
+  __shared__ __attribute__((aligned(16))) float lds[PATCH + (WIMG ? 2 : 1) * WSTAGE];
   __shared__ float2 coef[PRO ? CONV3_PRO_MAX_CI : 1];
   float* patch = lds;
   float* wt = lds + PATCH;
 
-  const int tid = threadIdx.x, lane = tid & 63, wave = tid >> 6, l31 = lane & 31, lhi = lane >> 5;
+  const int tid = threadIdx.x, lane = tid & 63, l31 = lane & 31, lhi = lane >> 5;
+  const int wave = WIMG ? __builtin_amdgcn_readfirstlane(tid >> 6) : tid >> 6;
   int block = blockIdx.x;
   if (p.xcd_remap) block = (block & 7) * ((int)gridDim.x >> 3) + (block >> 3);
   const int logical_block = block;
@@ -66,7 +72,7 @@
   const int cend = min(p.CI, cbeg + p.ci_per_split);
   const int HW = p.H * p.W;
 
-  int poff[NP], woff[NW];
+  int poff[NP], woff[NW > 0 ? NW : 1];
 #pragma unroll
   for (int e = 0; e < NP; ++e) {
     const int flat = e * 256 + tid;
@@ -87,7 +93,7 @@
   }
   const float* in_n = p.in + (int64_t)n * p.in_bs;
 
-  float rp[NP], rw[NW];
+  float rp[NP], rw[NW > 0 ? NW : 1];
   auto fetch = [&](int c0) {
     const int room = cend - c0;
 #pragma unroll
@@ -126,6 +132,23 @@
     }
   };
 
+  const int co_pad = (p.CO + 63) & ~63;
+  const uint32_t w_lane = (uint32_t)(((lane * 4) / BM) * co_pad + (lane * 4) % BM) * 4u;
+  const uint32_t w_lds = ring_lds_address(wt);
+  auto dma_weights = [&](int c0, int stage_index) {
+    const float* slice = reinterpret_cast<const float*>(p.w_packed) + (int64_t)c0 * 9 * co_pad + m0;
+#pragma unroll
+    for (int q = 0; q < (WDMA + 3) / 4; ++q) {
+      const int j = wave + 4 * q;
+      if (j >= WDMA) continue;
+      const uint64_t source = (uint64_t)(slice + (int64_t)j * WROWS * co_pad);
+      const uint32_t base_lo = (uint32_t)__builtin_amdgcn_readfirstlane((int)(uint32_t)source);
+      const uint32_t base_hi = (uint32_t)__builtin_amdgcn_readfirstlane((int)(uint32_t)(source >> 32));
+      const uint64_t base = ((uint64_t)base_hi << 32) | base_lo;
+      ring_glds16((const void*)base, w_lane, __builtin_amdgcn_readfirstlane(w_lds + (uint32_t)(stage_index * WSTAGE + j * 256) * 4u));
+    }
+  };
+
   f32x16 acc[MI][NI];
 #pragma unroll
   for (int mi = 0; mi < MI; ++mi)
@@ -138,6 +161,7 @@
   const float* b_base = patch + lhi * PHPW + ((wave * NI) * RPB + l31 / TW) * PW + l31 % TW;
 
   if (cbeg < cend) {
+    if constexpr (WIMG) dma_weights(cbeg, 0);
     fetch(cbeg);
     if (PRO) {
       for (int c = tid; c < cend - cbeg; c += 256) {
@@ -148,13 +172,18 @@
       __syncthreads();
     }
     stage(cbeg);
+    if (WIMG) asm volatile("s_waitcnt vmcnt(0)" ::: "memory");
     __syncthreads();
+    int cur = 0;
     for (int c0 = cbeg; c0 < cend; c0 += CI_T) {
       const bool more = c0 + CI_T < cend;
-      if (more) fetch(c0 + CI_T);
+      if (more) {
+        fetch(c0 + CI_T);
+        if constexpr (WIMG) dma_weights(c0 + CI_T, cur ^ 1);
+      }
 #pragma unroll 1
       for (int cp = 0; cp < CI_T / 2; ++cp) {
-        const float* a_cp = a_base + cp * (2 * 9 * LDW);
+        const float* a_cp = a_base + (WIMG ? cur * WSTAGE : 0) + cp * (2 * 9 * LDW);
         const float* b_cp = b_base + cp * (2 * PHPW);
 #pragma unroll
         for (int tap = 0; tap < 9; ++tap) {
@@ -172,11 +201,13 @@
               acc[mi][ni] = __builtin_amdgcn_mfma_f32_32x32x2f32(a[mi], b[ni], acc[mi][ni], 0, 0, 0);
         }
       }
+      if (WIMG) asm volatile("s_waitcnt vmcnt(0)" ::: "memory");
       __syncthreads();
       if (more) {
         stage(c0 + CI_T);
         __syncthreads();
       }
+      cur ^= 1;
     }
   }
 
@@ -627,7 +658,13 @@
 
 template <int BM, int CI_T, int TW>
 static void launch_conv3_w(const Conv3Params& p, int th, dim3 grid, hipStream_t stream) {
-  if (p.epi_x) {
+  if (p.w_packed && p.epi_x) {
+    if (th == 8) hipLaunchKernelGGL((conv3x3_lds_kernel<BM, 8, CI_T, false, TW, true, 0x1FF, true>), grid, dim3(256), 0, stream, p);
+    else hipLaunchKernelGGL((conv3x3_lds_kernel<BM, 4, CI_T, false, TW, true, 0x1FF, true>), grid, dim3(256), 0, stream, p);
+  } else if (p.w_packed) {
+    if (th == 8) hipLaunchKernelGGL((conv3x3_lds_kernel<BM, 8, CI_T, true, TW, false, 0x1FF, true>), grid, dim3(256), 0, stream, p);
+    else hipLaunchKernelGGL((conv3x3_lds_kernel<BM, 4, CI_T, true, TW, false, 0x1FF, true>), grid, dim3(256), 0, stream, p);
+  } else if (p.epi_x) {
     if (th == 8) hipLaunchKernelGGL((conv3x3_lds_kernel<BM, 8, CI_T, false, TW, true>), grid, dim3(256), 0, stream, p);
     else hipLaunchKernelGGL((conv3x3_lds_kernel<BM, 4, CI_T, false, TW, true>), grid, dim3(256), 0, stream, p);
   } else if (p.bn_mean) {
@@ -752,7 +789,12 @@
 int conv3x3_run(const float* in, int64_t in_bs, const float* w, int32_t w_base, int32_t w_so, int32_t w_si, int32_t w_skh,
                 int32_t w_skw, const float* bias, float* out, int64_t out_bs, int32_t N, int32_t CI, int32_t CO, int32_t H,
                 int32_t W, int accumulate, hipStream_t stream, const float* const* bn, const BnBackwardEpilogue* epilogue,
-                int precision, const Conv3Placement* placement) {
+                int precision, const Conv3Placement* placement, const float* w_image) {
+  static const bool no_image = getenv("SRGAN_NO_CONV3_IMAGE") != nullptr && atoi(getenv("SRGAN_NO_CONV3_IMAGE")) == 1;
+  if (no_image) w_image = nullptr;
+  SRGAN_REQUIRE(w_image == nullptr || (precision == 0 && placement == nullptr && (bn != nullptr) != (epilogue != nullptr) &&
+                                       (((uintptr_t)w_image) & 15) == 0), SRGAN_EUNSUPPORTED,
+                "conv3x3 weight image: the fp32 fused batch-norm forms, full window, 16-byte aligned image");
   Conv3Params p;
   p.taps = placement ? placement->taps : 0x1FF;
   p.out_plane = placement ? placement->out_plane : H * W;
@@ -827,13 +869,17 @@
     else if (plan.small) launch_conv3_mixed_small<8>(p, bm, precision, grid, stream);
     else launch_conv3_mixed(p, bm, th, tw, precision, grid, stream);
   }
-  else if (bm == 32) launch_conv3<32, 8>(p, th, tw, grid, stream);
-  else launch_conv3<64, 4>(p, th, tw, grid, stream);
+  else {
+    p.w_packed = w_image;
+    if (bm == 32) launch_conv3<32, 8>(p, th, tw, grid, stream);
+    else launch_conv3<64, 4>(p, th, tw, grid, stream);
+  }
   if (p.epi_partial && !epilogue->partial_out)
     bn_partial_reduce_run(p.epi_partial, p.epi_tiles, CO, p.bn_inv, epilogue->g_gamma, epilogue->g_beta, stream);
   const int status = launch_status();
   const int64_t pixels3 = (int64_t)N * H * W;
-  profile_bracket_end(profile_slot, stream, CO, pixels3, (int64_t)CI * __builtin_popcount((unsigned)p.taps), 2, bm, th * 32, split, 0, 0,
+  profile_bracket_end(profile_slot, stream, CO, pixels3, (int64_t)CI * __builtin_popcount((unsigned)p.taps), 2, bm, th * 32, split,
+                      (precision == 0 && p.w_packed) ? 1 : 0, 0,
                       (int64_t)CI * pixels3 + (epilogue ? (int64_t)CO * pixels3 : 0), precision);
   return status;
 }
diff --git a/sr-gan_amd/csrc/gather_gemm_kernels.hip b/sr-gan_amd/csrc/gather_gemm_kernels.hip
--- a/sr-gan_amd/csrc/gather_gemm_kernels.hip
+++ b/sr-gan_amd/csrc/gather_gemm_kernels.hip
@@ -1032,13 +1032,14 @@
 }
 
 static int fwd_bnrelu(const srgan_conv_desc* desc, const float* x, const srgan_bn_relu* bn, const float* w, const float* bias,
-                      float* y, int y_state, int* plan_only_split, void* stream) {
+                      float* y, int y_state, int* plan_only_split, void* stream, const float* image = nullptr) {
   ConvGeom g;
   SRGAN_GEOM(desc, g, "srgan_conv2d_fwd_bnrelu");
   SRGAN_REQUIRE(plan_only_split || (x && w && y && bn_ok(bn)), SRGAN_EINVAL, "srgan_conv2d_fwd_bnrelu pointers");
   SRGAN_REQUIRE(srgan_conv2d_bnrelu_supported(desc, 0), SRGAN_EUNSUPPORTED, "srgan_conv2d_fwd_bnrelu geometry support");
   const float* const coefficients[4] = {bn ? bn->mean : nullptr, bn ? bn->inv_std : nullptr, bn ? bn->gamma : nullptr,
                                         bn ? bn->beta : nullptr};
+  SRGAN_REQUIRE(image == nullptr || !pointwise(g), SRGAN_EUNSUPPORTED, "srgan_conv2d_fwd_bnrelu_image: 3x3 convolutions");
   if (pointwise(g) && (plan_only_split || ((uintptr_t)w & 15) == 0) &&
       pointwise_ksplit_wanted(g.N, g.C, g.K, g.H * g.W, true)) {
     if (plan_only_split) { *plan_only_split = 1; return SRGAN_OK; }
@@ -1050,7 +1051,13 @@
                          coefficients, nullptr, plan_only_split);
   if (plan_only_split) { *plan_only_split = conv3x3_splits(g.N, g.C, g.K, g.H, g.W); return SRGAN_OK; }
   return conv3x3_run(x, g.x_bs, w, 0, g.C * 9, 9, 3, 1, bias, y, g.y_bs, g.N, g.C, g.K, g.H, g.W, y_state,
-                     (hipStream_t)stream, coefficients);
+                     (hipStream_t)stream, coefficients, nullptr, 0, nullptr, image);
+}
+
+int srgan_conv2d_fwd_bnrelu_image(const srgan_conv_desc* desc, const float* x, const srgan_bn_relu* bn, const float* w,
+                                  const float* image, const float* bias, float* y, void* stream) {
+  SRGAN_REQUIRE(image != nullptr, SRGAN_EINVAL, "srgan_conv2d_fwd_bnrelu_image: the weight image");
+  return fwd_bnrelu(desc, x, bn, w, bias, y, 0, nullptr, stream, image);
 }
 
 int srgan_conv2d_fwd_bnrelu(const srgan_conv_desc* desc, const float* x, const srgan_bn_relu* bn, const float* w,
@@ -1069,7 +1076,8 @@
 }
 
 static int bwd_data_bnrelu(const srgan_conv_desc* desc, const float* gy, const float* w, const srgan_bn_relu* bn, const float* x,
-                          float* gx, float* g_gamma, float* g_beta, float* partials, int accumulate, void* stream) {
+                          float* gx, float* g_gamma, float* g_beta, float* partials, int accumulate, void* stream,
+                          const float* image = nullptr) {
   ConvGeom g;
   SRGAN_GEOM(desc, g, "srgan_conv2d_bwd_data_bnrelu");
   SRGAN_REQUIRE(gy && w && x && gx && bn_ok(bn), SRGAN_EINVAL, "srgan_conv2d_bwd_data_bnrelu pointers");
@@ -1081,12 +1089,28 @@
   epilogue.x = x; epilogue.x_bs = g.x_bs;
   epilogue.bn[0] = bn->mean; epilogue.bn[1] = bn->inv_std; epilogue.bn[2] = bn->gamma; epilogue.bn[3] = bn->beta;
   epilogue.g_gamma = g_gamma; epilogue.g_beta = g_beta; epilogue.partial_out = partials;
+  SRGAN_REQUIRE(image == nullptr || !pointwise(g), SRGAN_EUNSUPPORTED, "srgan_conv2d_bwd_data_bnrelu_image: 3x3 convolutions");
   if (pointwise(g))
     return pointwise_run(gy, g.y_bs, w, 1, g.C, nullptr, gx, g.x_bs, g.N, g.K, g.C, g.H * g.W, accumulate,
                          (hipStream_t)stream, nullptr, &epilogue);
   SRGAN_REQUIRE(!accumulate, SRGAN_EUNSUPPORTED, "srgan_conv2d_bwd_data_bnrelu 3x3: gx is stored, not accumulated");
   return conv3x3_run(gy, g.y_bs, w, 8, 9, g.C * 9, -3, -1, nullptr, gx, g.x_bs, g.N, g.K, g.C, g.H, g.W, 0,
-                     (hipStream_t)stream, nullptr, &epilogue);
+                     (hipStream_t)stream, nullptr, &epilogue, 0, nullptr, image);
+}
+
+int srgan_conv2d_bwd_data_bnrelu_image(const srgan_conv_desc* desc, const float* gy, const float* w, const float* image,
+                                       const srgan_bn_relu* bn, const float* x, float* gx, float* g_gamma, float* g_beta,
+                                       int accumulate, void* stream) {
+  SRGAN_REQUIRE(image != nullptr, SRGAN_EINVAL, "srgan_conv2d_bwd_data_bnrelu_image: the weight image");
+  return bwd_data_bnrelu(desc, gy, w, bn, x, gx, g_gamma, g_beta, nullptr, accumulate, stream, image);
+}
+
+int srgan_conv2d_bwd_data_bnrelu_partials_image(const srgan_conv_desc* desc, const float* gy, const float* w, const float* image,
+                                                const srgan_bn_relu* bn, const float* x, float* gx, float* partials,
+                                                int accumulate, void* stream) {
+  SRGAN_REQUIRE(partials != nullptr && image != nullptr, SRGAN_EINVAL,
+                "srgan_conv2d_bwd_data_bnrelu_partials_image: the partial-sum region and the weight image");
+  return bwd_data_bnrelu(desc, gy, w, bn, x, gx, nullptr, nullptr, partials, accumulate, stream, image);
 }
 
 int srgan_conv2d_bwd_data_bnrelu(const srgan_conv_desc* desc, const float* gy, const float* w, const srgan_bn_relu* bn,
@@ -1269,7 +1293,7 @@
                   SRGAN_FEATURE_BLOCKED16 | SRGAN_FEATURE_BATCHED_SHADOWS | SRGAN_FEATURE_CROWD_FULL_IMAGE |
                   SRGAN_FEATURE_IMAGE_BATCHES | SRGAN_FEATURE_BATCH_NORM_TRAIN | SRGAN_FEATURE_BLOCKED_BATCH_NORM |
                   SRGAN_FEATURE_BLOCKED_FROZEN_NORM | SRGAN_FEATURE_DEVICE_DRAWS | SRGAN_FEATURE_IMAGE_SUMMARIES |
-                  SRGAN_FEATURE_DISTRIBUTION_SUMMARIES;
+                  SRGAN_FEATURE_DISTRIBUTION_SUMMARIES | SRGAN_FEATURE_CONV3X3_WEIGHT_IMAGE;
   out->workspace_bytes = (int64_t)WORKSPACE_BYTES;
   out->max_tensor_elements = ((int64_t)1 << 31) - 1;
   return SRGAN_OK;
diff --git a/sr-gan_amd/csrc/launchers.h b/sr-gan_amd/csrc/launchers.h
--- a/sr-gan_amd/csrc/launchers.h
+++ b/sr-gan_amd/csrc/launchers.h
@@ -16,7 +16,8 @@
 int conv3x3_run(const float* in, int64_t in_bs, const float* w, int32_t w_base, int32_t w_so, int32_t w_si, int32_t w_skh,
                 int32_t w_skw, const float* bias, float* out, int64_t out_bs, int32_t N, int32_t CI, int32_t CO, int32_t H,
                 int32_t W, int accumulate, hipStream_t stream, const float* const* bn = nullptr,
-                const BnBackwardEpilogue* epilogue = nullptr, int precision = 0, const Conv3Placement* placement = nullptr);
+                const BnBackwardEpilogue* epilogue = nullptr, int precision = 0, const Conv3Placement* placement = nullptr,
+                const float* w_image = nullptr);
 
 constexpr int GROUP_OVERSUBSCRIPTION = 4;
 
diff --git a/sr-gan_amd/fused.py b/sr-gan_amd/fused.py
--- a/sr-gan_amd/fused.py
+++ b/sr-gan_amd/fused.py
@@ -201,6 +201,31 @@
     return cached[1]
 
 
+WEIGHT_IMAGE = True
+
+
+def _weight_images(layers):
+    from . import blocked16
+    cache = layers[0].__dict__.get('_srgan_weight_images')
+    if cache is None or cache['count'] != len(layers):
+        weights = [layer.conv2.weight for layer in layers]
+        arena = getattr(weights[0], '_srgan_arena', None)
+        if arena is None or any(getattr(w, '_srgan_arena', None) is not arena for w in weights):
+            return None
+        if blocked16._capturing():
+            return None
+        cache = layers[0].__dict__['_srgan_weight_images'] = dict(
+            count=len(layers), weights=weights, arena=arena, stamp=None, pointers=None,
+            shadows=[blocked16.shadow_of(layer.conv2, 'conv3x3_image', 0) for layer in layers])
+    arena = cache['arena']
+    stamp = (getattr(arena, 'version', 0), arena.data._version, cache['weights'][0].data_ptr(),
+             tuple(w._version for w in cache['weights']))
+    if stamp != cache['stamp']:
+        cache['pointers'] = [(s.forward.data_ptr(), s.transposed.data_ptr()) for s in (shadow.fresh() for shadow in cache['shadows'])]
+        cache['stamp'] = stamp
+    return cache['pointers']
+
+
 def dense_block(x, layers):
     n, c0, h, w = x.shape
     hw = h * w
@@ -243,14 +268,20 @@
     F._call('srgan_copy_channels', x.data.data_ptr(), c0, 0, buffer.data_ptr(), total, 0, c0, n, hw, 0, stream)
     forward1 = 'srgan_conv2d_fwd_bnrelu_into_zeros' if zero_b1 else 'srgan_conv2d_fwd_bnrelu'
     forward2 = 'srgan_conv2d_fwd_bnrelu_into_zeros' if zero_new else 'srgan_conv2d_fwd_bnrelu'
+    images = _weight_images(layers) if (WEIGHT_IMAGE and prologue) else None
     for index, layer in enumerate(layers):
         cin = c0 + index * growth
         b1 = b1_all[index] if b1_all is not None else _empty((n, width, h, w), device)
         if prologue:
             F._call(forward1, _desc(n, cin, h, w, width, 1, 1, 1, 0, buffer_bs, 0), buffer.data_ptr(),
                     bn_struct(layer.norm1), layer.conv1.weight.data_ptr(), None, b1.data_ptr(), stream)
-            F._call(forward2, _desc(n, width, h, w, growth, 3, 3, 1, 1, 0, buffer_bs), b1.data_ptr(),
-                    bn_struct(layer.norm2), layer.conv2.weight.data_ptr(), None, _ptr(buffer, cin * hw), stream)
+            if images is not None and not zero_new:
+                F._call('srgan_conv2d_fwd_bnrelu_image', _desc(n, width, h, w, growth, 3, 3, 1, 1, 0, buffer_bs), b1.data_ptr(),
+                        bn_struct(layer.norm2), layer.conv2.weight.data_ptr(), images[index][0], None, _ptr(buffer, cin * hw),
+                        stream)
+            else:
+                F._call(forward2, _desc(n, width, h, w, growth, 3, 3, 1, 1, 0, buffer_bs), b1.data_ptr(),
+                        bn_struct(layer.norm2), layer.conv2.weight.data_ptr(), None, _ptr(buffer, cin * hw), stream)
             if requires:
                 saved.append([None, b1, None])
             continue
@@ -286,6 +317,7 @@
                                       'gradient only; set srgan_amd.fused.ENABLED = False for parameter gradients of '
                                       'a recorded backward')
         stream = F._stream()
+        images = _weight_images(layers) if (WEIGHT_IMAGE and epilogue2) else None
         if not recorded and incoming_gradient_is_exclusive() and g.data.is_contiguous():
             gbuf = g.data
         else:
@@ -331,9 +363,17 @@
                 F._call('srgan_conv2d_bwd_weight', desc2, t2.data_ptr(), g_new, layer.conv2.weight.grad.data_ptr(), 1, 0,
                         stream)
             g_b1 = g_b1_all[index] if g_b1_all is not None else _empty(b1.shape, device)
-            if epilogue2 and plan is not None:
+            if epilogue2 and plan is not None and images is not None:
+                F._call('srgan_conv2d_bwd_data_bnrelu_partials_image', desc2, g_new, layer.conv2.weight.data_ptr(), images[index][1],
+                        bn_struct(layer.norm2), b1.data_ptr(), g_b1.data_ptr(), _ptr(scratch, plan['offsets'][index][2]), 0, stream)
+            elif epilogue2 and plan is not None:
                 F._call('srgan_conv2d_bwd_data_bnrelu_partials', desc2, g_new, layer.conv2.weight.data_ptr(),
                         bn_struct(layer.norm2), b1.data_ptr(), g_b1.data_ptr(), _ptr(scratch, plan['offsets'][index][2]), 0, stream)
+            elif epilogue2 and images is not None:
+                F._call('srgan_conv2d_bwd_data_bnrelu_image', desc2, g_new, layer.conv2.weight.data_ptr(), images[index][1],
+                        bn_struct(layer.norm2), b1.data_ptr(), g_b1.data_ptr(),
+                        layer.norm2.weight.grad.data_ptr() if want_params else None,
+                        layer.norm2.bias.grad.data_ptr() if want_params else None, 0, stream)
             elif epilogue2:
                 F._call('srgan_conv2d_bwd_data_bnrelu', desc2, g_new, layer.conv2.weight.data_ptr(),
                         bn_struct(layer.norm2), b1.data_ptr(), g_b1.data_ptr(),
```

New measurement: 88.77 images/s, median of 6. +1.3%, better.
